# theEricMa/TriplaneTurbo

Measured on AMD Instinct MI355X. Metric: rendered rays/sec (fwd+bwd) at 256x256 rays x 128 samples, higher is better.
Workload: dtype f32 (fp32-grade: exact 3-piece fp16 operand split, 6 x v_mfma_f32_32x32x16_f16 per k-step, fp32 accumulation)

## Files before the change

### triplaneturbo_amd/csrc/tt_backward.hip

```cpp
#include "tt_backward_common.h"

struct BwdGeoParams {
    const float* packed;
    MlpPtrs w;
    const float* rays_o;
    const float* rays_d;
    const float* t_starts;
    const float* t_ends;
    tt_render_cfg cfg;
    TileGeom geom;
    long long n_items;
    int* queue;
    const float* ws;
    int n_copies;
    float* grad_packed;
    MlpGradPtrs grads;
    unsigned long long* phase_cycles;
};

#define GEO_SCRATCH_FLOATS (2 * 64 * XS)
#define GOFF_W1T LDS_GEO_FLOATS
#define GOFF_W2T (GOFF_W1T + IMG16_FLOATS(32, 64))
#define LDS_GEO16_FLOATS (GOFF_W2T + IMG16_FLOATS(64, 64))
#define GLO_W1 LDS_GEO16_FLOATS
#define GLO_W2 (GLO_W1 + LO16_FLOATS(64, 32))
#define GLO_W1T (GLO_W2 + LO16_FLOATS(64, 64))
#define GLO_W2T (GLO_W1T + LO16_FLOATS(32, 64))
#define LDS_GEO3_FLOATS (GLO_W2T + LO16_FLOATS(64, 64))
template <int PREC>
struct GeoWFloats {
    static constexpr int value = PREC == PREC_S3 ? LDS_GEO3_FLOATS : LDS_GEO16_FLOATS;
};

template <int PREC, bool WG16, bool STATS = false>
__global__ __launch_bounds__(256, 1) void k_decode_bwd_geo(BwdGeoParams p) {
    constexpr bool EXACT = PREC == PREC_F32;
    constexpr int NT = PrecNT<PREC>::value, WF = GeoWFloats<PREC>::value;
    __shared__ __attribute__((aligned(16))) float L[WF + 4 * (GEO_SCRATCH_FLOATS + SCATTER_TAG_INTS)];
    {
        MlpPtrs w = p.w;
        stage_weights<PREC, 64, 32>(L + OFF_W1, L + GLO_W1, w.w1);
        stage_weights<PREC, 64, 64>(L + OFF_W2, L + GLO_W2, w.w2);
        lds_load_matrix(L + OFF_W3, w.w3, 1, 64, 64);
        stage_weights_t<PREC, 64, 32>(L + GOFF_W1T, L + GLO_W1T, w.w1);
        stage_weights_t<PREC, 64, 64>(L + GOFF_W2T, L + GLO_W2T, w.w2);
    }
    const tt_render_cfg& cfg = p.cfg;
    float sA1 = 1.f, sU = 1.f, sA2 = 1.f, sV = 1.f;
    if (WG16) {
        const unsigned* bnd = reinterpret_cast<const unsigned*>(p.queue) + TT_SLOT_BOUNDS;
        const float Pm = __builtin_bit_cast(float, bnd[TT_BOUND_PLANES]), Sb = __builtin_bit_cast(float, bnd[TT_BOUND_UP0]),
                    Gb = __builtin_bit_cast(float, bnd[TT_BOUND_UP1]);
        unsigned* word = reinterpret_cast<unsigned*>(L + WF);
        const int t = threadIdx.x;
        float w1row = 0.f, a1col = 0.f, w3abs = 0.f;
        if (t < 64) {
            for (int c = 0; c < 32; ++c) w1row += __builtin_fabsf(p.w.w1[t * 32 + c]);
            for (int r = 0; r < 64; ++r) a1col += __builtin_fabsf(p.w.w2[r * 64 + t]) * __builtin_fabsf(p.w.w3[r]);
            w3abs = __builtin_fabsf(p.w.w3[t]);
        }
        const float W1max = block_max(w1row, word), A1max = block_max(a1col, word), A2max = block_max(w3abs, word);
        const float jsum = (0.5f * cfg.plane_w + 0.5f * cfg.plane_h) / cfg.radius;
        const float Fmax = 3.f * Pm, H1max = W1max * Fmax;
        const float Umax = Fmax * (Sb + 2.f * jsum * Gb), QBmax = Fmax * 2.f * jsum * Gb;
        const float Vmax = Sb * H1max + W1max * QBmax;
        sA1 = wg16_scale(A1max);
        sU = wg16_scale(Umax);
        sA2 = wg16_scale(A2max);
        sV = wg16_scale(Vmax);
    }
    const TileGeom& tg = p.geom;
    const int lane = threadIdx.x & 63, i = lane & 31, hi = lane >> 5, wave_in_blk = threadIdx.x >> 6;
    float* Xs = L + WF + wave_in_blk * (GEO_SCRATCH_FLOATS + SCATTER_TAG_INTS);
    float* Ys = Xs + 64 * XS;
    int* tags = reinterpret_cast<int*>(Ys + 64 * XS);
    scatter_init_tags(tags, lane);
    __syncthreads();
    const int S = cfg.n_samples;
    ItemQueue iq = item_queue(p.queue, tg.n_blocks, tg.n_chunks, tg.unit);
    const int H = cfg.plane_h, W = cfg.plane_w;
    const size_t HW = (size_t)H * W;
    const size_t plane_stride = 6 * HW * TT_C;
    const float ju = 0.5f * W / cfg.radius, jv = 0.5f * H / cfg.radius;
    float* const grad_out =
        p.grad_packed + (size_t)(blockIdx.x % (unsigned)p.n_copies) * cfg.n_prompts * plane_stride;
    const unsigned grad_bytes =
        TT_DBG(cfg.flags, TT_DBG_NO_ATOMICS) ? 0u : (unsigned)(cfg.n_prompts * plane_stride * sizeof(float));

    const TileStats st = STATS ? tile_stats(cfg.stats) : TileStats{nullptr};
    f32x16 accW1[2][1] = {{ZERO16}, {ZERO16}};
    f32x16 accW2[2][2] = {{ZERO16, ZERO16}, {ZERO16, ZERO16}};
    float accw3 = 0.f;
#ifdef TT_TUNING
    unsigned long long ph_acc[20] = {0, 0, 0, 0, 0, 0, 0, 0, 0, 0, 0, 0, 0, 0, 0, 0, 0, 0, 0, 0};
    unsigned long long ph_t = __builtin_amdgcn_s_memtime();
#endif

#pragma nounroll
    for (;;) {
        long long b;
        int ck;
        if (!item_pop(iq, tg.order, tg.n_chunks, b, ck)) break;
        if (b >= tg.n_blocks) continue;
        bool ray_ok;
        const long long ray = tile_ray(tg, b, i, ray_ok);
        const float ray_okf = tt_opaque(ray_ok ? 1.f : 0.f);
        const int ks = i % tg.sb;
        const int view = (int)(ray / cfg.rays_per_view);
        const size_t pofs = (size_t)(view / cfg.views_per_prompt) * plane_stride;
        const float ox = p.rays_o[ray * 3 + 0], oy = p.rays_o[ray * 3 + 1], oz = p.rays_o[ray * 3 + 2];
        const float dx = p.rays_d ? p.rays_d[ray * 3 + 0] : 0.f, dy = p.rays_d ? p.rays_d[ray * 3 + 1] : 0.f,
                    dz = p.rays_d ? p.rays_d[ray * 3 + 2] : 0.f;
        const int s_end = (ck + 1) * tg.chunk < S ? (ck + 1) * tg.chunk : S;
        struct StepIn {
            f32x4 up;
            float ts, te;
        };
        auto load_step = [&](int sb0) {
            StepIn r;
            const int si = sb0 + ks;
            const long long sidx = ray * S + (si < S ? si : S - 1);
            r.up = *reinterpret_cast<const f32x4*>(p.ws + sidx * 4);
            r.ts = p.rays_d ? p.t_starts[sidx] : 0.f;
            r.te = p.rays_d ? p.t_ends[sidx] : 0.f;
            return r;
        };
        StepIn in = load_step(ck * tg.chunk), in_next;
#pragma nounroll
        for (int sb0 = ck * tg.chunk; sb0 < s_end; sb0 += tg.sb, in = in_next) {
            in_next = load_step(sb0 + tg.sb);
            const int si = sb0 + ks;
            const bool rvalid = ray_ok && si < s_end;
            const float vf = ray_okf * (si < s_end ? 1.f : 0.f);
            const float sbar = in.up[0] * vf, gbx = in.up[1] * vf, gby = in.up[2] * vf, gbz = in.up[3] * vf;
            tile_stat(st, TT_STAT_VISITED);
            TT_PHASE(0);
            if (!__any(!((__builtin_fabsf(sbar) + __builtin_fabsf(gbx)) + (__builtin_fabsf(gby) + __builtin_fabsf(gbz)) <=
                         cfg.skip_eps_geo)))
                continue;
            float tm, px, py, pz;
            sample_position(ox, oy, oz, dx, dy, dz, in.ts, in.te, tm, px, py, pz);
            const float X = scale_coord(px, cfg.radius), Y = scale_coord(py, cfg.radius),
                        Z = scale_coord(pz, cfg.radius);
            float f[16], u[16];
            bool anyp[3];
            const bool any = __any(gather_geo_bwd_c(p.packed, (unsigned)(pofs / TT_C), H, W, X, Y, Z, rvalid, sbar, gbx,
                                                    gby, gbz, ju, jv, lane, Xs, f, u, anyp,
                                                    tile_stat_ptr(st, TT_STAT_INBOUNDS)));
            TT_PHASE(1);
            if (!any) continue;
            tile_stat(st, TT_STAT_EXECUTED);
            float h1[32], h2[32], a2[32], a1[32], q[16], u1, u2;
            mvx<PREC, 64, 32, true>(L + OFF_W1, L + GLO_W1, f, h1, i, hi, 1.f, &u1);
#pragma unroll
            for (int r = 0; r < 32; ++r) h1[r] = fmaxf(h1[r], 0.f);
            mvx<PREC, 64, 64, true>(L + OFF_W2, L + GLO_W2, h1, h2, i, hi, u1, &u2);
#pragma unroll
            for (int r = 0; r < 32; ++r) h2[r] = fmaxf(h2[r], 0.f);
#pragma unroll
            for (int g = 0; g < 8; ++g) {
                f32x4 w3 = *reinterpret_cast<const f32x4*>(L + OFF_W3 + 8 * g + 4 * hi);
#pragma unroll
                for (int e2 = 0; e2 < 4; ++e2) a2[4 * g + e2] = h2[4 * g + e2] > 0.f ? w3[e2] : 0.f;
            }
            Split16<64, PAIR_SEQ, NT> a2s, a1s;
            float ua1 = 1.f;
            if (WG16) {
                split16_vec<64, PAIR_SEQ, NT>(a2, sA2, a2s);
                mv16_pre<64, 64, true, NT>(L + GOFF_W2T, a2s, 1.f / sA2, a1, i, hi, &ua1, L + GLO_W2T);
            } else {
                mvtx_copy<PREC, 64, 64, 64>(L + GOFF_W2T, L + GLO_W2T, L + OFF_W2, a2, a1, i, hi);
            }
#pragma unroll
            for (int r = 0; r < 32; ++r) a1[r] = h1[r] > 0.f ? a1[r] : 0.f;
            if (WG16) {
                split16_vec<64, PAIR_SEQ, NT>(a1, sA1 * ua1, a1s);
                mv16_pre<32, 64, false, NT>(L + GOFF_W1T, a1s, 1.f / sA1, q, i, hi, nullptr, L + GLO_W1T);
            } else {
                mvtx_copy<PREC, 32, 64, 32>(L + GOFF_W1T, L + GLO_W1T, L + OFF_W1, a1, q, i, hi);
            }
            TT_PHASE(3);
            {
                float qb[16];
#pragma unroll
                for (int r = 0; r < 16; ++r) qb[r] = fmaf(-sbar, f[r], u[r]);
                const bool region = WG16 ? true : cfg.flags >= 0;
                const bool do_wgrad = region && !TT_DBG(cfg.flags, TT_DBG_NO_WGRAD);
                if (do_wgrad) {
                    if (WG16) {
                        stage_rows16_pre<64>(Xs, a1s, i, hi);
                        stage_rows16<32>(Ys, u, i, hi, sU);
                        wgrad16<64, 32>(accW1, Xs, Ys, i, hi);
                    } else {
                        stage_rows<64>(Xs, a1, i, hi);
                        stage_rows<32>(Ys, u, i, hi);
                        wgrad<64, 32>(accW1, Xs, Ys, i, hi);
                    }
                }
                TT_PHASE(7);
                float t1[32];
                mvx<PREC, 64, 32>(L + OFF_W1, L + GLO_W1, qb, t1, i, hi);
#pragma unroll
                for (int r = 0; r < 32; ++r) t1[r] = h1[r] > 0.f ? t1[r] : 0.f;
                float v[32];
#pragma unroll
                for (int r = 0; r < 32; ++r) v[r] = fmaf(sbar * u1, h1[r], t1[r]);
                TT_PHASE(4);
                if (do_wgrad) {
                    if (WG16) {
                        stage_rows16_pre<64>(Xs, a2s, i, hi);
                        stage_rows16<64>(Ys, v, i, hi, sV);
                        wgrad16<64, 64>(accW2, Xs, Ys, i, hi);
                    } else {
                        stage_rows<64>(Xs, a2, i, hi);
                        stage_rows<64>(Ys, v, i, hi);
                        wgrad<64, 64>(accW2, Xs, Ys, i, hi);
                    }
                }
                TT_PHASE(8);
                float t2[32];
                mvx<PREC, 64, 64>(L + OFF_W2, L + GLO_W2, t1, t2, i, hi);
#pragma unroll
                for (int r = 0; r < 32; ++r) t2[r] = fmaf(sbar * u2, h2[r], h2[r] > 0.f ? t2[r] : 0.f);
                stage_rows<64>(Xs, t2, i, hi);
                accw3 += rowsum32(Xs, lane);
                TT_PHASE(5);
                if (region && !TT_DBG(cfg.flags, TT_DBG_NO_SCATTER)) {
                    scatter_clear<EXACT>(Xs, lane);
                    float* Qs = Xs + SCATTER_M_FLOATS;
                    TT_PHASE(9);
                    const int tex0 = (int)(pofs / TT_C);
                    scatter_planes<EXACT>(grad_out, grad_bytes, Qs, Xs, tags, Qs + 32 * 33, i, hi,
                                          [&](int pl, PlaneRefs& refs) {
                        Corners c;
                        float coef[4];
                        geo_corner_coefs(pl, H, W, X, Y, Z, rvalid, sbar, gbx, gby, gbz, ju, jv, c, coef);
                        int aoff[4];
#pragma unroll
                        for (int q4 = 0; q4 < 4; ++q4) aoff[q4] = tex0 + (int)(pl * HW) + c.off[q4];
                        refs = plane_refs<!EXACT>(coef, aoff, c.hs, hi);
#pragma unroll
                        for (int r = 0; r < 16; ++r) Qs[i * 33 + LIDX(r, hi)] = q[r] * refs.qs;
                    }
#ifdef TT_TUNING
                    , ph_acc + 14
#endif
                    );
                    TT_PHASE(10);
                }
            }
        }
    }
#ifdef TT_TUNING
    TT_PHASE(11);
    if (p.phase_cycles && lane == 0)
        for (int k = 0; k < 20; ++k) atomicAdd(p.phase_cycles + 20 + k, ph_acc[k]);
#endif
    __syncthreads();
    int parity = 0;
    flush_wgrad_reduced<64, 32>(L, parity, accW1, p.grads.w1, wave_in_blk, lane, 1.f / sA1, 1.f / sU);
    flush_wgrad_reduced<64, 64>(L, parity, accW2, p.grads.w2, wave_in_blk, lane, 1.f / sA2, 1.f / sV);
    atomicAdd(p.grads.w3 + lane, accw3);
    tile_stats_flush(st);
}

#ifdef TT_TUNING
unsigned long long* g_phase_cycles = nullptr;
extern "C" int tt_tuning_phase_cycles(unsigned long long* out40) {
    if (!g_phase_cycles) {
        if (hipMalloc((void**)&g_phase_cycles, 40 * sizeof(unsigned long long)) != hipSuccess) return -4;
        if (hipMemset(g_phase_cycles, 0, 40 * sizeof(unsigned long long)) != hipSuccess) return -4;
    }
    if (hipDeviceSynchronize() != hipSuccess) return -4;
    if (out40 && hipMemcpy(out40, g_phase_cycles, 40 * sizeof(unsigned long long), hipMemcpyDeviceToHost) != hipSuccess)
        return -4;
    return hipMemset(g_phase_cycles, 0, 40 * sizeof(unsigned long long)) == hipSuccess ? 0 : -4;
}
#endif
static void launch_bwd_geo(const BwdGeoParams& p0, long long blocks, hipStream_t s) {
    BwdGeoParams p = p0;
#ifdef TT_TUNING
    p.phase_cycles = g_phase_cycles;
#else
    p.phase_cycles = nullptr;
#endif
    if (use_wg16(p.cfg)) {
        unsigned* bnd = reinterpret_cast<unsigned*>(p.queue) + TT_SLOT_BOUNDS;
        launch_planes_bound(p.packed, p.cfg, 0, bnd + TT_BOUND_PLANES, s);
        const long long n = p.cfg.n_rays * p.cfg.n_samples;
        hipLaunchKernelGGL(k_absmax4, dim3(absmax_blocks(n), 1), dim3(256), 0, s, reinterpret_cast<const f32x4*>(p.ws), n, n,
                           bnd + TT_BOUND_UP0, bnd + TT_BOUND_UP1);
    }
    tt_dispatch_prec(tt_prec_of_r(p.cfg.flags), [&](auto P) {
        constexpr int PREC = decltype(P)::value;
        constexpr bool WG16 = PREC != PREC_F32;
        if (p.cfg.stats)
            hipLaunchKernelGGL((k_decode_bwd_geo<PREC, WG16, true>), dim3((unsigned)blocks), dim3(256), 0, s, p);
        else
            hipLaunchKernelGGL((k_decode_bwd_geo<PREC, WG16>), dim3((unsigned)blocks), dim3(256), 0, s, p);
    });
}

extern "C" int tt_render_bwd_geo(const float* packed, const tt_mlp_weights* w, const float* rays_o,
                                 const float* rays_d, const float* t_starts, const float* t_ends,
                                 const tt_render_cfg* cfg, const float* opacity, const float* depth,
                                 const float* trans, const float* sdf, const float* sdf_grad, const float* features,
                                 const float* g_opacity, const float* g_depth, const float* g_rgb_fg,
                                 const float* g_z_variance, const float* g_normal_acc, const float* g_weights,
                                 const float* g_sdf, const float* g_sdf_grad, float* g_inv_std_rays, float* workspace,
                                 float* grad_packed, const tt_mlp_grads* grads, void* stream) {
    int st = tt_validate_cfg(cfg);
    if (st != TT_OK) return st;
    if (!packed || !w || !rays_o || !rays_d || !t_starts || !t_ends || !opacity || !depth || !trans || !sdf ||
        !sdf_grad || !features || !workspace || !grad_packed || !grads)
        return TT_ERR_BAD_ARG;
    if (!w->w1 || !w->w2 || !w->w3 || !grads->w1 || !grads->w2 || !grads->w3) return TT_ERR_BAD_ARG;
    if (grad_buffer_too_large(cfg)) return TT_ERR_UNSUPPORTED;
    int cus = tt_num_cus();
    if (cus <= 0) return TT_ERR_DEVICE;
    hipStream_t s = (hipStream_t)stream;
    st = tt_launch_march_bwd(rays_d, t_starts, t_ends, cfg, sdf, sdf_grad, features, trans, opacity, depth, g_opacity,
                             g_depth, g_rgb_fg, g_z_variance, g_normal_acc, g_weights, g_sdf, g_sdf_grad, g_inv_std_rays,
                             workspace, s);
    if (st != TT_OK) return st;
    BwdGeoParams p;
    tt_fill_rays(p, packed, w, rays_o, rays_d, t_starts, t_ends, *cfg);
    p.cfg.flags |= debug_flags();
    p.ws = workspace;
    p.grad_packed = grad_packed;
    p.n_copies = cfg->grad_copies > 0 ? cfg->grad_copies : 1;
    p.grads = to_gptrs(grads);
    st = tt_plan_queue(cfg, 4LL * cus, s, &p.geom, &p.n_items, &p.queue);
    if (st != TT_OK) return st;
    launch_bwd_geo(p, tt_persistent_blocks(p.n_items, cus, 4), s);
    return tt_check_launch();
}

__global__ void k_interleave_ws(const float* __restrict__ g_sdf, const float* __restrict__ g_sdf_grad,
                                float* __restrict__ ws, long long n) {
    const long long i = (long long)blockIdx.x * blockDim.x + threadIdx.x;
    if (i >= n) return;
    f32x4 o = {g_sdf ? g_sdf[i] : 0.f, g_sdf_grad ? g_sdf_grad[i * 3 + 0] : 0.f,
               g_sdf_grad ? g_sdf_grad[i * 3 + 1] : 0.f, g_sdf_grad ? g_sdf_grad[i * 3 + 2] : 0.f};
    *reinterpret_cast<f32x4*>(ws + i * 4) = o;
}

extern "C" int tt_points_bwd_geo(const float* packed, const tt_mlp_weights* w, const float* points, int32_t n_batch,
                                 int64_t n_points, int32_t n_prompts, int32_t views_per_prompt, int32_t plane_h,
                                 int32_t plane_w, float radius, float sdf_bias_radius, int32_t flags,
                                 const float* g_sdf, const float* g_sdf_grad, float* workspace, float* grad_packed,
                                 const tt_mlp_grads* grads, void* stream) {
    tt_render_cfg cfg;
    int st = points_cfg(&cfg, n_batch, n_points, n_prompts, views_per_prompt, plane_h, plane_w, radius,
                        sdf_bias_radius, 1, flags);
    if (st != TT_OK) return st;
    if (grad_buffer_too_large(&cfg)) return TT_ERR_UNSUPPORTED;
    if (!packed || !w || !points || !workspace || !grad_packed || !grads || (!g_sdf && !g_sdf_grad))
        return TT_ERR_BAD_ARG;
    if (!w->w1 || !w->w2 || !w->w3 || !grads->w1 || !grads->w2 || !grads->w3) return TT_ERR_BAD_ARG;
    int cus = tt_num_cus();
    if (cus <= 0) return TT_ERR_DEVICE;
    hipStream_t s = (hipStream_t)stream;
    const long long n = cfg.n_rays;
    hipLaunchKernelGGL(k_interleave_ws, dim3((unsigned)((n + 255) / 256)), dim3(256), 0, s, g_sdf, g_sdf_grad,
                       workspace, n);
    st = tt_check_launch();
    if (st != TT_OK) return st;
    BwdGeoParams p;
    tt_fill_rays(p, packed, w, points, nullptr, nullptr, nullptr, cfg);
    p.ws = workspace;
    p.grad_packed = grad_packed;
    p.n_copies = 1;
    p.grads = to_gptrs(grads);
    st = tt_plan_queue(&cfg, 4LL * cus, s, &p.geom, &p.n_items, &p.queue);
    if (st != TT_OK) return st;
    launch_bwd_geo(p, tt_persistent_blocks(p.n_items, cus, 4), s);
    return tt_check_launch();
}
```

### triplaneturbo_amd/csrc/tt_backward_common.h

```cpp
#pragma once
#include "tt_device.h"
#include "tt_mfma16.h"
#include "tt_alpha.h"
#include "tt_launch.h"
#include <type_traits>

typedef int i32x4 __attribute__((ext_vector_type(4)));

#ifdef TT_TUNING
#define TT_PHASE(k)                                              \
    do {                                                         \
        __builtin_amdgcn_sched_barrier(0);                       \
        const unsigned long long t_now = __builtin_amdgcn_s_memtime(); \
        ph_acc[k] += t_now - ph_t;                               \
        ph_t = t_now;                                            \
        __builtin_amdgcn_sched_barrier(0);                       \
    } while (0)
#else
#define TT_PHASE(k) \
    do {            \
    } while (0)
#endif
#define XS 36

template <int N>
__device__ __forceinline__ void stage_rows(float* S, const float (&v)[N / 2], int j, int hi) {
#pragma unroll
    for (int r = 0; r < N / 2; ++r) S[LIDX(r, hi) * XS + j] = v[r];
}
template <int N, int OFF, int TOT>
__device__ __forceinline__ void stage_rows_sub(float* S, const float (&v)[TOT], int j, int hi) {
#pragma unroll
    for (int r = 0; r < N / 2; ++r) S[LIDX(r, hi) * XS + j] = v[OFF + r];
}

template <int NX, int NY>
__device__ __forceinline__ void wgrad(f32x16 (&acc)[NX / 32][NY / 32], const float* Xs, const float* Ys, int i,
                                      int hi) {
#pragma unroll
    for (int t4 = 0; t4 < 4; ++t4) {
        f32x4 xa[NX / 32], yb[NY / 32];
#pragma unroll
        for (int m = 0; m < NX / 32; ++m)
            xa[m] = *reinterpret_cast<const f32x4*>(Xs + (32 * m + i) * XS + 16 * hi + 4 * t4);
#pragma unroll
        for (int n = 0; n < NY / 32; ++n)
            yb[n] = *reinterpret_cast<const f32x4*>(Ys + (32 * n + i) * XS + 16 * hi + 4 * t4);
#pragma unroll
        for (int k = 0; k < 4; ++k)
#pragma unroll
            for (int m = 0; m < NX / 32; ++m)
#pragma unroll
                for (int n = 0; n < NY / 32; ++n)
                    acc[m][n] = __builtin_amdgcn_mfma_f32_32x32x2f32(xa[m][k], yb[n][k], acc[m][n], 0, 0, 0);
    }
}

template <int NY>
__device__ __forceinline__ void wgrad_row(f32x16 (&acc)[NY / 32], const float* Xs, const float* Ys, int i, int hi) {
#pragma unroll
    for (int t4 = 0; t4 < 4; ++t4) {
        f32x4 yb[NY / 32];
        const f32x4 xa = *reinterpret_cast<const f32x4*>(Xs + i * XS + 16 * hi + 4 * t4);
#pragma unroll
        for (int n = 0; n < NY / 32; ++n)
            yb[n] = *reinterpret_cast<const f32x4*>(Ys + (32 * n + i) * XS + 16 * hi + 4 * t4);
#pragma unroll
        for (int k = 0; k < 4; ++k)
#pragma unroll
            for (int n = 0; n < NY / 32; ++n)
                acc[n] = __builtin_amdgcn_mfma_f32_32x32x2f32(xa[k], yb[n][k], acc[n], 0, 0, 0);
    }
}

__device__ __forceinline__ float rowsum32(const float* Xs, int lane) {
    float s = 0.f;
#pragma unroll
    for (int g = 0; g < 8; ++g) {
        f32x4 a = *reinterpret_cast<const f32x4*>(Xs + lane * XS + 4 * g);
        s += (a[0] + a[1]) + (a[2] + a[3]);
    }
    return s;
}

typedef unsigned u32x4 __attribute__((ext_vector_type(4)));

__device__ __forceinline__ float wg16_scale(float bound) {
    int E = (int)(__builtin_bit_cast(unsigned, bound * 1.0001f) >> 23) & 0xff;
    E = E < 16 ? 16 : (E > 240 ? 240 : E);
    return __builtin_bit_cast(float, (unsigned)(268 - E) << 23);
}
__device__ __forceinline__ unsigned wg16_pack(float x) {
    unsigned out;
    float r;
    asm("v_cvt_pk_f16_f32 %0, %2, 0\n\t"
        "v_fma_mix_f32 %1, %2, 1.0, -%0 op_sel_hi:[0,0,1]\n\t"
        "v_cvt_pk_f16_f32 %0, %2, %1"
        : "=&v"(out), "=&v"(r)
        : "v"(x));
    return out;
}
template <int N>
__device__ __forceinline__ void stage_rows16(float* S, const float (&v)[N / 2], int j, int hi, float sc) {
    unsigned* U = reinterpret_cast<unsigned*>(S);
#pragma unroll
    for (int r = 0; r < N / 2; ++r) U[LIDX(r, hi) * XS + j] = wg16_pack(v[r] * sc);
}
template <int N, int OFF, int TOT>
__device__ __forceinline__ void stage_rows16_sub(float* S, const float (&v)[TOT], int j, int hi, float sc) {
    unsigned* U = reinterpret_cast<unsigned*>(S);
#pragma unroll
    for (int r = 0; r < N / 2; ++r) U[LIDX(r, hi) * XS + j] = wg16_pack(v[OFF + r] * sc);
}
template <int N, int PAIR, int NT>
__device__ __forceinline__ void stage_rows16_pre(float* S, const Split16<N, PAIR, NT>& v, int j, int hi) {
    unsigned* U = reinterpret_cast<unsigned*>(S);
#pragma unroll
    for (int t = 0; t < N / 4; ++t) {
        U[LIDX(pair_reg<PAIR>(t, 0), hi) * XS + j] = __builtin_amdgcn_perm(v.l[t], v.h[t], 0x05040100u);
        U[LIDX(pair_reg<PAIR>(t, 1), hi) * XS + j] = __builtin_amdgcn_perm(v.l[t], v.h[t], 0x07060302u);
    }
}
__device__ __forceinline__ h8_t wg16_frag(const float* S, int row, int t, int hi) {
    return __builtin_bit_cast(h8_t, *reinterpret_cast<const u32x4*>(S + row * XS + 8 * t + 4 * hi));
}
__device__ __forceinline__ h8_t wg16_swap(h8_t v) {
    u32x4 u = __builtin_bit_cast(u32x4, v);
#pragma unroll
    for (int d = 0; d < 4; ++d) u[d] = __builtin_amdgcn_alignbit(u[d], u[d], 16);
    return __builtin_bit_cast(h8_t, u);
}
template <int NX, int NY>
__device__ __forceinline__ void wgrad16(f32x16 (&acc)[NX / 32][NY / 32], const float* Xs, const float* Ys, int i,
                                        int hi) {
#pragma unroll
    for (int t = 0; t < 4; ++t) {
        h8_t xa[NX / 32], yb[NY / 32], ys[NY / 32];
#pragma unroll
        for (int m = 0; m < NX / 32; ++m) xa[m] = wg16_frag(Xs, 32 * m + i, t, hi);
#pragma unroll
        for (int n = 0; n < NY / 32; ++n) {
            yb[n] = wg16_frag(Ys, 32 * n + i, t, hi);
            ys[n] = wg16_swap(yb[n]);
        }
#pragma unroll
        for (int m = 0; m < NX / 32; ++m)
#pragma unroll
            for (int n = 0; n < NY / 32; ++n)
                acc[m][n] = __builtin_amdgcn_mfma_f32_32x32x16_f16(xa[m], yb[n], acc[m][n], 0, 0, 0);
#pragma unroll
        for (int m = 0; m < NX / 32; ++m)
#pragma unroll
            for (int n = 0; n < NY / 32; ++n)
                acc[m][n] = __builtin_amdgcn_mfma_f32_32x32x16_f16(xa[m], ys[n], acc[m][n], 0, 0, 0);
    }
}
template <int NY>
__device__ __forceinline__ void wgrad16_row(f32x16 (&acc)[NY / 32], const float* Xs, const float* Ys, int i, int hi) {
#pragma unroll
    for (int t = 0; t < 4; ++t) {
        const h8_t xa = wg16_frag(Xs, i, t, hi);
        h8_t yb[NY / 32], ys[NY / 32];
#pragma unroll
        for (int n = 0; n < NY / 32; ++n) {
            yb[n] = wg16_frag(Ys, 32 * n + i, t, hi);
            ys[n] = wg16_swap(yb[n]);
        }
#pragma unroll
        for (int n = 0; n < NY / 32; ++n) acc[n] = __builtin_amdgcn_mfma_f32_32x32x16_f16(xa, yb[n], acc[n], 0, 0, 0);
#pragma unroll
        for (int n = 0; n < NY / 32; ++n) acc[n] = __builtin_amdgcn_mfma_f32_32x32x16_f16(xa, ys[n], acc[n], 0, 0, 0);
    }
}

__device__ __forceinline__ float block_max(float v, unsigned* word) {
    __syncthreads();
    if (threadIdx.x == 0) *word = 0u;
    __syncthreads();
#pragma unroll
    for (int o = 32; o > 0; o >>= 1) v = fmaxf(v, __shfl_xor(v, o));
    if ((threadIdx.x & 63) == 0) atomicMax(word, __builtin_bit_cast(unsigned, v));
    __syncthreads();
    const float r = __builtin_bit_cast(float, *word);
    __syncthreads();
    return r;
}

template <int NX, int NY>
__device__ __forceinline__ void flush_wgrad(const f32x16 (&acc)[NX / 32][NY / 32], float* __restrict__ dst, int i,
                                            int hi, float ux = 1.f, float uy = 1.f) {
#pragma unroll
    for (int m = 0; m < NX / 32; ++m)
#pragma unroll
        for (int n = 0; n < NY / 32; ++n)
#pragma unroll
            for (int r = 0; r < 16; ++r)
                atomicAdd(dst + (32 * m + LIDX(r, hi)) * NY + 32 * n + i, (acc[m][n][r] * ux) * uy);
}

template <class Addr>
__device__ __forceinline__ void flush_tile_reduced(float* R, int parity, const f32x16& acc, int wave, int lane,
                                                   float ux, float uy, Addr addr) {
    float* B = R + parity * 4096;
#pragma unroll
    for (int r = 0; r < 16; ++r) B[(wave * 16 + r) * 64 + lane] = (acc[r] * ux) * uy;
    __syncthreads();
#pragma unroll
    for (int q = 0; q < 4; ++q) {
        const int r = 4 * wave + q;
        const float v = (B[r * 64 + lane] + B[(16 + r) * 64 + lane]) + (B[(32 + r) * 64 + lane] + B[(48 + r) * 64 + lane]);
        atomicAdd(addr(r), v);
    }
}
template <int NX, int NY>
__device__ __forceinline__ void flush_wgrad_reduced(float* R, int& parity, const f32x16 (&acc)[NX / 32][NY / 32],
                                                    float* __restrict__ dst, int wave, int lane, float ux, float uy) {
    const int i = lane & 31, hi = lane >> 5;
#pragma unroll
    for (int m = 0; m < NX / 32; ++m)
#pragma unroll
        for (int n = 0; n < NY / 32; ++n) {
            flush_tile_reduced(R, parity, acc[m][n], wave, lane, ux, uy,
                               [&](int r) { return dst + (32 * m + LIDX(r, hi)) * NY + 32 * n + i; });
            parity ^= 1;
        }
}

#define ZERO16 \
    { 0.f, 0.f, 0.f, 0.f, 0.f, 0.f, 0.f, 0.f, 0.f, 0.f, 0.f, 0.f, 0.f, 0.f, 0.f, 0.f }

#define MS XS

#define M16_RS 40
#define M16_PLANE (65 * M16_RS)
#define SCATTER_M_FLOATS 2624
template <bool EXACT>
__device__ __forceinline__ void scatter_clear(float* M, int lane) {
    const f32x4 z = {0.f, 0.f, 0.f, 0.f};
    if (EXACT) {
#pragma unroll
        for (int g = 0; g < MS / 4; ++g) *reinterpret_cast<f32x4*>(M + lane * MS + 4 * g) = z;
    } else {
#pragma unroll
        for (int g = 0; g < SCATTER_M_FLOATS / 256; ++g) *reinterpret_cast<f32x4*>(M + (g * 64 + lane) * 4) = z;
        if (lane < (SCATTER_M_FLOATS % 256) / 4)
            *reinterpret_cast<f32x4*>(M + ((SCATTER_M_FLOATS / 256) * 64 + lane) * 4) = z;
    }
}

#define SCATTER_TAG_INTS 160

struct PlaneRefs {
    float c0, c1;
    int o0, o1;
    int h0, h1;
    float qs;
};
template <bool NORM>
__device__ __forceinline__ PlaneRefs plane_refs(const float (&coef)[4], const int (&aoff)[4], const int (&hs)[4],
                                                int hi) {
    PlaneRefs r;
    float cn = 1.f;
    r.qs = 1.f;
    if (NORM) {
        const float m = fmaxf(fmaxf(__builtin_fabsf(coef[0]), __builtin_fabsf(coef[1])),
                              fmaxf(__builtin_fabsf(coef[2]), __builtin_fabsf(coef[3])));
        int E = (int)(__builtin_bit_cast(unsigned, m) >> 23);
        E = E < 16 ? 16 : (E > 240 ? 240 : E);
        cn = __builtin_bit_cast(float, (unsigned)(268 - E) << 23);
        r.qs = __builtin_bit_cast(float, (unsigned)(E - 14) << 23);
    }
    r.c0 = (hi ? coef[2] : coef[0]) * cn;
    r.c1 = (hi ? coef[3] : coef[1]) * cn;
    r.o0 = hi ? aoff[2] : aoff[0];
    r.o1 = hi ? aoff[3] : aoff[1];
    r.h0 = hi ? hs[2] : hs[0];
    r.h1 = hi ? hs[3] : hs[1];
    return r;
}
__device__ __forceinline__ void scatter_init_tags(int* tags, int lane) {
    if (lane < 32) tags[lane] = -2;
}

template <bool EXACT>
__device__ __forceinline__ void m_store(float* M, int row, int i, float c) {
    if (EXACT) {
        M[row * MS + i] = c;
    } else {
        half_t h, l;
        split16(c, h, l);
        half_t* Mh = reinterpret_cast<half_t*>(M);
        Mh[row * M16_RS + i] = h;
        Mh[M16_PLANE + row * M16_RS + i] = l;
    }
}
template <bool EXACT>
__device__ __forceinline__ void m_zero(float* M, int row, int i) {
    if (EXACT) {
        M[row * MS + i] = 0.f;
    } else {
        half_t* Mh = reinterpret_cast<half_t*>(M);
        Mh[row * M16_RS + i] = (half_t)0.f;
        Mh[M16_PLANE + row * M16_RS + i] = (half_t)0.f;
    }
}

__device__ __forceinline__ void scatter_lost(const PlaneRefs& r, bool l0, bool l1, const float* Qs, float* Ls,
                                             __amdgpu_buffer_rsrc_t grsrc, int i, int hi) {
    const float lc0 = l0 ? r.c0 : 0.f, lc1 = l1 ? r.c1 : 0.f;
    const unsigned long long bal = __ballot(__builtin_fabsf(lc0) + __builtin_fabsf(lc1) != 0.f);
    if (bal == 0) return;
    float* Lc = Ls;
    int* Lo = reinterpret_cast<int*>(Ls + 32 * 4);
    Lc[4 * i + 2 * hi] = lc0;
    Lc[4 * i + 2 * hi + 1] = lc1;
    Lo[4 * i + 2 * hi] = r.o0;
    Lo[4 * i + 2 * hi + 1] = r.o1;
    unsigned todo = (unsigned)(bal & 0xffffffffull) | (unsigned)(bal >> 32);
    while (todo) {
        const int s0 = __builtin_ctz(todo);
        todo &= todo - 1;
        int s1 = -1;
        if (todo) {
            s1 = __builtin_ctz(todo);
            todo &= todo - 1;
        }
        const int sidx2 = hi ? s1 : s0;
        if (sidx2 >= 0) {
            const f32x4 c4 = *reinterpret_cast<const f32x4*>(Lc + 4 * sidx2);
            const i32x4 o4 = *reinterpret_cast<const i32x4*>(Lo + 4 * sidx2);
            const float v = Qs[sidx2 * 33 + i];
#pragma unroll
            for (int q = 0; q < 4; ++q) {
                const unsigned tex = c4[q] != 0.f ? (unsigned)o4[q] : ~0u;
                __builtin_amdgcn_raw_ptr_buffer_atomic_fadd_f32(v * c4[q], grsrc, (int)((tex << 7) | (4u * (unsigned)i)),
                                                                0, 0);
            }
        }
    }
}

#define SC2_HT 256
#define SC2_CT 136
#define SC2_INTS (SC2_HT + 2 * SC2_CT + 64)

struct Sc2State {
    int rx0, rx1;
    bool l0, l1;
    int n;
};

__device__ __forceinline__ Sc2State sc2_claim_rank(const PlaneRefs& r, int* htab, int* ct, int* cdump, int* dummy,
                                                   int lane, unsigned long long* st = nullptr) {
    Sc2State s;
    const bool a0 = r.c0 != 0.f, a1 = r.c1 != 0.f;
    int* const e0 = a0 ? htab + r.h0 : dummy;
    int* const e1 = a1 ? htab + r.h1 : dummy;
    const int old0 = atomicCAS(e0, -1, r.o0);
    const int old1 = atomicCAS(e1, -1, r.o1);
    const bool w0 = tt_eq_either(old0, -1, r.o0), w1 = tt_eq_either(old1, -1, r.o1);
    s.l0 = !w0;
    s.l1 = !w1;
    const bool m0 = old0 == -1, m1 = old1 == -1;
    const unsigned long long b0 = __ballot(m0), b1 = __ballot(m1);
    const int n0 = __popcll(b0);
    const int r0 = (int)__builtin_amdgcn_mbcnt_hi((unsigned)(b0 >> 32), __builtin_amdgcn_mbcnt_lo((unsigned)b0, 0u));
    const int r1 = n0 + (int)__builtin_amdgcn_mbcnt_hi((unsigned)(b1 >> 32), __builtin_amdgcn_mbcnt_lo((unsigned)b1, 0u));
    s.n = n0 + __popcll(b1);
    int* const x0 = m0 ? e0 : dummy;
    int* const x1 = m1 ? e1 : dummy;
    *x0 = -2 - r0;
    *x1 = -2 - r1;
    *(m0 ? ct + r0 : cdump + lane) = r.o0;
    *(m1 ? ct + r1 : cdump + lane) = r.o1;
    *(lane < 8 ? ct + s.n + lane : cdump + lane) = -1;
    const int q0 = -2 - *e0, q1 = -2 - *e1;
    *x0 = m0 ? -1 : -2;
    *x1 = m1 ? -1 : -2;
    s.rx0 = w0 ? q0 : 255;
    s.rx1 = w1 ? q1 : 255;
#ifdef TT_TUNING
    if (st) {
        st[0] += __popcll(__ballot(a0)) + __popcll(__ballot(a1));
        st[1] += __popcll(__ballot((s.l0 ? r.c0 : 0.f) != 0.f)) + __popcll(__ballot((s.l1 ? r.c1 : 0.f) != 0.f));
        st[2] += 1;
    }
#endif
    return s;
}
__device__ __forceinline__ int sc2_row_a(int rx) { return rx < 64 ? rx : 64; }
__device__ __forceinline__ int sc2_row_b(int rx) {
    const unsigned d = (unsigned)(rx - 64);
    return (int)(d < 64u ? d : 64u);
}

struct ScA16 {
    h8_t ah[2][2], al[2][2];
};
struct ScB16 {
    float bs[2][8];
    h8_t bh[2], bl[2];
    float bun;
};
struct ScA32 {
    f32x4 a4[2][4];
};
struct ScB32 {
    float bq[16];
};
__device__ __forceinline__ void sc2_load_a(const float* M, int i, int hi, int n, ScA16& A) {
    const half_t* Mh = reinterpret_cast<const half_t*>(M);
#pragma unroll
    for (int m = 0; m < 2; ++m) {
        if (m == 1 && n <= 32) break;
#pragma unroll
        for (int ks = 0; ks < 2; ++ks) {
            const half_t* a = Mh + (32 * m + i) * M16_RS + 16 * ks + 8 * hi;
            A.ah[m][ks] = *reinterpret_cast<const h8_t*>(a);
            A.al[m][ks] = *reinterpret_cast<const h8_t*>(a + M16_PLANE);
        }
    }
}
__device__ __forceinline__ void sc2_load_a(const float* M, int i, int hi, int n, ScA32& A) {
#pragma unroll
    for (int m = 0; m < 2; ++m) {
        if (m == 1 && n <= 32) break;
#pragma unroll
        for (int t4 = 0; t4 < 4; ++t4)
            A.a4[m][t4] = *reinterpret_cast<const f32x4*>(M + (32 * m + i) * MS + 16 * hi + 4 * t4);
    }
}
__device__ __forceinline__ void sc2_load_b(const float* Qs, int i, int hi, ScB16& B) {
#pragma unroll
    for (int ks = 0; ks < 2; ++ks)
#pragma unroll
        for (int j = 0; j < 8; ++j) B.bs[ks][j] = Qs[(16 * ks + 8 * hi + j) * 33 + i];
}
__device__ __forceinline__ void sc2_load_b(const float* Qs, int i, int hi, ScB32& B) {
#pragma unroll
    for (int t = 0; t < 16; ++t) B.bq[t] = Qs[(t + 16 * hi) * 33 + i];
}
__device__ __forceinline__ void sc2_split_b(ScB32&) {}
__device__ __forceinline__ void sc2_split_b(ScB16& B) {
    const float (&bs)[2][8] = B.bs;
    float mx = 0.f;
#pragma unroll
    for (int ks = 0; ks < 2; ++ks)
#pragma unroll
        for (int j = 0; j < 8; ++j) mx = fmaxf(mx, __builtin_fabsf(bs[ks][j]));
    mx = fmaxf(mx, __shfl_xor(mx, 32));
    int E = (int)(__builtin_bit_cast(unsigned, mx) >> 23);
    E = E < 16 ? 16 : (E > 240 ? 240 : E);
    const float bsc = __builtin_bit_cast(float, (unsigned)(268 - E) << 23);
    B.bun = __builtin_bit_cast(float, (unsigned)(E - 14) << 23);
#pragma unroll
    for (int ks = 0; ks < 2; ++ks)
#pragma unroll
        for (int j = 0; j < 4; ++j) {
            const float x0 = bs[ks][2 * j] * bsc, x1 = bs[ks][2 * j + 1] * bsc;
            h2_t ph, pq;
            split_pair(x0, x1, ph, pq);
            B.bh[ks][2 * j] = ph.x;
            B.bh[ks][2 * j + 1] = ph.y;
            B.bl[ks][2 * j] = pq.x;
            B.bl[ks][2 * j + 1] = pq.y;
        }
}
__device__ __forceinline__ void sc2_gemm(const ScA16& A, const ScB16& B, int n, f32x16& acc0, f32x16& acc1) {
    acc0 = f32x16 ZERO16;
#pragma unroll
    for (int ks = 0; ks < 2; ++ks) {
        acc0 = __builtin_amdgcn_mfma_f32_32x32x16_f16(A.ah[0][ks], B.bh[ks], acc0, 0, 0, 0);
        acc0 = __builtin_amdgcn_mfma_f32_32x32x16_f16(A.ah[0][ks], B.bl[ks], acc0, 0, 0, 0);
        acc0 = __builtin_amdgcn_mfma_f32_32x32x16_f16(A.al[0][ks], B.bh[ks], acc0, 0, 0, 0);
    }
#pragma unroll
    for (int r = 0; r < 16; ++r) acc0[r] *= B.bun;
    if (n > 32) {
        acc1 = f32x16 ZERO16;
#pragma unroll
        for (int ks = 0; ks < 2; ++ks) {
            acc1 = __builtin_amdgcn_mfma_f32_32x32x16_f16(A.ah[1][ks], B.bh[ks], acc1, 0, 0, 0);
            acc1 = __builtin_amdgcn_mfma_f32_32x32x16_f16(A.ah[1][ks], B.bl[ks], acc1, 0, 0, 0);
            acc1 = __builtin_amdgcn_mfma_f32_32x32x16_f16(A.al[1][ks], B.bh[ks], acc1, 0, 0, 0);
        }
#pragma unroll
        for (int r = 0; r < 16; ++r) acc1[r] *= B.bun;
    }
}
__device__ __forceinline__ void sc2_gemm(const ScA32& A, const ScB32& B, int n, f32x16& acc0, f32x16& acc1) {
    acc0 = f32x16 ZERO16;
#pragma unroll
    for (int t = 0; t < 16; ++t) acc0 = __builtin_amdgcn_mfma_f32_32x32x2f32(A.a4[0][t >> 2][t & 3], B.bq[t], acc0, 0, 0, 0);
    if (n > 32) {
        acc1 = f32x16 ZERO16;
#pragma unroll
        for (int t = 0; t < 16; ++t) acc1 = __builtin_amdgcn_mfma_f32_32x32x2f32(A.a4[1][t >> 2][t & 3], B.bq[t], acc1, 0, 0, 0);
    }
}
__device__ __forceinline__ void sc2_flush(const f32x16& acc0, const f32x16& acc1, const int* ct, int n,
                                          __amdgpu_buffer_rsrc_t grsrc, unsigned lane_b, int hi) {
#pragma unroll
    for (int g = 0; g < 4; ++g) {
        if (n > 8 * g) {
            const i32x4 k0 = *reinterpret_cast<const i32x4*>(ct + 8 * g + 4 * hi);
#pragma unroll
            for (int e2 = 0; e2 < 4; ++e2)
                __builtin_amdgcn_raw_ptr_buffer_atomic_fadd_f32(acc0[4 * g + e2], grsrc,
                                                                (int)(((unsigned)k0[e2] << 7) | lane_b), 0, 0);
        }
    }
#pragma unroll
    for (int g = 0; g < 4; ++g) {
        if (n > 32 + 8 * g) {
            const i32x4 k1 = *reinterpret_cast<const i32x4*>(ct + 32 + 8 * g + 4 * hi);
#pragma unroll
            for (int e2 = 0; e2 < 4; ++e2)
                __builtin_amdgcn_raw_ptr_buffer_atomic_fadd_f32(acc1[4 * g + e2], grsrc,
                                                                (int)(((unsigned)k1[e2] << 7) | lane_b), 0, 0);
        }
    }
}

template <bool EXACT, class Prep>
__device__ __forceinline__ void scatter_planes(float* __restrict__ grad, unsigned grad_bytes, const float* Qs, float* M,
                                               int* tags, float* Ls, int i, int hi, Prep&& prep,
                                               unsigned long long* st = nullptr) {
    const __amdgpu_buffer_rsrc_t grsrc = __builtin_amdgcn_make_buffer_rsrc(grad, 0, (int)grad_bytes, 0x00020000);
    const unsigned lane_b = 4u * (unsigned)i;
    const int lane = i + 32 * hi;
    int* const dummy = tags + i;
    int* const htab = reinterpret_cast<int*>(Ls + 256);
    int* const ctag = htab + SC2_HT;
    int* const cdump = ctag + 2 * SC2_CT;
    typedef typename std::conditional<EXACT, ScA32, ScA16>::type AOp;
    typedef typename std::conditional<EXACT, ScB32, ScB16>::type BOp;
#ifdef TT_TUNING
    unsigned long long sp_t = __builtin_amdgcn_s_memtime();
#define TT_SUBPHASE(k)                                                    \
    do {                                                                  \
        if (st) {                                                         \
            __builtin_amdgcn_sched_barrier(0);                            \
            const unsigned long long t_now = __builtin_amdgcn_s_memtime(); \
            st[k] += t_now - sp_t;                                        \
            sp_t = t_now;                                                 \
            __builtin_amdgcn_sched_barrier(0);                            \
        }                                                                 \
    } while (0)
#else
#define TT_SUBPHASE(k) \
    do {               \
    } while (0)
#endif
    {
        const i32x4 e4 = {-1, -1, -1, -1};
        *reinterpret_cast<i32x4*>(htab + 4 * lane) = e4;
    }
    PlaneRefs rc, rn;
    Sc2State sc, sn;
    prep(0, rc);
    sc = sc2_claim_rank(rc, htab, ctag, cdump, dummy, lane, st);
    scatter_lost(rc, sc.l0, sc.l1, Qs, Ls, grsrc, i, hi);
    m_store<EXACT>(M, sc2_row_a(sc.rx0), i, rc.c0);
    m_store<EXACT>(M, sc2_row_a(sc.rx1), i, rc.c1);
#pragma unroll
    for (int pl = 0; pl < 3; ++pl) {
        const int* const ct = ctag + SC2_CT * (pl & 1);
        int* const ct_next = ctag + SC2_CT * ((pl + 1) & 1);
        const bool pass_b = sc.n > 64;
        f32x16 acc0, acc1;
        AOp A;
        BOp B;
        sc2_load_a(M, i, hi, sc.n, A);
        m_zero<EXACT>(M, sc2_row_a(sc.rx0), i);
        m_zero<EXACT>(M, sc2_row_a(sc.rx1), i);
        if (pass_b) {
            m_store<EXACT>(M, sc2_row_b(sc.rx0), i, rc.c0);
            m_store<EXACT>(M, sc2_row_b(sc.rx1), i, rc.c1);
        }
        sc2_load_b(Qs, i, hi, B);
        if (pl < 2) prep(pl + 1, rn);
        sc2_split_b(B);
        sc2_gemm(A, B, sc.n, acc0, acc1);
        TT_SUBPHASE(3);
        if (pass_b) {
            sc2_flush(acc0, acc1, ct, 64, grsrc, lane_b, hi);
            sc2_load_a(M, i, hi, sc.n - 64, A);
            m_zero<EXACT>(M, sc2_row_b(sc.rx0), i);
            m_zero<EXACT>(M, sc2_row_b(sc.rx1), i);
        }
        if (pl < 2) sn = sc2_claim_rank(rn, htab, ct_next, cdump, dummy, lane, st);
        TT_SUBPHASE(4);
        if (pass_b) {
            sc2_gemm(A, B, sc.n - 64, acc0, acc1);
            sc2_flush(acc0, acc1, ct + 64, sc.n - 64, grsrc, lane_b, hi);
        } else {
            sc2_flush(acc0, acc1, ct, sc.n, grsrc, lane_b, hi);
        }
        if (pl < 2) {
            scatter_lost(rn, sn.l0, sn.l1, Qs, Ls, grsrc, i, hi);
            m_store<EXACT>(M, sc2_row_a(sn.rx0), i, rn.c0);
            m_store<EXACT>(M, sc2_row_a(sn.rx1), i, rn.c1);
            rc = rn;
            sc = sn;
        }
        TT_SUBPHASE(5);
    }
}

struct BwdTexParams {
    const float* packed;
    MlpPtrs w;
    const float* rays_o;
    const float* rays_d;
    const float* t_starts;
    const float* t_ends;
    tt_render_cfg cfg;
    const float* weights;
    const float* features;
    const float* g_rgb;
    const float* g_features;
    TileGeom geom;
    long long n_items;
    int* queue;
    int n_copies;
    float* grad_packed;
    MlpGradPtrs grads;
    unsigned long long* phase_cycles;
};

#define TEX_W_FLOATS (LDS_W_FLOATS - OFF_V1)
#define TV1 0
#define TV2 (OFF_V2 - OFF_V1)
#define TV3 (OFF_V3 - OFF_V1)
#define TV1T TEX_W_FLOATS
#define TV2T (TV1T + IMG16_FLOATS(96, 64))
#define TEX_W16_FLOATS (TV2T + IMG16_FLOATS(64, 64))
#define TLO_V1 TEX_W_FLOATS
#define TLO_V2 (TLO_V1 + LO16_FLOATS(64, 96))
#define TEX_W3P_FLOATS (TLO_V2 + LO16_FLOATS(64, 64))
template <int PREC>
struct TexWFloats {
    static constexpr int value = PREC == PREC_S3 ? TEX_W3P_FLOATS : TEX_W16_FLOATS;
};

static inline bool grad_buffer_too_large(const tt_render_cfg* cfg) {
    return (long long)cfg->n_prompts * 6 * cfg->plane_h * cfg->plane_w * TT_C * 4 >= (1LL << 32) - 256;
}

#ifdef TT_TUNING
extern unsigned long long* g_phase_cycles;
#endif
static __global__ __launch_bounds__(256) void k_absmax4(const f32x4* __restrict__ x, long long seg4, long long seg_stride4,
                                                 unsigned* __restrict__ out0, unsigned* __restrict__ out1) {
    const f32x4* seg = x + (long long)blockIdx.y * seg_stride4;
    const long long stride = (long long)gridDim.x * blockDim.x;
    float m0 = 0.f, m1 = 0.f;
    long long e = (long long)blockIdx.x * blockDim.x + threadIdx.x;
    for (; e + 3 * stride < seg4; e += 4 * stride) {
        const f32x4 a = seg[e], b = seg[e + stride], c = seg[e + 2 * stride], d = seg[e + 3 * stride];
        m0 = fmaxf(fmaxf(m0, __builtin_fabsf(a[0])), fmaxf(__builtin_fabsf(b[0]), fmaxf(__builtin_fabsf(c[0]), __builtin_fabsf(d[0]))));
#pragma unroll
        for (int k = 1; k < 4; ++k)
            m1 = fmaxf(fmaxf(m1, __builtin_fabsf(a[k])), fmaxf(__builtin_fabsf(b[k]), fmaxf(__builtin_fabsf(c[k]), __builtin_fabsf(d[k]))));
    }
    for (; e < seg4; e += stride) {
        const f32x4 v = seg[e];
        m0 = fmaxf(m0, __builtin_fabsf(v[0]));
        m1 = fmaxf(m1, fmaxf(__builtin_fabsf(v[1]), fmaxf(__builtin_fabsf(v[2]), __builtin_fabsf(v[3]))));
    }
    if (!out1) m0 = fmaxf(m0, m1);
    __shared__ unsigned w[2];
    if (threadIdx.x < 2) w[threadIdx.x] = 0u;
    __syncthreads();
    for (int o = 32; o > 0; o >>= 1) {
        m0 = fmaxf(m0, __shfl_xor(m0, o));
        m1 = fmaxf(m1, __shfl_xor(m1, o));
    }
    if ((threadIdx.x & 63) == 0) {
        atomicMax(&w[0], __builtin_bit_cast(unsigned, m0));
        atomicMax(&w[1], __builtin_bit_cast(unsigned, m1));
    }
    __syncthreads();
    if (threadIdx.x == 0) {
        if (w[0] > __hip_atomic_load(out0, __ATOMIC_RELAXED, __HIP_MEMORY_SCOPE_AGENT)) atomicMax(out0, w[0]);
        if (out1 && w[1] > __hip_atomic_load(out1, __ATOMIC_RELAXED, __HIP_MEMORY_SCOPE_AGENT)) atomicMax(out1, w[1]);
    }
}
static __global__ __launch_bounds__(256) void k_absmax1(const float* __restrict__ x, long long n, unsigned* __restrict__ out) {
    float m = 0.f;
    for (long long e = (long long)blockIdx.x * blockDim.x + threadIdx.x; e < n; e += (long long)gridDim.x * blockDim.x)
        m = fmaxf(m, __builtin_fabsf(x[e]));
    for (int o = 32; o > 0; o >>= 1) m = fmaxf(m, __shfl_xor(m, o));
    __shared__ unsigned w;
    if (threadIdx.x == 0) w = 0u;
    __syncthreads();
    if ((threadIdx.x & 63) == 0) atomicMax(&w, __builtin_bit_cast(unsigned, m));
    __syncthreads();
    if (threadIdx.x == 0 && w > __hip_atomic_load(out, __ATOMIC_RELAXED, __HIP_MEMORY_SCOPE_AGENT)) atomicMax(out, w);
}
static inline unsigned absmax_blocks(long long n) {
    long long b = (n + 256 * 8 - 1) / (256 * 8);
    return (unsigned)(b < 1 ? 1 : (b > 1024 ? 1024 : b));
}
static inline void launch_planes_bound(const float* packed, const tt_render_cfg& cfg, int first_plane, unsigned* out,
                                hipStream_t s) {
    const long long hw4 = (long long)cfg.plane_h * cfg.plane_w * TT_C / 4;
    hipLaunchKernelGGL(k_absmax4, dim3(absmax_blocks(3 * hw4), (unsigned)cfg.n_prompts), dim3(256), 0, s,
                       reinterpret_cast<const f32x4*>(packed) + first_plane * hw4, 3 * hw4, 6 * hw4, out,
                       (unsigned*)nullptr);
}

static inline bool use_wg16(const tt_render_cfg& cfg) { return !(cfg.flags & TT_R_EXACT_F32); }

static inline int points_cfg(tt_render_cfg* c, int32_t n_batch, int64_t n_points, int32_t n_prompts,
                      int32_t views_per_prompt, int32_t plane_h, int32_t plane_w, float radius, float sdf_bias_radius,
                      int32_t grad_copies, int32_t q_flags) {
    if (!tt_points_counts_ok(n_batch, n_points, n_prompts, views_per_prompt, q_flags) || n_points > 0x7fffffffLL)
        return TT_ERR_BAD_ARG;
    c->n_prompts = n_prompts;
    c->views_per_prompt = views_per_prompt;
    c->plane_h = plane_h;
    c->plane_w = plane_w;
    c->rays_per_view = (int32_t)n_points;
    c->n_samples = 1;
    c->n_rays = (int64_t)n_batch * n_points;
    c->radius = radius;
    c->sdf_bias_radius = sdf_bias_radius;
    c->inv_std = 1.f;
    c->inv_std_dev = nullptr;
    c->stats = nullptr;
    c->cos_anneal_ratio = 1.f;
    c->rgb_grad_shrink = 1.f;
    c->flags = (q_flags & TT_Q_EXACT_F32) ? TT_R_EXACT_F32 : ((q_flags & TT_Q_SPLIT2) ? TT_R_SPLIT2 : 0);
    c->image_w = 0;
    c->tile_sb = 1;
    c->tile_chunk = 0;
    c->grad_copies = grad_copies;
    c->skip_eps_tex = 0.f;
    c->skip_eps_geo = 0.f;
    return tt_validate_cfg(c);
}
```

### triplaneturbo_amd/csrc/tt_backward_tex.hip

```cpp
#include "tt_backward_common.h"

#define TEX_SCRATCH_FLOATS (128 * XS)

template <int PREC, bool WG16, bool STATS = false>
__global__ __launch_bounds__(256, 1) void k_decode_bwd_tex(BwdTexParams p) {
    constexpr bool EXACT = PREC == PREC_F32;
    constexpr bool COPIES = PREC != PREC_S3;
    constexpr int NT = PrecNT<PREC>::value, WF = TexWFloats<PREC>::value;
    __shared__ __attribute__((aligned(16))) float Lt[WF + 4 * (TEX_SCRATCH_FLOATS + SCATTER_TAG_INTS)];
    {
        MlpPtrs w = p.w;
        stage_weights<PREC, 64, 96>(Lt + TV1, Lt + TLO_V1, w.v1);
        stage_weights<PREC, 64, 64>(Lt + TV2, Lt + TLO_V2, w.v2);
        lds_load_matrix(Lt + TV3, w.v3, 3, 64, 64);
        if constexpr (COPIES) {
            stage_weights_t<PREC, 64, 96>(Lt + TV1T, nullptr, w.v1);
            stage_weights_t<PREC, 64, 64>(Lt + TV2T, nullptr, w.v2);
        }
    }
    const tt_render_cfg& cfg = p.cfg;
    float sKB1 = 1.f, sE = 1.f, sK2B = 1.f, sK1 = 1.f;
    if (WG16) {
        const unsigned* bnd = reinterpret_cast<const unsigned*>(p.queue) + TT_SLOT_BOUNDS;
        const float Pm = __builtin_bit_cast(float, bnd[TT_BOUND_PLANES]), Gr = __builtin_bit_cast(float, bnd[TT_BOUND_UP0]),
                    Gf = __builtin_bit_cast(float, bnd[TT_BOUND_UP1]);
        unsigned* word = reinterpret_cast<unsigned*>(Lt + WF);
        const int t = threadIdx.x;
        const float CBmax = __builtin_fabsf(cfg.rgb_grad_shrink) * (1.002f * 0.25f) * Gr + Gf;
        float v1row = 0.f, k2b = 0.f, kb1 = 0.f;
        if (t < 64) {
            for (int c = 0; c < 96; ++c) v1row += __builtin_fabsf(p.w.v1[t * 96 + c]);
            for (int o = 0; o < 3; ++o) k2b += __builtin_fabsf(p.w.v3[o * 64 + t]);
            for (int r = 0; r < 64; ++r) {
                float c3 = 0.f;
                for (int o = 0; o < 3; ++o) c3 += __builtin_fabsf(p.w.v3[o * 64 + r]);
                kb1 += __builtin_fabsf(p.w.v2[r * 64 + t]) * c3;
            }
        }
        const float V1max = block_max(v1row, word), K2Bw = block_max(k2b, word), KB1w = block_max(kb1, word);
        sE = wg16_scale(Pm);
        sK1 = wg16_scale(V1max * Pm);
        sK2B = wg16_scale(K2Bw * CBmax);
        sKB1 = wg16_scale(KB1w * CBmax);
    }
    const TileGeom& tg = p.geom;
    const int lane = threadIdx.x & 63, i = lane & 31, hi = lane >> 5, wave_in_blk = threadIdx.x >> 6;
    float* Xs = Lt + WF + wave_in_blk * (TEX_SCRATCH_FLOATS + SCATTER_TAG_INTS);
    float* Ys = Xs + 32 * XS;
    int* tags = reinterpret_cast<int*>(Xs + 128 * XS);
    float* Cb = Xs + 32;
#define CB_AT(idx) Cb[((idx) >> 2) * XS + ((idx)&3)]
    scatter_init_tags(tags, lane);
    __syncthreads();
    const int S = cfg.n_samples;
    const int H = cfg.plane_h, W = cfg.plane_w;
    const size_t HW = (size_t)H * W;
    const size_t plane_stride = 6 * HW * TT_C;
    ItemQueue iq = item_queue(p.queue, tg.n_blocks, tg.n_chunks, tg.unit);
    const float shrink = cfg.rgb_grad_shrink;
    float* const grad_out =
        p.grad_packed + (size_t)(blockIdx.x % (unsigned)p.n_copies) * cfg.n_prompts * plane_stride;
    const unsigned grad_bytes =
        TT_DBG(cfg.flags, TT_DBG_NO_ATOMICS) ? 0u : (unsigned)(cfg.n_prompts * plane_stride * sizeof(float));

    const TileStats st = STATS ? tile_stats(cfg.stats) : TileStats{nullptr};
    f32x16 accV1a[2][2] = {{ZERO16, ZERO16}, {ZERO16, ZERO16}};
    f32x16 accV1b[2][1] = {{ZERO16}, {ZERO16}};
    f32x16 accV2[2][2] = {{ZERO16, ZERO16}, {ZERO16, ZERO16}};
    float accV3[2][3] = {{0.f, 0.f, 0.f}, {0.f, 0.f, 0.f}};
#ifdef TT_TUNING
    unsigned long long ph_acc[20] = {0, 0, 0, 0, 0, 0, 0, 0, 0, 0, 0, 0, 0, 0, 0, 0, 0, 0, 0, 0};
    unsigned long long scat_st[3] = {0, 0, 0};
    unsigned long long ph_t = __builtin_amdgcn_s_memtime();
#endif

#pragma nounroll
    for (;;) {
      long long b;
      int ck;
      TT_PHASE(17);
      if (!item_pop(iq, tg.order, tg.n_chunks, b, ck)) break;
      TT_PHASE(18);
        if (b >= tg.n_blocks) continue;
      bool ray_ok;
      const long long ray = tile_ray(tg, b, i, ray_ok);
      const float ray_okf = tt_opaque(ray_ok ? 1.f : 0.f);
      const int ks = i % tg.sb;
      const int view = (int)(ray / cfg.rays_per_view);
      const size_t pofs = (size_t)(view / cfg.views_per_prompt) * plane_stride;
      const int s_end = (ck + 1) * tg.chunk < S ? (ck + 1) * tg.chunk : S;
      TT_PHASE(19);
      struct StepIn {
          float wgt, f[3], gf[3], ts, te;
      };
      auto load_step = [&](int sb0) {
          StepIn r;
          const int si = sb0 + ks;
          const long long sidx = ray * S + (si < S ? si : S - 1);
          r.wgt = p.weights ? p.weights[sidx] : 0.f;
#pragma unroll
          for (int o = 0; o < 3; ++o) {
              r.f[o] = p.weights ? p.features[sidx * 3 + o] : 0.f;
              r.gf[o] = p.g_features ? p.g_features[sidx * 3 + o] : 0.f;
          }
          r.ts = p.rays_d ? p.t_starts[sidx] : 0.f;
          r.te = p.rays_d ? p.t_ends[sidx] : 0.f;
          return r;
      };
      StepIn in = load_step(ck * tg.chunk), in_next;
#pragma nounroll
      for (int sb0 = ck * tg.chunk; sb0 < s_end; sb0 += tg.sb, in = in_next) {
        in_next = load_step(sb0 + tg.sb);
        const int si = sb0 + ks;
        const bool valid = ray_ok && si < s_end;
        const float vf = ray_okf * (si < s_end ? 1.f : 0.f);
        long long rr = ray;
        asm volatile("" : "+v"(rr));
        const float ox = p.rays_o[rr * 3 + 0], oy = p.rays_o[rr * 3 + 1], oz = p.rays_o[rr * 3 + 2];
        const float dx = p.rays_d ? p.rays_d[rr * 3 + 0] : 0.f, dy = p.rays_d ? p.rays_d[rr * 3 + 1] : 0.f,
                    dz = p.rays_d ? p.rays_d[rr * 3 + 2] : 0.f;
        float grgb[3];
#pragma unroll
        for (int o = 0; o < 3; ++o) grgb[o] = p.g_rgb ? p.g_rgb[rr * 3 + o] : 0.f;
        float cb[3];
#pragma unroll
        for (int o = 0; o < 3; ++o) {
            const float s = sigmoid_(in.f[o]);
            const float c = shrink * in.wgt * grgb[o] * 1.002f * s * (1.f - s) + in.gf[o];
            cb[o] = c * vf;
        }
        tile_stat(st, TT_STAT_VISITED);
        TT_PHASE(0);
        if (!__any(!((__builtin_fabsf(cb[0]) + __builtin_fabsf(cb[1])) + __builtin_fabsf(cb[2]) <= cfg.skip_eps_tex)))
            continue;
#ifdef TT_TUNING
        {
            const unsigned long long live = __ballot(cb[0] != 0.f || cb[1] != 0.f || cb[2] != 0.f) & 0xffffffffull;
            const unsigned long long big = __ballot(fabsf(cb[0]) + fabsf(cb[1]) + fabsf(cb[2]) > 1e-12f) & 0xffffffffull;
            ph_acc[12] += 1;
            ph_acc[13] += __popcll(live);
            ph_acc[14] += __popcll(big);
        }
#endif
        float tm, px, py, pz;
        sample_position(ox, oy, oz, dx, dy, dz, in.ts, in.te, tm, px, py, pz);
        const float X = scale_coord(px, cfg.radius), Y = scale_coord(py, cfg.radius), Z = scale_coord(pz, cfg.radius);
        float e[48];
        const bool any =
            __any(gather_tex_c(p.packed, (unsigned)(pofs / TT_C), H, W, X, Y, Z, valid, lane, Xs, e,
                               tile_stat_ptr(st, TT_STAT_INBOUNDS)));
        TT_PHASE(1);
        if (!any) continue;
        tile_stat(st, TT_STAT_EXECUTED);
        const bool region = cfg.flags >= 0;
        const bool region_w = WG16 ? true : region;
        const bool do_wgrad = region_w && !TT_DBG(cfg.flags, TT_DBG_NO_WGRAD);
        float k1[32], k2[32];
        if (WG16) {
            Split16<96, PAIR_SEQ, NT> es;
            split16_vec<96, PAIR_SEQ, NT>(e, sE, es);
            if (do_wgrad) stage_rows16_pre<96>(Ys, es, i, hi);
            TT_PHASE(2);
            mv16_pre<64, 96, false, NT>(Lt + TV1, es, 1.f / sE, k1, i, hi, nullptr, Lt + TLO_V1);
        } else {
            if (do_wgrad) stage_rows<96>(Ys, e, i, hi);
            TT_PHASE(2);
            mvx<PREC, 64, 96>(Lt + TV1, Lt + TLO_V1, e, k1, i, hi);
        }
#pragma unroll
        for (int r = 0; r < 32; ++r) k1[r] = fmaxf(k1[r], 0.f);
        TT_PHASE(3);
        Split16<64, PAIR_SEQ, NT> k1s;
        if (WG16) {
            split16_vec<64, PAIR_SEQ, NT>(k1, sK1, k1s);
            mv16_pre<64, 64, false, NT>(Lt + TV2, k1s, 1.f / sK1, k2, i, hi, nullptr, Lt + TLO_V2);
        } else {
            mvx<PREC, 64, 64>(Lt + TV2, Lt + TLO_V2, k1, k2, i, hi);
        }
#pragma unroll
        for (int r = 0; r < 32; ++r) k2[r] = fmaxf(k2[r], 0.f);
        TT_PHASE(4);
        if (hi == 0) {
            CB_AT(0 * 32 + i) = cb[0];
            CB_AT(1 * 32 + i) = cb[1];
            CB_AT(2 * 32 + i) = cb[2];
        }
#pragma unroll
        for (int h2 = 0; h2 < 2; ++h2) {
            if (h2 == 0)
                stage_rows_sub<32, 0, 32>(Xs, k2, i, hi);
            else
                stage_rows_sub<32, 16, 32>(Xs, k2, i, hi);
#pragma unroll
            for (int g = 0; g < 4; ++g) {
                const f32x4 kk = *reinterpret_cast<const f32x4*>(Xs + i * XS + 16 * hi + 4 * g);
#pragma unroll
                for (int o = 0; o < 3; ++o) {
                    const f32x4 cc = *reinterpret_cast<const f32x4*>(&CB_AT(o * 32 + 16 * hi + 4 * g));
                    accV3[h2][o] += (kk[0] * cc[0] + kk[1] * cc[1]) + (kk[2] * cc[2] + kk[3] * cc[3]);
                }
            }
        }
        TT_PHASE(5);
#pragma unroll
        for (int g = 0; g < 8; ++g) {
            f32x4 v0 = *reinterpret_cast<const f32x4*>(Lt + TV3 + 0 * 64 + 8 * g + 4 * hi);
            f32x4 v1 = *reinterpret_cast<const f32x4*>(Lt + TV3 + 1 * 64 + 8 * g + 4 * hi);
            f32x4 v2 = *reinterpret_cast<const f32x4*>(Lt + TV3 + 2 * 64 + 8 * g + 4 * hi);
#pragma unroll
            for (int e2 = 0; e2 < 4; ++e2) {
                const float t = fmaf(v0[e2], cb[0], fmaf(v1[e2], cb[1], v2[e2] * cb[2]));
                k2[4 * g + e2] = k2[4 * g + e2] > 0.f ? t : 0.f;
            }
        }
        float kb1[32];
        if constexpr (COPIES)
            mvtx_copy<PREC, 64, 64, 64>(Lt + TV2T, nullptr, Lt + TV2, k2, kb1, i, hi);
        else
            mvtx<PREC, 64, 64, 64>(Lt + TV2, Lt + TLO_V2, 0, k2, kb1, i, hi);
#pragma unroll
        for (int r = 0; r < 32; ++r) kb1[r] = k1[r] > 0.f ? kb1[r] : 0.f;
        TT_PHASE(6);
        if (do_wgrad) {
            __builtin_amdgcn_sched_barrier(0);
#pragma unroll
            for (int h2 = 0; h2 < 2; ++h2) {
                if (WG16) {
                    if (h2 == 0)
                        stage_rows16_sub<32, 0, 32>(Xs, kb1, i, hi, sKB1);
                    else
                        stage_rows16_sub<32, 16, 32>(Xs, kb1, i, hi, sKB1);
                    wgrad16_row<64>(accV1a[h2], Xs, Ys, i, hi);
                    wgrad16_row<32>(accV1b[h2], Xs, Ys + 64 * XS, i, hi);
                } else {
                    if (h2 == 0)
                        stage_rows_sub<32, 0, 32>(Xs, kb1, i, hi);
                    else
                        stage_rows_sub<32, 16, 32>(Xs, kb1, i, hi);
                    wgrad_row<64>(accV1a[h2], Xs, Ys, i, hi);
                    wgrad_row<32>(accV1b[h2], Xs, Ys + 64 * XS, i, hi);
                }
            }
            TT_PHASE(7);
            if (WG16) {
                stage_rows16<64>(Xs, k2, i, hi, sK2B);
                stage_rows16_pre<64>(Xs + 64 * XS, k1s, i, hi);
                wgrad16<64, 64>(accV2, Xs, Xs + 64 * XS, i, hi);
            } else {
                stage_rows<64>(Xs, k2, i, hi);
                stage_rows<64>(Xs + 64 * XS, k1, i, hi);
                wgrad<64, 64>(accV2, Xs, Xs + 64 * XS, i, hi);
            }
            TT_PHASE(8);
        }
        if (region && !TT_DBG(cfg.flags, TT_DBG_NO_SCATTER)) {
            float* M = Xs;
            float* Es = Xs + (EXACT ? 65 * XS : SCATTER_M_FLOATS);
            scatter_clear<EXACT>(M, lane);
            float eb[48];
            if constexpr (COPIES)
                mvtx_copy<PREC, 96, 64, 96>(Lt + TV1T, nullptr, Lt + TV1, kb1, eb, i, hi);
            else
                mvtx<PREC, 96, 64, 96>(Lt + TV1, Lt + TLO_V1, 0, kb1, eb, i, hi);
            TT_PHASE(9);
            const int tex0 = (int)(pofs / TT_C);
            scatter_planes<EXACT>(grad_out, grad_bytes, Es, M, tags, Es + 32 * 33, i, hi, [&](int pl, PlaneRefs& refs) {
                Corners c;
                corners_setup(PLANE_U(pl, X, Y, Z), PLANE_V(pl, X, Y, Z), H, W, valid, c);
                int aoff[4];
#pragma unroll
                for (int q4 = 0; q4 < 4; ++q4)
                    aoff[q4] = tex0 + (int)((3 + pl) * HW) + c.off[q4];
                refs = plane_refs<!EXACT>(c.w, aoff, c.hs, hi);
#pragma unroll
                for (int r = 0; r < 16; ++r) Es[i * 33 + LIDX(r, hi)] = eb[16 * pl + r] * refs.qs;
            }
#ifdef TT_TUNING
            , scat_st
#endif
            );
            TT_PHASE(10);
        }
      }
    }
#ifdef TT_TUNING
    TT_PHASE(11);
    ph_acc[15] = scat_st[0];
    ph_acc[16] = scat_st[1];
    if (p.phase_cycles && lane == 0)
        for (int k = 0; k < 20; ++k) atomicAdd(p.phase_cycles + k, ph_acc[k]);
#endif
    __syncthreads();
    int parity = 0;
    {
        const float u1 = 1.f / sKB1, u2 = 1.f / sE;
#pragma unroll
        for (int m = 0; m < 2; ++m) {
            float* const base = p.grads.v1 + (32 * m) * 96 + i;
            flush_tile_reduced(Lt, parity, accV1a[m][0], wave_in_blk, lane, u1, u2,
                               [&](int r) { return base + LIDX(r, hi) * 96; });
            parity ^= 1;
            flush_tile_reduced(Lt, parity, accV1a[m][1], wave_in_blk, lane, u1, u2,
                               [&](int r) { return base + LIDX(r, hi) * 96 + 32; });
            parity ^= 1;
            flush_tile_reduced(Lt, parity, accV1b[m][0], wave_in_blk, lane, u1, u2,
                               [&](int r) { return base + LIDX(r, hi) * 96 + 64; });
            parity ^= 1;
        }
    }
    flush_wgrad_reduced<64, 64>(Lt, parity, accV2, p.grads.v2, wave_in_blk, lane, 1.f / sK2B, 1.f / sK1);
#pragma unroll
    for (int h2 = 0; h2 < 2; ++h2)
#pragma unroll
        for (int o = 0; o < 3; ++o) atomicAdd(p.grads.v3 + o * 64 + 32 * h2 + i, accV3[h2][o]);
    tile_stats_flush(st);
}

static void launch_bwd_tex(const BwdTexParams& p0, long long blocks, hipStream_t s) {
    BwdTexParams p = p0;
#ifdef TT_TUNING
    p.phase_cycles = g_phase_cycles;
#else
    p.phase_cycles = nullptr;
#endif
    if (use_wg16(p.cfg)) {
        unsigned* bnd = reinterpret_cast<unsigned*>(p.queue) + TT_SLOT_BOUNDS;
        launch_planes_bound(p.packed, p.cfg, 3, bnd + TT_BOUND_PLANES, s);
        if (p.g_rgb)
            hipLaunchKernelGGL(k_absmax1, dim3(absmax_blocks(p.cfg.n_rays * 3)), dim3(256), 0, s, p.g_rgb,
                               (long long)p.cfg.n_rays * 3, bnd + TT_BOUND_UP0);
        if (p.g_features) {
            const long long n = p.cfg.n_rays * p.cfg.n_samples * 3;
            hipLaunchKernelGGL(k_absmax1, dim3(absmax_blocks(n)), dim3(256), 0, s, p.g_features, n, bnd + TT_BOUND_UP1);
        }
    }
    tt_dispatch_prec(tt_prec_of_r(p.cfg.flags), [&](auto P) {
        constexpr int PREC = decltype(P)::value;
        constexpr bool WG16 = PREC != PREC_F32;
        if (p.cfg.stats)
            hipLaunchKernelGGL((k_decode_bwd_tex<PREC, WG16, true>), dim3((unsigned)blocks), dim3(256), 0, s, p);
        else
            hipLaunchKernelGGL((k_decode_bwd_tex<PREC, WG16>), dim3((unsigned)blocks), dim3(256), 0, s, p);
    });
}

extern "C" int tt_render_bwd_tex(const float* packed, const tt_mlp_weights* w, const float* rays_o,
                                 const float* rays_d, const float* t_starts, const float* t_ends,
                                 const tt_render_cfg* cfg, const float* weights, const float* features,
                                 const float* g_rgb_fg, const float* g_features, float* grad_packed,
                                 const tt_mlp_grads* grads, void* stream) {
    int st = tt_validate_cfg(cfg);
    if (st != TT_OK) return st;
    if (!packed || !w || !rays_o || !rays_d || !t_starts || !t_ends || !weights || !features || !grad_packed ||
        !grads)
        return TT_ERR_BAD_ARG;
    if (!w->v1 || !w->v2 || !w->v3 || !grads->v1 || !grads->v2 || !grads->v3) return TT_ERR_BAD_ARG;
    if (grad_buffer_too_large(cfg)) return TT_ERR_UNSUPPORTED;
    int cus = tt_num_cus();
    if (cus <= 0) return TT_ERR_DEVICE;
    hipStream_t s = (hipStream_t)stream;
    BwdTexParams p;
    tt_fill_rays(p, packed, w, rays_o, rays_d, t_starts, t_ends, *cfg);
    p.cfg.flags |= debug_flags();
    p.weights = weights;
    p.features = features;
    p.g_rgb = g_rgb_fg;
    p.g_features = g_features;
    p.grad_packed = grad_packed;
    p.n_copies = cfg->grad_copies > 0 ? cfg->grad_copies : 1;
    p.grads = to_gptrs(grads);
    st = tt_plan_queue(cfg, 4LL * cus, s, &p.geom, &p.n_items, &p.queue, 12);
    if (st != TT_OK) return st;
    launch_bwd_tex(p, tt_persistent_blocks(p.n_items, cus, 4), s);
    return tt_check_launch();
}

extern "C" int tt_points_bwd_tex(const float* packed, const tt_mlp_weights* w, const float* points, int32_t n_batch,
                                 int64_t n_points, int32_t n_prompts, int32_t views_per_prompt, int32_t plane_h,
                                 int32_t plane_w, float radius, int32_t plane_base, int32_t flags,
                                 const float* g_features, float* grad_packed, const tt_mlp_grads* grads,
                                 void* stream) {
    tt_render_cfg cfg;
    int st = points_cfg(&cfg, n_batch, n_points, n_prompts, views_per_prompt, plane_h, plane_w, radius, 0.5f, 1,
                        flags);
    if (st != TT_OK) return st;
    if (grad_buffer_too_large(&cfg)) return TT_ERR_UNSUPPORTED;
    if (!packed || !w || !points || !g_features || !grad_packed || !grads) return TT_ERR_BAD_ARG;
    if (!w->v1 || !w->v2 || !w->v3 || !grads->v1 || !grads->v2 || !grads->v3) return TT_ERR_BAD_ARG;
    if (plane_base != 0 && plane_base != 3) return TT_ERR_BAD_ARG;
    int cus = tt_num_cus();
    if (cus <= 0) return TT_ERR_DEVICE;
    const ptrdiff_t shift = (ptrdiff_t)(plane_base - 3) * plane_h * plane_w * TT_C;
    hipStream_t s = (hipStream_t)stream;
    BwdTexParams p;
    tt_fill_rays(p, packed + shift, w, points, nullptr, nullptr, nullptr, cfg);
    p.weights = nullptr;
    p.features = nullptr;
    p.g_rgb = nullptr;
    p.g_features = g_features;
    p.grad_packed = grad_packed + shift;
    p.n_copies = 1;
    p.grads = to_gptrs(grads);
    st = tt_plan_queue(&cfg, 4LL * cus, s, &p.geom, &p.n_items, &p.queue);
    if (st != TT_OK) return st;
    launch_bwd_tex(p, tt_persistent_blocks(p.n_items, cus, 4), s);
    return tt_check_launch();
}
```

### triplaneturbo_amd/csrc/tt_device.h

```cpp
#pragma once
#include <hip/hip_runtime.h>
#include <stdint.h>

typedef float f32x16 __attribute__((ext_vector_type(16)));
typedef float f32x4 __attribute__((ext_vector_type(4)));

#ifdef TT_TUNING
#define TT_DBG(flags, bit) (((flags) & (bit)) != 0)
#else
#define TT_DBG(flags, bit) false
#endif
#define TT_DBG_NO_SCATTER 0x100
#define TT_DBG_NO_WGRAD 0x200
#define TT_DBG_NO_GATHER 0x400
#define TT_DBG_NO_MLP 0x800
#define TT_DBG_NO_STORE 0x1000
#define TT_DBG_NO_ATOMICS 0x2000

#define TT_C 32
#define TT_HID 64
#define TT_TILE 32

#define LIDX(r, hi) (((r) & 3) + 8 * ((r) >> 2) + 4 * (hi))

#include "tt_mask.h"

#define W1S 36
#define W2S 68
#define V1S 100
#define V2S 68
#define OFF_W1 0
#define OFF_W2 (OFF_W1 + 64 * W1S)
#define OFF_W3 (OFF_W2 + 64 * W2S)
#define OFF_V1 (OFF_W3 + 64)
#define OFF_V2 (OFF_V1 + 64 * V1S)
#define OFF_V3 (OFF_V2 + 64 * V2S)
#define LDS_W_FLOATS (OFF_V3 + 3 * 64)
#define LDS_GEO_FLOATS (OFF_W3 + 64)

struct MlpPtrs {
    const float* w1;
    const float* w2;
    const float* w3;
    const float* v1;
    const float* v2;
    const float* v3;
};

__device__ __forceinline__ void lds_load_matrix(float* dst, const float* __restrict__ src, int rows, int cols,
                                                int stride) {
    for (int e = threadIdx.x; e < rows * cols; e += blockDim.x) {
        int r = e / cols, c = e - r * cols;
        dst[r * stride + c] = src[e];
    }
}

__device__ __forceinline__ void lds_load_geo_weights(float* L, const MlpPtrs& w) {
    lds_load_matrix(L + OFF_W1, w.w1, 64, 32, W1S);
    lds_load_matrix(L + OFF_W2, w.w2, 64, 64, W2S);
    lds_load_matrix(L + OFF_W3, w.w3, 1, 64, 64);
}
__device__ __forceinline__ void lds_load_tex_weights(float* L, const MlpPtrs& w) {
    lds_load_matrix(L + OFF_V1, w.v1, 64, 96, V1S);
    lds_load_matrix(L + OFF_V2, w.v2, 64, 64, V2S);
    lds_load_matrix(L + OFF_V3, w.v3, 3, 64, 64);
}

template <int NOUT, int NIN>
__device__ __forceinline__ void mv_fwd(const float* Wl, const float (&x)[NIN / 2], float (&y)[NOUT / 2], int i,
                                       int hi) {
    constexpr int MT = NOUT / 32;
    f32x16 acc[MT];
    f32x4 a_cur[MT], a_nxt[MT];
    const float* row = Wl + i * (NIN + 4) + 4 * hi;
#pragma unroll
    for (int m = 0; m < MT; ++m) {
        acc[m] = f32x16{0.f, 0.f, 0.f, 0.f, 0.f, 0.f, 0.f, 0.f, 0.f, 0.f, 0.f, 0.f, 0.f, 0.f, 0.f, 0.f};
        a_cur[m] = *reinterpret_cast<const f32x4*>(row + 32 * m * (NIN + 4));
    }
#pragma unroll
    for (int g = 0; g < NIN / 8; ++g) {
        if (g + 1 < NIN / 8) {
#pragma unroll
            for (int m = 0; m < MT; ++m)
                a_nxt[m] = *reinterpret_cast<const f32x4*>(row + 32 * m * (NIN + 4) + 8 * (g + 1));
        }
#pragma unroll
        for (int k = 0; k < 4; ++k)
#pragma unroll
            for (int m = 0; m < MT; ++m)
                acc[m] = __builtin_amdgcn_mfma_f32_32x32x2f32(a_cur[m][k], x[4 * g + k], acc[m], 0, 0, 0);
#pragma unroll
        for (int m = 0; m < MT; ++m) a_cur[m] = a_nxt[m];
    }
#pragma unroll
    for (int m = 0; m < MT; ++m)
#pragma unroll
        for (int k = 0; k < 16; ++k) y[16 * m + k] = acc[m][k];
}

template <int NOUT, int NIN, int STRIDE = NOUT + 4>
__device__ __forceinline__ void mv_bwd(const float* Wl, const float (&x)[NIN / 2], float (&y)[NOUT / 2], int i,
                                       int hi) {
    constexpr int MT = NOUT / 32;
    const float* base = Wl + 4 * hi * STRIDE + i;
    if (MT == 1) {
        f32x16 acc0 = {0.f, 0.f, 0.f, 0.f, 0.f, 0.f, 0.f, 0.f, 0.f, 0.f, 0.f, 0.f, 0.f, 0.f, 0.f, 0.f};
        f32x16 acc1 = acc0;
#pragma unroll
        for (int r = 0; r < NIN / 4; ++r) {
            const float a0 = base[LIDX(r, 0) * STRIDE], a1 = base[LIDX(r + NIN / 4, 0) * STRIDE];
            acc0 = __builtin_amdgcn_mfma_f32_32x32x2f32(a0, x[r], acc0, 0, 0, 0);
            acc1 = __builtin_amdgcn_mfma_f32_32x32x2f32(a1, x[r + NIN / 4], acc1, 0, 0, 0);
        }
#pragma unroll
        for (int k = 0; k < 16; ++k) y[k] = acc0[k] + acc1[k];
    } else {
        f32x16 acc[MT];
#pragma unroll
        for (int m = 0; m < MT; ++m)
            acc[m] = f32x16{0.f, 0.f, 0.f, 0.f, 0.f, 0.f, 0.f, 0.f, 0.f, 0.f, 0.f, 0.f, 0.f, 0.f, 0.f, 0.f};
#pragma unroll
        for (int r = 0; r < NIN / 2; ++r) {
#pragma unroll
            for (int m = 0; m < MT; ++m) {
                const float a = base[LIDX(r, 0) * STRIDE + 32 * m];
                acc[m] = __builtin_amdgcn_mfma_f32_32x32x2f32(a, x[r], acc[m], 0, 0, 0);
            }
        }
#pragma unroll
        for (int m = 0; m < MT; ++m)
#pragma unroll
            for (int k = 0; k < 16; ++k) y[16 * m + k] = acc[m][k];
    }
}

template <int N>
__device__ __forceinline__ float dot_lds(const float* wl, const float (&x)[N / 2], int hi) {
    float s = 0.f;
#pragma unroll
    for (int g = 0; g < N / 8; ++g) {
        f32x4 a = *reinterpret_cast<const f32x4*>(wl + 8 * g + 4 * hi);
        s = fmaf(a[0], x[4 * g + 0], s);
        s = fmaf(a[1], x[4 * g + 1], s);
        s = fmaf(a[2], x[4 * g + 2], s);
        s = fmaf(a[3], x[4 * g + 3], s);
    }
    return s + __shfl_xor(s, 32);
}

struct Corners {
    int off[4];
    float w[4];
    float du[4];
    float dv[4];
    int hs[4];
    bool any;
    int inmask;
};

#pragma clang fp contract(off)
__device__ __forceinline__ void corners_setup(float gx, float gy, int H, int W, bool valid, Corners& c) {
    gx = __builtin_fabsf(gx) < 1e30f ? gx : 4.f;
    gy = __builtin_fabsf(gy) < 1e30f ? gy : 4.f;
    float ix = ((gx + 1.f) * (float)W - 1.f) / 2.f;
    float iy = ((gy + 1.f) * (float)H - 1.f) / 2.f;
    float fx = floorf(ix), fy = floorf(iy);
    float wx1 = ix - fx, wx0 = (fx + 1.f) - ix;
    float wy1 = iy - fy, wy0 = (fy + 1.f) - iy;
    int x0 = (int)fminf(fmaxf(fx, -2.f), (float)W + 1.f);
    int y0 = (int)fminf(fmaxf(fy, -2.f), (float)H + 1.f);
    x0 = valid ? x0 : -2;
    const float bx0 = (unsigned)x0 < (unsigned)W ? 1.f : 0.f, bx1 = (unsigned)(x0 + 1) < (unsigned)W ? 1.f : 0.f;
    const float by0 = (unsigned)y0 < (unsigned)H ? 1.f : 0.f, by1 = (unsigned)(y0 + 1) < (unsigned)H ? 1.f : 0.f;
    const float mx0 = wx0 * bx0, mx1 = wx1 * bx1, my0 = wy0 * by0, my1 = wy1 * by1;
    c.w[0] = mx0 * my0;
    c.w[1] = mx1 * my0;
    c.w[2] = mx0 * my1;
    c.w[3] = mx1 * my1;
    c.du[0] = -(my0 * bx0);
    c.du[1] = my0 * bx1;
    c.du[2] = -(my1 * bx0);
    c.du[3] = my1 * bx1;
    c.dv[0] = -(mx0 * by0);
    c.dv[1] = -(mx1 * by0);
    c.dv[2] = mx0 * by1;
    c.dv[3] = mx1 * by1;
    const int xc0 = min(max(x0, 0), W - 1), xc1 = min(max(x0 + 1, 0), W - 1);
    const int yc0 = min(max(y0, 0), H - 1) * W, yc1 = min(max(y0 + 1, 0), H - 1) * W;
    c.off[0] = yc0 + xc0;
    c.off[1] = yc0 + xc1;
    c.off[2] = yc1 + xc0;
    c.off[3] = yc1 + xc1;
    const float i0 = bx0 * by0, i1 = bx1 * by0, i2 = bx0 * by1, i3 = bx1 * by1;
    c.hs[0] = ((y0 & 15) << 4) | (x0 & 15);
    c.hs[1] = ((y0 & 15) << 4) | ((x0 + 1) & 15);
    c.hs[2] = (((y0 + 1) & 15) << 4) | (x0 & 15);
    c.hs[3] = (((y0 + 1) & 15) << 4) | ((x0 + 1) & 15);
    c.any = (bx0 + bx1) * (by0 + by1) != 0.f;
    c.inmask = (int)i0 | ((int)i1 << 1) | ((int)i2 << 2) | ((int)i3 << 3);
}

__device__ __forceinline__ float scale_coord(float x, float radius) {
    float t = (x - (-radius)) / (radius - (-radius));
    return t * 2.f + (-1.f);
}

__device__ __forceinline__ void sample_position(float ox, float oy, float oz, float dx, float dy, float dz, float ts,
                                                float te, float& tm, float& px, float& py, float& pz) {
    tm = (ts + te) / 2.f;
    px = ox + dx * tm;
    py = oy + dy * tm;
    pz = oz + dz * tm;
}

__device__ __forceinline__ float sphere_bias(float px, float py, float pz, float bias_radius, float& nrm) {
    nrm = sqrtf((px * px + py * py) + pz * pz);
    return nrm - bias_radius;
}
#pragma clang fp contract(fast)

#define PLANE_U(p, X, Y, Z) ((p) == 2 ? (Z) : (X))
#define PLANE_V(p, X, Y, Z) ((p) == 1 ? (Z) : (Y))

template <bool NEED_J>
__device__ __forceinline__ bool gather_geo(const float* __restrict__ planes, int H, int W, float X, float Y, float Z,
                                           bool valid, float jscale_u, float jscale_v, int hi, float (&f)[16],
                                           float (&jx)[16], float (&jy)[16], float (&jz)[16], int dbg = 0) {
#pragma unroll
    for (int r = 0; r < 16; ++r) {
        f[r] = 0.f;
        jx[r] = 0.f;
        jy[r] = 0.f;
        jz[r] = 0.f;
    }
    bool any = false;
    const size_t HW = (size_t)H * W;
#pragma unroll
    for (int p = 0; p < 3; ++p) {
        Corners c;
        corners_setup(PLANE_U(p, X, Y, Z), PLANE_V(p, X, Y, Z), H, W, valid, c);
        if (!__any(c.any)) continue;
        any = any || c.any;
#pragma unroll
        for (int k = 0; k < 4; ++k) {
            const f32x4* t = reinterpret_cast<const f32x4*>(planes + (p * HW + (size_t)c.off[k]) * TT_C) + hi;
            f32x4 v[4];
            if (TT_DBG(dbg, TT_DBG_NO_GATHER)) {
                const f32x4 z = {c.w[k], c.du[k], c.dv[k], X};
                v[0] = v[1] = v[2] = v[3] = z;
            } else {
                v[0] = t[0];
                v[1] = t[2];
                v[2] = t[4];
                v[3] = t[6];
            }
            const float wk = c.w[k], a = c.du[k] * jscale_u, b = c.dv[k] * jscale_v;
#pragma unroll
            for (int q = 0; q < 4; ++q)
#pragma unroll
                for (int e = 0; e < 4; ++e) {
                    const float tv = v[q][e];
                    f[4 * q + e] = fmaf(wk, tv, f[4 * q + e]);
                    if (NEED_J) {
                        if (p == 0) {
                            jx[4 * q + e] = fmaf(a, tv, jx[4 * q + e]);
                            jy[4 * q + e] = fmaf(b, tv, jy[4 * q + e]);
                        } else if (p == 1) {
                            jx[4 * q + e] = fmaf(a, tv, jx[4 * q + e]);
                            jz[4 * q + e] = fmaf(b, tv, jz[4 * q + e]);
                        } else {
                            jz[4 * q + e] = fmaf(a, tv, jz[4 * q + e]);
                            jy[4 * q + e] = fmaf(b, tv, jy[4 * q + e]);
                        }
                    }
                }
        }
    }
    return any;
}

__device__ __forceinline__ bool gather_tex(const float* __restrict__ planes, int H, int W, float X, float Y, float Z,
                                           bool valid, int hi, float (&e)[48], int dbg = 0) {
#pragma unroll
    for (int r = 0; r < 48; ++r) e[r] = 0.f;
    bool any = false;
    const size_t HW = (size_t)H * W;
#pragma unroll
    for (int p = 0; p < 3; ++p) {
        Corners c;
        corners_setup(PLANE_U(p, X, Y, Z), PLANE_V(p, X, Y, Z), H, W, valid, c);
        if (!__any(c.any)) continue;
        any = any || c.any;
#pragma unroll
        for (int k = 0; k < 4; ++k) {
            const f32x4* t = reinterpret_cast<const f32x4*>(planes + ((3 + p) * HW + (size_t)c.off[k]) * TT_C) + hi;
            f32x4 v[4];
            if (TT_DBG(dbg, TT_DBG_NO_GATHER)) {
                const f32x4 z = {c.w[k], Y, Z, X};
                v[0] = v[1] = v[2] = v[3] = z;
            } else {
                v[0] = t[0];
                v[1] = t[2];
                v[2] = t[4];
                v[3] = t[6];
            }
            const float wk = c.w[k];
#pragma unroll
            for (int q = 0; q < 4; ++q)
#pragma unroll
                for (int ee = 0; ee < 4; ++ee) e[16 * p + 4 * q + ee] = fmaf(wk, v[q][ee], e[16 * p + 4 * q + ee]);
        }
    }
    return any;
}

struct TileStats {
    unsigned long long* p;
    unsigned* w;
};
enum { TT_STAT_VISITED = 0, TT_STAT_EXECUTED = 1, TT_STAT_INBOUNDS = 2 };
__device__ __forceinline__ TileStats tile_stats(uint64_t* stats64) {
    TileStats st = {nullptr, nullptr};
    __shared__ unsigned tt_stat_slots[16 * 4];
    st.p = reinterpret_cast<unsigned long long*>(stats64);
    if (st.p) {
        st.w = tt_stat_slots + 4 * __builtin_amdgcn_readfirstlane((int)(threadIdx.x >> 6));
        if ((threadIdx.x & 63) < 4) st.w[threadIdx.x & 63] = 0u;
    }
    return st;
}
__device__ __forceinline__ void tile_stat(const TileStats& st, int which, unsigned v = 1) {
    if (st.p) {
        if ((threadIdx.x & 63) == 0) st.w[which] += v;
    }
}
__device__ __forceinline__ unsigned* tile_stat_ptr(const TileStats& st, int which) { return st.p ? st.w + which : nullptr; }
__device__ __forceinline__ void tile_stats_flush(const TileStats& st) {
    if (st.p) {
        const int l = threadIdx.x & 63;
        if (l < 3) atomicAdd(st.p + l, (unsigned long long)st.w[l]);
    }
}

typedef int ti32x4 __attribute__((ext_vector_type(4)));
#define GC_TABLE_FLOATS(NW) (3 * 32 * 4 * (1 + (NW)))
#define GC_TILE_FLOATS (32 * 36)

#define GC_PLANE_TABLE_FLOATS (32 * 16)
#define GC_SCRATCH_FLOATS (GC_PLANE_TABLE_FLOATS + GC_TILE_FLOATS)

__device__ __forceinline__ const f32x4* gc_addr(const float* __restrict__ planes, int texel, unsigned cbyte) {
    return reinterpret_cast<const f32x4*>(reinterpret_cast<const char*>(planes) + (((unsigned)texel << 7) | cbyte));
}

__device__ __forceinline__ void gc_load16(const float* __restrict__ pl, const int* Toff, int js, f32x4 (&t)[4][4]) {
#pragma unroll
    for (int n = 0; n < 4; ++n) {
        const ti32x4 o4 = *reinterpret_cast<const ti32x4*>(Toff + (8 * n + js) * 4);
#pragma unroll
        for (int k = 0; k < 4; ++k) t[n][k] = *reinterpret_cast<const f32x4*>(pl + (size_t)(unsigned)o4[k] * TT_C);
    }
}

__device__ __forceinline__ void gc_transpose(float* R, const f32x4 (&acc)[4], int i, int hi, int js, int c,
                                             float* out16) {
#pragma unroll
    for (int n = 0; n < 4; ++n) *reinterpret_cast<f32x4*>(R + (8 * n + js) * 36 + 4 * c) = acc[n];
#pragma unroll
    for (int q = 0; q < 4; ++q) {
        const f32x4 v = *reinterpret_cast<const f32x4*>(R + i * 36 + 4 * (hi + 2 * q));
#pragma unroll
        for (int ee = 0; ee < 4; ++ee) out16[4 * q + ee] = v[ee];
    }
}

template <bool NEED_J>
__device__ __forceinline__ bool gather_geo_c(const float* __restrict__ planes, unsigned tex0, int H, int W, float X,
                                             float Y, float Z, bool valid, float jscale_u, float jscale_v, int lane,
                                             float* T, float (&f)[16], float (&jx)[16], float (&jy)[16],
                                             float (&jz)[16], unsigned* inb = nullptr) {
    const int i = lane & 31, hi = lane >> 5, js = lane >> 3, c = lane & 7;
    int* Toff = reinterpret_cast<int*>(T);
    float* Tw = T + 32 * 4;
    float* Ta = T + 2 * 32 * 4;
    float* Tb = T + 3 * 32 * 4;
    float* R = T + GC_PLANE_TABLE_FLOATS;
    const size_t HW = (size_t)H * W;
    const f32x4 z4 = {0.f, 0.f, 0.f, 0.f};
    f32x4 af[4] = {z4, z4, z4, z4}, ax[4] = {z4, z4, z4, z4}, ay[4] = {z4, z4, z4, z4}, az[4] = {z4, z4, z4, z4};
    bool any = false;
#pragma unroll
    for (int p = 0; p < 3; ++p) {
        Corners cn;
        corners_setup(PLANE_U(p, X, Y, Z), PLANE_V(p, X, Y, Z), H, W, valid, cn);
        any = any || cn.any;
        const unsigned long long inmask = __ballot(cn.any);
        if (inb) {
            if ((threadIdx.x & 63) == 0) *inb += (unsigned)__popcll(inmask & 0xffffffffull);
        }
        if (inmask == 0) continue;
        if (hi == 0) {
            const unsigned b = tex0 + (unsigned)(p * HW);
            const ti32x4 o = {(int)(b + cn.off[0]), (int)(b + cn.off[1]), (int)(b + cn.off[2]), (int)(b + cn.off[3])};
            *reinterpret_cast<ti32x4*>(Toff + i * 4) = o;
            const f32x4 w = {cn.w[0], cn.w[1], cn.w[2], cn.w[3]};
            *reinterpret_cast<f32x4*>(Tw + i * 4) = w;
        } else if (NEED_J) {
            const f32x4 a = {cn.du[0] * jscale_u, cn.du[1] * jscale_u, cn.du[2] * jscale_u, cn.du[3] * jscale_u};
            const f32x4 b = {cn.dv[0] * jscale_v, cn.dv[1] * jscale_v, cn.dv[2] * jscale_v, cn.dv[3] * jscale_v};
            *reinterpret_cast<f32x4*>(Ta + i * 4) = a;
            *reinterpret_cast<f32x4*>(Tb + i * 4) = b;
        }
        f32x4 t[4][4];
        gc_load16(planes + 4 * c, Toff, js, t);
#pragma unroll
        for (int n = 0; n < 4; ++n) {
            const f32x4 w4 = *reinterpret_cast<const f32x4*>(Tw + (8 * n + js) * 4);
            f32x4 a4 = z4, b4 = z4;
            if (NEED_J) {
                a4 = *reinterpret_cast<const f32x4*>(Ta + (8 * n + js) * 4);
                b4 = *reinterpret_cast<const f32x4*>(Tb + (8 * n + js) * 4);
            }
#pragma unroll
            for (int k = 0; k < 4; ++k)
#pragma unroll
                for (int ee = 0; ee < 4; ++ee) {
                    const float tv = t[n][k][ee];
                    af[n][ee] = fmaf(w4[k], tv, af[n][ee]);
                    if (NEED_J) {
                        if (p == 0) {
                            ax[n][ee] = fmaf(a4[k], tv, ax[n][ee]);
                            ay[n][ee] = fmaf(b4[k], tv, ay[n][ee]);
                        } else if (p == 1) {
                            ax[n][ee] = fmaf(a4[k], tv, ax[n][ee]);
                            az[n][ee] = fmaf(b4[k], tv, az[n][ee]);
                        } else {
                            az[n][ee] = fmaf(a4[k], tv, az[n][ee]);
                            ay[n][ee] = fmaf(b4[k], tv, ay[n][ee]);
                        }
                    }
                }
        }
    }
    gc_transpose(R, af, i, hi, js, c, f);
    if (NEED_J) {
        gc_transpose(R, ax, i, hi, js, c, jx);
        gc_transpose(R, ay, i, hi, js, c, jy);
        gc_transpose(R, az, i, hi, js, c, jz);
    }
    return any;
}

__device__ __forceinline__ bool gather_tex_cp(const float* __restrict__ planes, unsigned tex0, int H, int W, float X,
                                              float Y, float Z, bool valid, int lane, float* T, float (&e)[48]) {
    const int i = lane & 31, hi = lane >> 5, js = lane >> 3, c = lane & 7;
    int* Toff = reinterpret_cast<int*>(T);
    float* Tw = T + 32 * 4;
    float* R = T + GC_PLANE_TABLE_FLOATS;
    const size_t HW = (size_t)H * W;
    bool any = false;
#pragma unroll
    for (int p = 0; p < 3; ++p) {
        Corners cn;
        corners_setup(PLANE_U(p, X, Y, Z), PLANE_V(p, X, Y, Z), H, W, valid, cn);
        any = any || cn.any;
        if (!__any(cn.any)) {
#pragma unroll
            for (int r = 0; r < 16; ++r) e[16 * p + r] = 0.f;
            continue;
        }
        if (hi == 0) {
            const unsigned b = tex0 + (unsigned)((3 + p) * HW);
            const ti32x4 o = {(int)(b + cn.off[0]), (int)(b + cn.off[1]), (int)(b + cn.off[2]), (int)(b + cn.off[3])};
            *reinterpret_cast<ti32x4*>(Toff + i * 4) = o;
        } else {
            const f32x4 w = {cn.w[0], cn.w[1], cn.w[2], cn.w[3]};
            *reinterpret_cast<f32x4*>(Tw + i * 4) = w;
        }
        f32x4 t[4][4], acc[4];
        gc_load16(planes + 4 * c, Toff, js, t);
#pragma unroll
        for (int n = 0; n < 4; ++n) {
            const f32x4 w4 = *reinterpret_cast<const f32x4*>(Tw + (8 * n + js) * 4);
            f32x4 a = {0.f, 0.f, 0.f, 0.f};
#pragma unroll
            for (int k = 0; k < 4; ++k)
#pragma unroll
                for (int ee = 0; ee < 4; ++ee) a[ee] = fmaf(w4[k], t[n][k][ee], a[ee]);
            acc[n] = a;
        }
        gc_transpose(R, acc, i, hi, js, c, &e[16 * p]);
    }
    return any;
}

__device__ __forceinline__ bool gather_tex_c(const float* __restrict__ planes, unsigned tex0, int H, int W, float X,
                                             float Y, float Z, bool valid, int lane, float* T, float (&e)[48],
                                             unsigned* inb = nullptr) {
    const int i = lane & 31, hi = lane >> 5, js = lane >> 3, c = lane & 7;
    int* Toff = reinterpret_cast<int*>(T);
    float* Tw = T + 3 * 32 * 4;
    float* R = T + GC_TABLE_FLOATS(1);
    const size_t HW = (size_t)H * W;
    bool any = false, anyp[3];
#pragma unroll
    for (int p = 0; p < 3; ++p) {
        Corners cn;
        corners_setup(PLANE_U(p, X, Y, Z), PLANE_V(p, X, Y, Z), H, W, valid, cn);
        const unsigned long long inmask = __ballot(cn.any);
        if (inb) {
            if ((threadIdx.x & 63) == 0) *inb += (unsigned)__popcll(inmask & 0xffffffffull);
        }
        anyp[p] = inmask != 0;
        any = any || cn.any;
        if (hi == 0) {
            const unsigned b = tex0 + (unsigned)((3 + p) * HW);
            const ti32x4 o = {(int)(b + cn.off[0]), (int)(b + cn.off[1]), (int)(b + cn.off[2]), (int)(b + cn.off[3])};
            *reinterpret_cast<ti32x4*>(Toff + (p * 32 + i) * 4) = o;
        } else {
            const f32x4 w = {cn.w[0], cn.w[1], cn.w[2], cn.w[3]};
            *reinterpret_cast<f32x4*>(Tw + (p * 32 + i) * 4) = w;
        }
    }
#pragma unroll
    for (int p = 0; p < 3; ++p) {
        if (!anyp[p]) {
#pragma unroll
            for (int r = 0; r < 16; ++r) e[16 * p + r] = 0.f;
            continue;
        }
        f32x4 acc[4];
#pragma unroll
        for (int n = 0; n < 4; ++n) {
            const int sidx = (p * 32 + 8 * n + js) * 4;
            const ti32x4 o4 = *reinterpret_cast<const ti32x4*>(Toff + sidx);
            const f32x4 w4 = *reinterpret_cast<const f32x4*>(Tw + sidx);
            f32x4 a = {0.f, 0.f, 0.f, 0.f};
#pragma unroll
            for (int k = 0; k < 4; ++k) {
                const f32x4 t = *gc_addr(planes, o4[k], 16u * (unsigned)c);
#pragma unroll
                for (int ee = 0; ee < 4; ++ee) a[ee] = fmaf(w4[k], t[ee], a[ee]);
            }
            acc[n] = a;
        }
#pragma unroll
        for (int n = 0; n < 4; ++n) *reinterpret_cast<f32x4*>(R + (8 * n + js) * 36 + 4 * c) = acc[n];
#pragma unroll
        for (int q = 0; q < 4; ++q) {
            const f32x4 v = *reinterpret_cast<const f32x4*>(R + i * 36 + 4 * (hi + 2 * q));
#pragma unroll
            for (int ee = 0; ee < 4; ++ee) e[16 * p + 4 * q + ee] = v[ee];
        }
    }
    return any;
}

__device__ __forceinline__ void geo_corner_coefs(int p, int H, int W, float X, float Y, float Z, bool valid, float sbar,
                                                 float gux, float guy, float guz, float jscale_u, float jscale_v,
                                                 Corners& cn, float (&coef)[4]) {
    corners_setup(PLANE_U(p, X, Y, Z), PLANE_V(p, X, Y, Z), H, W, valid, cn);
    const float gu = (p == 2 ? guz : gux) * jscale_u, gv = (p == 1 ? guz : guy) * jscale_v;
#pragma unroll
    for (int k = 0; k < 4; ++k) coef[k] = fmaf(cn.w[k], sbar, fmaf(cn.du[k], gu, cn.dv[k] * gv));
}

__device__ __forceinline__ bool gather_geo_bwd_c(const float* __restrict__ planes, unsigned tex0, int H, int W, float X,
                                                 float Y, float Z, bool valid, float sbar, float gux, float guy,
                                                 float guz, float jscale_u, float jscale_v, int lane, float* T,
                                                 float (&f)[16], float (&u)[16], bool (&anyp)[3],
                                                 unsigned* inb = nullptr) {
    const int i = lane & 31, hi = lane >> 5, js = lane >> 3, c = lane & 7;
    int* Toff = reinterpret_cast<int*>(T);
    float* Tw = T + 3 * 32 * 4;
    float* Tc = T + 2 * 3 * 32 * 4;
    float* R = T + GC_TABLE_FLOATS(2);
    const size_t HW = (size_t)H * W;
    bool any = false;
#pragma unroll
    for (int p = 0; p < 3; ++p) {
        Corners cn;
        float coef[4];
        geo_corner_coefs(p, H, W, X, Y, Z, valid, sbar, gux, guy, guz, jscale_u, jscale_v, cn, coef);
        const unsigned long long inmask = __ballot(cn.any);
        if (inb) {
            if ((threadIdx.x & 63) == 0) *inb += (unsigned)__popcll(inmask & 0xffffffffull);
        }
        anyp[p] = inmask != 0;
        any = any || cn.any;
        if (hi == 0) {
            const unsigned b = tex0 + (unsigned)(p * HW);
            const ti32x4 o = {(int)(b + cn.off[0]), (int)(b + cn.off[1]), (int)(b + cn.off[2]), (int)(b + cn.off[3])};
            *reinterpret_cast<ti32x4*>(Toff + (p * 32 + i) * 4) = o;
            const f32x4 w = {cn.w[0], cn.w[1], cn.w[2], cn.w[3]};
            *reinterpret_cast<f32x4*>(Tw + (p * 32 + i) * 4) = w;
        } else {
            const f32x4 w = {coef[0], coef[1], coef[2], coef[3]};
            *reinterpret_cast<f32x4*>(Tc + (p * 32 + i) * 4) = w;
        }
    }
    f32x4 af[4], au[4];
#pragma unroll
    for (int n = 0; n < 4; ++n) {
        const f32x4 z = {0.f, 0.f, 0.f, 0.f};
        af[n] = z;
        au[n] = z;
    }
#pragma unroll
    for (int p = 0; p < 3; ++p) {
        if (!anyp[p]) continue;
        f32x4 t[4][4];
#pragma unroll
        for (int n = 0; n < 4; ++n) {
            const ti32x4 o4 = *reinterpret_cast<const ti32x4*>(Toff + (p * 32 + 8 * n + js) * 4);
#pragma unroll
            for (int k = 0; k < 4; ++k)
                t[n][k] = *gc_addr(planes, o4[k], 16u * (unsigned)c);
        }
#pragma unroll
        for (int n = 0; n < 4; ++n) {
            const int sidx = (p * 32 + 8 * n + js) * 4;
            const f32x4 w4 = *reinterpret_cast<const f32x4*>(Tw + sidx);
            const f32x4 c4 = *reinterpret_cast<const f32x4*>(Tc + sidx);
#pragma unroll
            for (int k = 0; k < 4; ++k)
#pragma unroll
                for (int ee = 0; ee < 4; ++ee) {
                    af[n][ee] = fmaf(w4[k], t[n][k][ee], af[n][ee]);
                    au[n][ee] = fmaf(c4[k], t[n][k][ee], au[n][ee]);
                }
        }
    }
#pragma unroll
    for (int n = 0; n < 4; ++n) *reinterpret_cast<f32x4*>(R + (8 * n + js) * 36 + 4 * c) = af[n];
#pragma unroll
    for (int q = 0; q < 4; ++q) {
        const f32x4 v = *reinterpret_cast<const f32x4*>(R + i * 36 + 4 * (hi + 2 * q));
#pragma unroll
        for (int ee = 0; ee < 4; ++ee) f[4 * q + ee] = v[ee];
    }
#pragma unroll
    for (int n = 0; n < 4; ++n) *reinterpret_cast<f32x4*>(R + (8 * n + js) * 36 + 4 * c) = au[n];
#pragma unroll
    for (int q = 0; q < 4; ++q) {
        const f32x4 v = *reinterpret_cast<const f32x4*>(R + i * 36 + 4 * (hi + 2 * q));
#pragma unroll
        for (int ee = 0; ee < 4; ++ee) u[4 * q + ee] = v[ee];
    }
    return any;
}

struct ItemQueue {
    int* ctr;
    long long unit;
    long long nb;
    long long n_local;
    int home;
    int hop;
};
__device__ __forceinline__ ItemQueue item_queue(int* ctr, long long n_blocks, int n_chunks, long long unit) {
    ItemQueue q;
    q.ctr = ctr;
    q.unit = unit;
    const long long n_units = (n_blocks + unit - 1) / unit;
    q.nb = ((n_units + 7) / 8) * unit;
    q.n_local = q.nb * n_chunks;
    q.home = blockIdx.x & 7;
    q.hop = 0;
    return q;
}
__device__ __forceinline__ bool item_pop(ItemQueue& q, int order, int n_chunks, long long& b, int& ck) {
    while (q.hop < 8) {
        const int xcd = (q.home + q.hop) & 7;
        int li = 0;
        if ((threadIdx.x & 63) == 0) li = atomicAdd(q.ctr + xcd, 1);
        li = __builtin_amdgcn_readfirstlane(li);
        if (li < q.n_local) {
            long long bl;
            if (order == 0) {
                ck = (int)(li / q.nb);
                bl = li - (long long)ck * q.nb;
            } else {
                bl = li / n_chunks;
                ck = (int)(li - bl * n_chunks);
            }
            const long long round = bl / q.unit;
            b = (round * 8 + xcd) * q.unit + (bl - round * q.unit);
            return true;
        }
        ++q.hop;
    }
    return false;
}

struct TileGeom {
    long long n_rays;
    int rays_per_view;
    int image_w, image_h;
    int sb, bw, bh;
    int bpr, bpv;
    int n_samples, chunk, n_chunks;
    long long n_blocks;
    long long unit;
    int order;
};

__device__ __forceinline__ long long tile_ray(const TileGeom& g, long long b, int j, bool& rvalid) {
    long long ray;
    float okf = 1.f;
    const int jr = j / g.sb;
    if (g.image_w > 0) {
        const long long view = b / g.bpv;
        const int rem = (int)(b - view * g.bpv);
        const int by = rem / g.bpr, bx = rem - by * g.bpr;
        const int x = bx * g.bw + (jr % g.bw), y = by * g.bh + (jr / g.bw);
        okf = tt_opaque(x < g.image_w ? 1.f : 0.f) * (y < g.image_h ? 1.f : 0.f);
        ray = view * g.rays_per_view + (long long)min(y, g.image_h - 1) * g.image_w + min(x, g.image_w - 1);
    } else {
        ray = b * (32 / g.sb) + jr;
    }
    okf = tt_opaque(okf) * (ray < g.n_rays ? 1.f : 0.f);
    rvalid = okf != 0.f;
    return ray < g.n_rays - 1 ? ray : g.n_rays - 1;
}

__device__ __forceinline__ float sigmoidf_(float x) { return 1.f / (1.f + expf(-x)); }
```

### triplaneturbo_amd/csrc/tt_forward.hip

```cpp
#ifndef TT_MV16_FENCE
#define TT_MV16_FENCE 1
#endif
#include "tt_device.h"
#include "tt_mfma16.h"
#include "tt_alpha.h"
#include "tt_launch.h"

__device__ __forceinline__ void rot_dst(int k3, int y, int x, int H, int W, int& h, int& w) {
    if (k3 == 0) {
        h = x;
        w = y;
    } else if (k3 == 1) {
        h = H - 1 - y;
        w = W - 1 - x;
    } else {
        h = x;
        w = H - 1 - y;
    }
}

template <bool UNPACK>
__global__ __launch_bounds__(256) void k_planes_pack(const float* __restrict__ src, float* __restrict__ dst, int H,
                                                     int W, int n_copies, size_t copy_stride) {
    extern __shared__ float tile[];
    const int y = blockIdx.x, plane = blockIdx.y;
    const int k3 = plane % 3;
    const size_t HW = (size_t)H * W;
    const float* nchw_c = (UNPACK ? dst : src) + (size_t)plane * TT_C * HW;
    float* nchw = const_cast<float*>(nchw_c);
    const float* nhwc_c = (UNPACK ? src : dst) + (size_t)plane * HW * TT_C;
    float* nhwc = const_cast<float*>(nhwc_c);
    const int ws = W + 1;
    if (!UNPACK) {
        for (int e = threadIdx.x; e < TT_C * W; e += blockDim.x) {
            int c = e / W, x = e - c * W;
            tile[c * ws + x] = nchw[(size_t)c * HW + (size_t)y * W + x];
        }
        __syncthreads();
        for (int e = threadIdx.x; e < TT_C * W; e += blockDim.x) {
            int x = e >> 5, c = e & 31, h, w;
            rot_dst(k3, y, x, H, W, h, w);
            nhwc[((size_t)h * W + w) * TT_C + c] = tile[c * ws + x];
        }
    } else {
        for (int e = threadIdx.x; e < TT_C * W; e += blockDim.x) {
            int x = e >> 5, c = e & 31, h, w;
            rot_dst(k3, y, x, H, W, h, w);
            const size_t o = ((size_t)h * W + w) * TT_C + c;
            float acc = nhwc[o];
            for (int k = 1; k < n_copies; ++k) acc += nhwc[o + (size_t)k * copy_stride];
            tile[c * ws + x] = acc;
        }
        __syncthreads();
        for (int e = threadIdx.x; e < TT_C * W; e += blockDim.x) {
            int c = e / W, x = e - c * W;
            nchw[(size_t)c * HW + (size_t)y * W + x] = tile[c * ws + x];
        }
    }
}

__host__ __device__ inline int pack4_row_stride(int W) { return W + (36 - W % 32) % 32; }
template <bool UNPACK>
__global__ __launch_bounds__(256) void k_planes_pack4(const float* __restrict__ src, float* __restrict__ dst, int H,
                                                      int W, int n_copies, size_t copy_stride) {
    extern __shared__ __attribute__((aligned(16))) float tile[];
    const int y = blockIdx.x, plane = blockIdx.y;
    const int k3 = plane % 3;
    const size_t HW = (size_t)H * W;
    const float* nchw_c = (UNPACK ? dst : src) + (size_t)plane * TT_C * HW + (size_t)y * W;
    float* nchw = const_cast<float*>(nchw_c);
    const float* nhwc_c = (UNPACK ? src : dst) + (size_t)plane * HW * TT_C;
    float* nhwc = const_cast<float*>(nhwc_c);
    const int RS = pack4_row_stride(W), W4 = W >> 2;
    const int c_lane = threadIdx.x & 31, x4_0 = threadIdx.x >> 5;
    if (!UNPACK) {
        for (int e4 = threadIdx.x; e4 < TT_C * W4; e4 += 256) {
            const int c = e4 / W4, x4 = e4 - c * W4;
            *reinterpret_cast<f32x4*>(tile + c * RS + 4 * x4) =
                *reinterpret_cast<const f32x4*>(nchw_c + (size_t)c * HW + 4 * x4);
        }
        __syncthreads();
        for (int x4 = x4_0; x4 < W4; x4 += 8) {
            const f32x4 v = *reinterpret_cast<const f32x4*>(tile + c_lane * RS + 4 * x4);
#pragma unroll
            for (int j = 0; j < 4; ++j) {
                int h, w;
                rot_dst(k3, y, 4 * x4 + j, H, W, h, w);
                nhwc[((size_t)h * W + w) * TT_C + c_lane] = v[j];
            }
        }
    } else {
        for (int x4 = x4_0; x4 < W4; x4 += 8) {
            f32x4 v;
#pragma unroll
            for (int j = 0; j < 4; ++j) {
                int h, w;
                rot_dst(k3, y, 4 * x4 + j, H, W, h, w);
                const size_t o = ((size_t)h * W + w) * TT_C + c_lane;
                float acc = nhwc_c[o];
                for (int k = 1; k < n_copies; ++k) acc += nhwc_c[o + (size_t)k * copy_stride];
                v[j] = acc;
            }
            *reinterpret_cast<f32x4*>(tile + c_lane * RS + 4 * x4) = v;
        }
        __syncthreads();
        for (int e4 = threadIdx.x; e4 < TT_C * W4; e4 += 256) {
            const int c = e4 / W4, x4 = e4 - c * W4;
            *reinterpret_cast<f32x4*>(nchw + (size_t)c * HW + 4 * x4) =
                *reinterpret_cast<const f32x4*>(tile + c * RS + 4 * x4);
        }
    }
}

struct DecodeCfg {
    const float* planes;
    unsigned tex0;
    float* T;
    int H, W;
    float radius;
    float ju, jv;
    int dbg;
    TileStats st = {nullptr};
};


template <int PREC>
__device__ __forceinline__ void decode_tex_fwd(const float* L, const DecodeCfg& dc, float X, float Y, float Z,
                                               bool valid, int i, int hi, float (&c)[3]) {
    c[0] = c[1] = c[2] = 0.f;
    float e[48];
    bool any = gather_tex_cp(dc.planes, dc.tex0, dc.H, dc.W, X, Y, Z, valid, 32 * hi + i, dc.T, e);
    if (TT_DBG(dc.dbg, TT_DBG_NO_MLP)) {
        float t = 0.f;
#pragma unroll
        for (int r = 0; r < 48; ++r) t += e[r];
        c[0] = c[1] = c[2] = t;
    } else if (__any(any)) {
        float k1[32], k2[32], u1, u2;
        mvx<PREC, 64, 96, true>(L + OFF_V1, L + LO_V1, e, k1, i, hi, 1.f, &u1);
#pragma unroll
        for (int r = 0; r < 32; ++r) k1[r] = fmaxf(k1[r], 0.f);
        mvx<PREC, 64, 64, true>(L + OFF_V2, L + LO_V2, k1, k2, i, hi, u1, &u2);
#pragma unroll
        for (int r = 0; r < 32; ++r) k2[r] = fmaxf(k2[r], 0.f);
#pragma unroll
        for (int o = 0; o < 3; ++o) c[o] = dot_lds<64>(L + OFF_V3 + 64 * o, k2, hi) * u2;
    }
}

template <bool NEED_N, int PREC>
__device__ __forceinline__ void decode_geo_fwd(const float* L, const DecodeCfg& dc, float X, float Y, float Z,
                                               bool valid, int i, int hi, float& s0, float (&gq)[3]) {
    s0 = 0.f;
    gq[0] = gq[1] = gq[2] = 0.f;
    float f[16], jx[16], jy[16], jz[16];
    bool any = gather_geo_c<NEED_N>(dc.planes, dc.tex0, dc.H, dc.W, X, Y, Z, valid, dc.ju, dc.jv, 32 * hi + i, dc.T, f, jx,
                                 jy, jz, tile_stat_ptr(dc.st, TT_STAT_INBOUNDS));
    if (TT_DBG(dc.dbg, TT_DBG_NO_MLP)) {
        float t = 0.f, tx = 0.f, ty = 0.f, tz = 0.f;
#pragma unroll
        for (int r = 0; r < 16; ++r) {
            t += f[r];
            tx += jx[r];
            ty += jy[r];
            tz += jz[r];
        }
        s0 = t;
        gq[0] = tx;
        gq[1] = ty;
        gq[2] = tz;
    } else if (__any(any)) {
        tile_stat(dc.st, TT_STAT_EXECUTED);
        float h1[32], h2[32], u1, u2;
        mvx<PREC, 64, 32, true>(L + OFF_W1, L + LO_W1, f, h1, i, hi, 1.f, &u1);
#pragma unroll
        for (int r = 0; r < 32; ++r) h1[r] = fmaxf(h1[r], 0.f);
        mvx<PREC, 64, 64, true>(L + OFF_W2, L + LO_W2, h1, h2, i, hi, u1, &u2);
#pragma unroll
        for (int r = 0; r < 32; ++r) h2[r] = fmaxf(h2[r], 0.f);
        s0 = dot_lds<64>(L + OFF_W3, h2, hi) * u2;
        if (NEED_N) {
            float a2[32], a1[32], q[16];
#pragma unroll
            for (int g = 0; g < 8; ++g) {
                f32x4 w3 = *reinterpret_cast<const f32x4*>(L + OFF_W3 + 8 * g + 4 * hi);
#pragma unroll
                for (int e2 = 0; e2 < 4; ++e2) a2[4 * g + e2] = h2[4 * g + e2] > 0.f ? w3[e2] : 0.f;
            }
            float ua1;
            mvtx<PREC, 64, 64, 64, true>(L + OFF_W2, L + LO_W2, 0, a2, a1, i, hi, 1.f, &ua1);
#pragma unroll
            for (int r = 0; r < 32; ++r) a1[r] = h1[r] > 0.f ? a1[r] : 0.f;
            mvtx<PREC, 32, 64, 32>(L + OFF_W1, L + LO_W1, 0, a1, q, i, hi, ua1);
            float sx = 0.f, sy = 0.f, sz = 0.f;
#pragma unroll
            for (int r = 0; r < 16; ++r) {
                sx = fmaf(q[r], jx[r], sx);
                sy = fmaf(q[r], jy[r], sy);
                sz = fmaf(q[r], jz[r], sz);
            }
            gq[0] = sx + __shfl_xor(sx, 32);
            gq[1] = sy + __shfl_xor(sy, 32);
            gq[2] = sz + __shfl_xor(sz, 32);
        }
    }
}

template <bool NEED_N, bool NEED_TEX, int PREC>
__device__ __forceinline__ void decode_fwd(const float* L, const DecodeCfg& dc, float px, float py, float pz,
                                           bool valid, int i, int hi, float& s0, float (&gq)[3], float (&c)[3]) {
    const float X = scale_coord(px, dc.radius), Y = scale_coord(py, dc.radius), Z = scale_coord(pz, dc.radius);
    c[0] = c[1] = c[2] = 0.f;
    if (NEED_TEX) decode_tex_fwd<PREC>(L, dc, X, Y, Z, valid, i, hi, c);
    decode_geo_fwd<NEED_N, PREC>(L, dc, X, Y, Z, valid, i, hi, s0, gq);
}

struct QueryParams {
    const float* packed;
    MlpPtrs w;
    const float* points;
    int n_batch;
    long long n_points;
    int views_per_prompt;
    int H, W;
    float radius, bias_radius;
    float* out_sdf;
    float* out_grad;
    float* out_feat;
};

template <bool NEED_N, bool NEED_TEX, int PREC>
__device__ __forceinline__ void stage_decode_images(float* L, const MlpPtrs& w) {
    stage_weights<PREC, 64, 32>(L + OFF_W1, L + LO_W1, w.w1);
    stage_weights<PREC, 64, 64>(L + OFF_W2, L + LO_W2, w.w2);
    lds_load_matrix(L + OFF_W3, w.w3, 1, 64, 64);
    if (NEED_TEX) {
        stage_weights<PREC, 64, 96>(L + OFF_V1, L + LO_V1, w.v1);
        stage_weights<PREC, 64, 64>(L + OFF_V2, L + LO_V2, w.v2);
        lds_load_matrix(L + OFF_V3, w.v3, 3, 64, 64);
    }
}

#define TT_DR_GEO_SAMPLES 64
#define TT_DR_GEO_MIN_ITEMS 0
#define DECODE_THREADS 512

template <bool NEED_N, bool NEED_TEX, int PREC>
__global__ __launch_bounds__(DECODE_THREADS) void k_query_points(QueryParams p) {
    __shared__ __attribute__((aligned(16))) float L[FwdWFloats<PREC>::value + (DECODE_THREADS / 64) * GC_SCRATCH_FLOATS];
    float* T = L + FwdWFloats<PREC>::value + (threadIdx.x >> 6) * GC_SCRATCH_FLOATS;
    stage_decode_images<NEED_N, NEED_TEX, PREC>(L, p.w);
    __syncthreads();
    const int lane = threadIdx.x & 63, i = lane & 31, hi = lane >> 5;
    const long long tiles_per_batch = (p.n_points + TT_TILE - 1) / TT_TILE;
    const long long n_tiles = tiles_per_batch * p.n_batch;
    const long long wave0 = (long long)blockIdx.x * (blockDim.x >> 6) + (threadIdx.x >> 6);
    const long long n_waves = (long long)gridDim.x * (blockDim.x >> 6);
    const size_t plane_stride = (size_t)6 * p.H * p.W * TT_C;
#pragma nounroll
    for (long long tile = wave0; tile < n_tiles; tile += n_waves) {
        const int b = (int)(tile / tiles_per_batch);
        const long long n = (tile - (long long)b * tiles_per_batch) * TT_TILE + i;
        const bool valid = n < p.n_points;
        const long long idx = (long long)b * p.n_points + (valid ? n : 0);
        DecodeCfg dc;
        dc.planes = p.packed;
        dc.tex0 = (unsigned)((size_t)(b / p.views_per_prompt) * (plane_stride / TT_C));
        dc.T = T;
        dc.H = p.H;
        dc.W = p.W;
        dc.radius = p.radius;
        dc.ju = 0.5f * p.W / p.radius;
        dc.jv = 0.5f * p.H / p.radius;
        dc.dbg = 0;
        const float px = p.points[idx * 3 + 0], py = p.points[idx * 3 + 1], pz = p.points[idx * 3 + 2];
        float s0, gq[3], c[3];
        decode_fwd<NEED_N, NEED_TEX, PREC>(L, dc, px, py, pz, valid, i, hi, s0, gq, c);
        float nrm;
        const float sdf = s0 + sphere_bias(px, py, pz, p.bias_radius, nrm);
        if (valid && hi == 0) {
            if (p.out_sdf) p.out_sdf[idx] = sdf;
            if (NEED_N && p.out_grad) {
                p.out_grad[idx * 3 + 0] = gq[0] + px / nrm;
                p.out_grad[idx * 3 + 1] = gq[1] + py / nrm;
                p.out_grad[idx * 3 + 2] = gq[2] + pz / nrm;
            }
            if (NEED_TEX && p.out_feat) {
                p.out_feat[idx * 3 + 0] = c[0];
                p.out_feat[idx * 3 + 1] = c[1];
                p.out_feat[idx * 3 + 2] = c[2];
            }
        }
    }
}

#define OFF_D1 LDS_GEO_FLOATS
#define OFF_D2 (OFF_D1 + 64 * W1S)
#define OFF_D3 (OFF_D2 + 64 * W2S)
#define LDS_FIELD_FLOATS (OFF_D3 + 3 * 64)
#define LO_FW1 LDS_FIELD_FLOATS
#define LO_FW2 (LO_FW1 + LO16_FLOATS(64, 32))
#define LO_D1 (LO_FW2 + LO16_FLOATS(64, 64))
#define LO_D2 (LO_D1 + LO16_FLOATS(64, 32))
#define LDS_FIELD3_FLOATS (LO_D2 + LO16_FLOATS(64, 64))
template <int PREC>
struct FieldWFloats {
    static constexpr int value = PREC == PREC_S3 ? LDS_FIELD3_FLOATS : LDS_FIELD_FLOATS;
};

struct QueryFieldParams {
    const float* packed;
    MlpPtrs w;
    const float* points;
    int n_batch;
    long long n_points;
    int views_per_prompt;
    int H, W;
    float radius, bias_radius;
    float* out_sdf;
    float* out_def;
};

template <int PREC>
struct QueryFieldWaves {
    static constexpr int value = PREC == PREC_S3 ? 8 : 4;
};
template <int PREC>
__global__ __launch_bounds__(64 * QueryFieldWaves<PREC>::value, PREC == PREC_S3 ? 1 : 2) void k_query_field(QueryFieldParams p) {
    __shared__ __attribute__((aligned(16))) float L[FieldWFloats<PREC>::value + QueryFieldWaves<PREC>::value * GC_SCRATCH_FLOATS];
    float* T = L + FieldWFloats<PREC>::value + (threadIdx.x >> 6) * GC_SCRATCH_FLOATS;
    {
        MlpPtrs w = p.w;
        stage_weights<PREC, 64, 32>(L + OFF_W1, L + LO_FW1, w.w1);
        stage_weights<PREC, 64, 64>(L + OFF_W2, L + LO_FW2, w.w2);
        lds_load_matrix(L + OFF_W3, w.w3, 1, 64, 64);
        stage_weights<PREC, 64, 32>(L + OFF_D1, L + LO_D1, w.v1);
        stage_weights<PREC, 64, 64>(L + OFF_D2, L + LO_D2, w.v2);
        lds_load_matrix(L + OFF_D3, w.v3, 3, 64, 64);
    }
    __syncthreads();
    const int lane = threadIdx.x & 63, i = lane & 31, hi = lane >> 5;
    const long long tiles_per_batch = (p.n_points + TT_TILE - 1) / TT_TILE;
    const long long n_tiles = tiles_per_batch * p.n_batch;
    const long long wave0 = (long long)blockIdx.x * (blockDim.x >> 6) + (threadIdx.x >> 6);
    const long long n_waves = (long long)gridDim.x * (blockDim.x >> 6);
    const size_t plane_stride = (size_t)6 * p.H * p.W * TT_C;
#pragma nounroll
    for (long long tile = wave0; tile < n_tiles; tile += n_waves) {
        const int b = (int)(tile / tiles_per_batch);
        const long long n = (tile - (long long)b * tiles_per_batch) * TT_TILE + i;
        const bool valid = n < p.n_points;
        const long long idx = (long long)b * p.n_points + (valid ? n : 0);
        const unsigned tex0 = (unsigned)((size_t)(b / p.views_per_prompt) * (plane_stride / TT_C));
        const float px = p.points[idx * 3 + 0], py = p.points[idx * 3 + 1], pz = p.points[idx * 3 + 2];
        const float X = scale_coord(px, p.radius), Y = scale_coord(py, p.radius), Z = scale_coord(pz, p.radius);
        float f[16], jx[16], jy[16], jz[16];
        const bool any =
            __any(gather_geo_c<false>(p.packed, tex0, p.H, p.W, X, Y, Z, valid, 0.f, 0.f, lane, T, f, jx, jy, jz));
        float s0 = 0.f, d[3] = {0.f, 0.f, 0.f};
        if (any) {
            float h1[32], h2[32];
            mvx<PREC, 64, 32>(L + OFF_W1, L + LO_FW1, f, h1, i, hi);
#pragma unroll
            for (int r = 0; r < 32; ++r) h1[r] = fmaxf(h1[r], 0.f);
            mvx<PREC, 64, 64>(L + OFF_W2, L + LO_FW2, h1, h2, i, hi);
#pragma unroll
            for (int r = 0; r < 32; ++r) h2[r] = fmaxf(h2[r], 0.f);
            s0 = dot_lds<64>(L + OFF_W3, h2, hi);
            mvx<PREC, 64, 32>(L + OFF_D1, L + LO_D1, f, h1, i, hi);
#pragma unroll
            for (int r = 0; r < 32; ++r) h1[r] = fmaxf(h1[r], 0.f);
            mvx<PREC, 64, 64>(L + OFF_D2, L + LO_D2, h1, h2, i, hi);
#pragma unroll
            for (int r = 0; r < 32; ++r) h2[r] = fmaxf(h2[r], 0.f);
#pragma unroll
            for (int o = 0; o < 3; ++o) d[o] = dot_lds<64>(L + OFF_D3 + 64 * o, h2, hi);
        }
        float nrm;
        const float sdf = s0 + sphere_bias(px, py, pz, p.bias_radius, nrm);
        if (valid && hi == 0) {
            p.out_sdf[idx] = sdf;
            p.out_def[idx * 3 + 0] = d[0];
            p.out_def[idx * 3 + 1] = d[1];
            p.out_def[idx * 3 + 2] = d[2];
        }
    }
}

struct DecodeRaysParams {
    const float* packed;
    MlpPtrs w;
    const float* rays_o;
    const float* rays_d;
    const float* t_starts;
    const float* t_ends;
    tt_render_cfg cfg;
    TileGeom geom;
    long long n_items;
    int* queue;
    float* sdf;
    float* sdf_grad;
    float* features;
};

template <bool NEED_N, bool NEED_TEX, int PREC>
__global__ __launch_bounds__(DECODE_THREADS) void k_decode_rays(DecodeRaysParams p) {
    __shared__ __attribute__((aligned(16))) float L[FwdWFloats<PREC>::value + (DECODE_THREADS / 64) * GC_SCRATCH_FLOATS];
    float* T = L + FwdWFloats<PREC>::value + (threadIdx.x >> 6) * GC_SCRATCH_FLOATS;
    stage_decode_images<NEED_N, NEED_TEX, PREC>(L, p.w);
    __syncthreads();
    const tt_render_cfg& cfg = p.cfg;
    const TileGeom& tg = p.geom;
    const int lane = threadIdx.x & 63, i = lane & 31, hi = lane >> 5;
    const int S = cfg.n_samples;
    ItemQueue iq = item_queue(p.queue, tg.n_blocks, tg.n_chunks, tg.unit);
    const size_t plane_stride = (size_t)6 * cfg.plane_h * cfg.plane_w * TT_C;
    const TileStats st = tile_stats(cfg.stats);

#pragma nounroll
    for (;;) {
        long long b;
        int ck;
        if (!item_pop(iq, tg.order, tg.n_chunks, b, ck)) break;
        if (b >= tg.n_blocks) continue;
        bool ray_ok;
        const long long ray = tile_ray(tg, b, i, ray_ok);
        const float ray_okf = tt_opaque(ray_ok ? 1.f : 0.f);
        const int ks = i % tg.sb;
        const int view = (int)(ray / cfg.rays_per_view);
        DecodeCfg dc;
        dc.st = st;
        dc.planes = p.packed;
        dc.tex0 = (unsigned)((size_t)(view / cfg.views_per_prompt) * (plane_stride / TT_C));
        dc.T = T;
        dc.H = cfg.plane_h;
        dc.W = cfg.plane_w;
        dc.radius = cfg.radius;
        dc.ju = 0.5f * cfg.plane_w / cfg.radius;
        dc.jv = 0.5f * cfg.plane_h / cfg.radius;
        dc.dbg = cfg.flags;
        const float ox = p.rays_o[ray * 3 + 0], oy = p.rays_o[ray * 3 + 1], oz = p.rays_o[ray * 3 + 2];
        const float dx = p.rays_d[ray * 3 + 0], dy = p.rays_d[ray * 3 + 1], dz = p.rays_d[ray * 3 + 2];
        const int s_end = (ck + 1) * tg.chunk < S ? (ck + 1) * tg.chunk : S;
        auto load_t = [&](int sb0_, float& ts_, float& te_) {
            const int si_ = sb0_ + ks;
            const long long sidx_ = ray * S + (si_ < S ? si_ : S - 1);
            ts_ = p.t_starts[sidx_];
            te_ = p.t_ends[sidx_];
        };
        float ts_n, te_n;
        load_t(ck * tg.chunk, ts_n, te_n);
#pragma nounroll
        for (int sb0 = ck * tg.chunk; sb0 < s_end; sb0 += tg.sb) {
            const int si = sb0 + ks;
            const bool rvalid = ray_okf * (si < s_end ? 1.f : 0.f) != 0.f;
            tile_stat(st, TT_STAT_VISITED);
            const long long sidx = ray * S + (si < S ? si : S - 1);
            const float ts = ts_n, te = te_n;
            load_t(sb0 + tg.sb, ts_n, te_n);
            float tm, px, py, pz;
            sample_position(ox, oy, oz, dx, dy, dz, ts, te, tm, px, py, pz);
            float s0, gq[3], c[3];
            decode_fwd<NEED_N, NEED_TEX, PREC>(L, dc, px, py, pz, rvalid, i, hi, s0, gq, c);
            float nrm;
            const float sdf = s0 + sphere_bias(px, py, pz, cfg.sdf_bias_radius, nrm);
            if (rvalid && hi == 0 && !TT_DBG(cfg.flags, TT_DBG_NO_STORE)) {
                p.sdf[sidx] = sdf;
                if (NEED_N) {
                    p.sdf_grad[sidx * 3 + 0] = gq[0] + px / nrm;
                    p.sdf_grad[sidx * 3 + 1] = gq[1] + py / nrm;
                    p.sdf_grad[sidx * 3 + 2] = gq[2] + pz / nrm;
                }
                if (NEED_TEX) {
                    p.features[sidx * 3 + 0] = c[0];
                    p.features[sidx * 3 + 1] = c[1];
                    p.features[sidx * 3 + 2] = c[2];
                }
            }
        }
    }
    tile_stats_flush(st);
}

struct RenderEvalParams {
    const float* packed;
    MlpPtrs w;
    const float* rays_o;
    const float* rays_d;
    const float* t_starts;
    const float* t_ends;
    tt_render_cfg cfg;
    TileGeom geom;
    int* queue;
    float eps_T, eps_w;
    float* opacity;
    float* depth;
    float* rgb_fg;
    float* z_var;
    float* nacc;
    unsigned long long* stats;
};

template <int PREC>
__global__ __launch_bounds__(DECODE_THREADS) void k_render_eval(RenderEvalParams p) {
    __shared__ __attribute__((aligned(16))) float L[FwdWFloats<PREC>::value + (DECODE_THREADS / 64) * GC_SCRATCH_FLOATS];
    float* T = L + FwdWFloats<PREC>::value + (threadIdx.x >> 6) * GC_SCRATCH_FLOATS;
    stage_decode_images<true, true, PREC>(L, p.w);
    __syncthreads();
    const tt_render_cfg& cfg = p.cfg;
    const TileGeom& tg = p.geom;
    const int lane = threadIdx.x & 63, i = lane & 31, hi = lane >> 5;
    const int S = cfg.n_samples;
    const float kstd = load_inv_std(cfg.inv_std_dev, cfg.inv_std);
    ItemQueue iq = item_queue(p.queue, tg.n_blocks, 1, tg.unit);
    const size_t plane_stride = (size_t)6 * cfg.plane_h * cfg.plane_w * TT_C;
    unsigned long long n_geo = 0, n_tex = 0;
#pragma nounroll
    for (;;) {
        long long b;
        int ck;
        if (!item_pop(iq, 1, 1, b, ck)) break;
        if (b >= tg.n_blocks) continue;
        bool ray_ok;
        const long long ray = tile_ray(tg, b, i, ray_ok);
        const float ray_okf = tt_opaque(ray_ok ? 1.f : 0.f);
        const int view = (int)(ray / cfg.rays_per_view);
        DecodeCfg dc;
        dc.planes = p.packed;
        dc.tex0 = (unsigned)((size_t)(view / cfg.views_per_prompt) * (plane_stride / TT_C));
        dc.T = T;
        dc.H = cfg.plane_h;
        dc.W = cfg.plane_w;
        dc.radius = cfg.radius;
        dc.ju = 0.5f * cfg.plane_w / cfg.radius;
        dc.jv = 0.5f * cfg.plane_h / cfg.radius;
        dc.dbg = 0;
        float T = 1.f, acc0 = 0.f, acc1 = 0.f, acc2 = 0.f, acc3 = 0.f, acc4 = 0.f;
        const float hif = (float)hi, lof = 1.f - hif;
#pragma nounroll
        for (int si = 0; si < S; ++si) {
            float tm, px, py, pz, cosv, ux, uy, uz, sdf, dt;
            {
                long long rr = ray;
                asm volatile("" : "+v"(rr));
                const float* ro = p.rays_o + rr * 3;
                const float* rd = p.rays_d + rr * 3;
                const float ts = p.t_starts[rr * S + si], te = p.t_ends[rr * S + si];
                const float ox = ro[0], oy = ro[1], oz = ro[2];
                const float dx = rd[0], dy = rd[1], dz = rd[2];
                sample_position(ox, oy, oz, dx, dy, dz, ts, te, tm, px, py, pz);
            }
            const float X = scale_coord(px, dc.radius), Y = scale_coord(py, dc.radius), Z = scale_coord(pz, dc.radius);
            const float livef = ray_okf * (__builtin_fabsf(T) < p.eps_T ? 0.f : 1.f);
            const bool live = livef != 0.f;
            {
                float s0, gq[3];
                decode_geo_fwd<true, PREC>(L, dc, X, Y, Z, live, i, hi, s0, gq);
                ++n_geo;
                float nrm;
                long long rr = ray;
                asm volatile("" : "+v"(rr));
                const float* ro = p.rays_o + rr * 3;
                const float* rd = p.rays_d + rr * 3;
                const float ts = p.t_starts[rr * S + si], te = p.t_ends[rr * S + si];
                dt = te - ts;
                const float ox = ro[0], oy = ro[1], oz = ro[2];
                const float dx = rd[0], dy = rd[1], dz = rd[2];
                sample_position(ox, oy, oz, dx, dy, dz, ts, te, tm, px, py, pz);
                sdf = s0 + sphere_bias(px, py, pz, cfg.sdf_bias_radius, nrm);
                const float gx = gq[0] + px / nrm, gy = gq[1] + py / nrm, gz = gq[2] + pz / nrm;
                const float gn = fmaxf(sqrtf(gx * gx + gy * gy + gz * gz), 1e-12f);
                const float ign = rcp_(gn);
                ux = gx * ign, uy = gy * ign, uz = gz * ign;
                cosv = dx * ux + dy * uy + dz * uz;
            }
            float alpha = (cfg.flags & TT_R_VOLSDF) ? volsdf_alpha_terms(sdf, dt, kstd).alpha
                                                    : neus_alpha_terms(sdf, cosv, dt, kstd, cfg.cos_anneal_ratio).alpha;
            if (!live) alpha = 0.f;
            const float wgt = alpha * T;
            T *= 1.f - alpha;
            acc0 = fmaf(wgt, lof, acc0);
            acc1 = fmaf(wgt * lof, tm, acc1);
            acc2 = fmaf(wgt * lof * tm, tm, acc2);
            acc3 = fmaf(wgt, hi ? uz : ux, acc3);
            acc4 = fmaf(wgt * lof, uy, acc4);
            const bool want_tex = __builtin_fabsf(wgt) > p.eps_w;
            if (__any(want_tex)) {
                float c[3];
                if constexpr (PREC == PREC_F32) {
                    long long rr = ray;
                    asm volatile("" : "+v"(rr));
                    const float* ro = p.rays_o + rr * 3;
                    const float* rd = p.rays_d + rr * 3;
                    float tm2, qx, qy, qz;
                    sample_position(ro[0], ro[1], ro[2], rd[0], rd[1], rd[2], p.t_starts[rr * S + si], p.t_ends[rr * S + si], tm2,
                                    qx, qy, qz);
                    decode_tex_fwd<PREC>(L, dc, scale_coord(qx, dc.radius), scale_coord(qy, dc.radius),
                                         scale_coord(qz, dc.radius), want_tex, i, hi, c);
                } else {
                    decode_tex_fwd<PREC>(L, dc, X, Y, Z, want_tex, i, hi, c);
                }
                ++n_tex;
                if (want_tex) {
                    const float wh = wgt * hif;
                    acc0 = fmaf(wh, sigmoid_(c[0]) * 1.002f - 0.001f, acc0);
                    acc1 = fmaf(wh, sigmoid_(c[1]) * 1.002f - 0.001f, acc1);
                    acc2 = fmaf(wh, sigmoid_(c[2]) * 1.002f - 0.001f, acc2);
                }
            }
            if (p.eps_T > 0.f && !__any(ray_okf * (__builtin_fabsf(T) < p.eps_T ? 0.f : 1.f) != 0.f)) break;
        }
        if (ray_ok) {
            if (hi == 0) {
                const float op = acc0, dep = acc1, wt2 = acc2;
                p.opacity[ray] = op;
                p.depth[ray] = dep;
                p.z_var[ray] = wt2 - 2.f * dep * dep + dep * dep * op;
                p.nacc[ray * 3 + 0] = acc3;
                p.nacc[ray * 3 + 1] = acc4;
            } else {
                p.rgb_fg[ray * 3 + 0] = acc0;
                p.rgb_fg[ray * 3 + 1] = acc1;
                p.rgb_fg[ray * 3 + 2] = acc2;
                p.nacc[ray * 3 + 2] = acc3;
            }
        }
    }
    if (p.stats && lane == 0) {
        atomicAdd(p.stats + 0, n_geo);
        atomicAdd(p.stats + 1, n_tex);
    }
}

extern "C" int tt_planes_pack(const float* space_cache, float* packed, int32_t n_prompts, int32_t plane_h,
                              int32_t plane_w, void* stream) {
    if (!space_cache || !packed || n_prompts <= 0 || plane_h <= 0 || plane_w <= 0) return TT_ERR_BAD_ARG;
    if (plane_h != plane_w) return TT_ERR_UNSUPPORTED;
    dim3 grid(plane_h, n_prompts * 6);
    if (plane_w % 4 == 0 && ((uintptr_t)space_cache & 15) == 0) {
        size_t lds = (size_t)TT_C * pack4_row_stride(plane_w) * sizeof(float);
        hipLaunchKernelGGL(k_planes_pack4<false>, grid, dim3(256), lds, (hipStream_t)stream, space_cache, packed,
                           plane_h, plane_w, 1, (size_t)0);
    } else {
        size_t lds = (size_t)TT_C * (plane_w + 1) * sizeof(float);
        hipLaunchKernelGGL(k_planes_pack<false>, grid, dim3(256), lds, (hipStream_t)stream, space_cache, packed,
                           plane_h, plane_w, 1, (size_t)0);
    }
    return tt_check_launch();
}

extern "C" int tt_planes_unpack_grad(const float* grad_packed, float* grad_space_cache, int32_t n_prompts,
                                     int32_t plane_h, int32_t plane_w, int32_t n_copies, void* stream) {
    if (!grad_packed || !grad_space_cache || n_prompts <= 0 || plane_h <= 0 || plane_w <= 0 || n_copies <= 0)
        return TT_ERR_BAD_ARG;
    if (plane_h != plane_w) return TT_ERR_UNSUPPORTED;
    dim3 grid(plane_h, n_prompts * 6);
    const size_t copy_stride = (size_t)n_prompts * 6 * plane_h * plane_w * TT_C;
    if (plane_w % 4 == 0 && ((uintptr_t)grad_space_cache & 15) == 0) {
        size_t lds = (size_t)TT_C * pack4_row_stride(plane_w) * sizeof(float);
        hipLaunchKernelGGL(k_planes_pack4<true>, grid, dim3(256), lds, (hipStream_t)stream, grad_packed,
                           grad_space_cache, plane_h, plane_w, n_copies, copy_stride);
    } else {
        size_t lds = (size_t)TT_C * (plane_w + 1) * sizeof(float);
        hipLaunchKernelGGL(k_planes_pack<true>, grid, dim3(256), lds, (hipStream_t)stream, grad_packed,
                           grad_space_cache, plane_h, plane_w, n_copies, copy_stride);
    }
    return tt_check_launch();
}

extern "C" int tt_query_points(const float* packed, const tt_mlp_weights* w, const float* points, int32_t n_batch,
                               int64_t n_points, int32_t n_prompts, int32_t views_per_prompt, int32_t plane_h,
                               int32_t plane_w, float radius, float sdf_bias_radius, int32_t flags, float* out_sdf,
                               float* out_sdf_grad, float* out_features, void* stream) {
    if (!packed || !w || !points) return TT_ERR_BAD_ARG;
    const int st = tt_validate_points(n_batch, n_points, n_prompts, views_per_prompt, plane_h, plane_w, radius, flags);
    if (st != TT_OK) return st;
    const bool need_n = (flags & TT_Q_NORMAL) != 0, need_t = (flags & TT_Q_TEX) != 0;
    if (!w->w1 || !w->w2 || !w->w3 || (need_t && (!w->v1 || !w->v2 || !w->v3))) return TT_ERR_BAD_ARG;
    QueryParams p;
    tt_fill_points(p, packed, w, points, n_batch, n_points, views_per_prompt, plane_h, plane_w, radius);
    p.bias_radius = sdf_bias_radius;
    p.out_sdf = out_sdf;
    p.out_grad = out_sdf_grad;
    p.out_feat = out_features;
    const int cus = tt_num_cus();
    if (cus <= 0) return TT_ERR_DEVICE;
    const dim3 grid = tt_point_blocks(n_points, n_batch, DECODE_THREADS / 64, cus);
    tt_dispatch(tt_prec_of_q(flags), need_n, need_t, [&](auto P, auto N, auto T) {
        hipLaunchKernelGGL((k_query_points<decltype(N)::value, decltype(T)::value, decltype(P)::value>), grid,
                           dim3(DECODE_THREADS), 0, (hipStream_t)stream, p);
    });
    return tt_check_launch();
}

bool tt_planes_too_large(long long n_prompts, int plane_h, int plane_w) {
    return n_prompts * 6 * plane_h * plane_w * TT_C * 4 >= (1LL << 32);
}

int tt_validate_cfg(const tt_render_cfg* cfg) {
    if (!cfg) return TT_ERR_BAD_ARG;
    if (cfg->n_prompts <= 0 || cfg->views_per_prompt <= 0 || cfg->rays_per_view <= 0 || cfg->n_samples <= 0 ||
        cfg->n_rays <= 0)
        return TT_ERR_BAD_ARG;
    if (cfg->n_rays != (int64_t)cfg->n_prompts * cfg->views_per_prompt * cfg->rays_per_view) return TT_ERR_BAD_ARG;
    if (cfg->plane_h <= 0 || cfg->plane_h != cfg->plane_w) return TT_ERR_UNSUPPORTED;
    if (tt_planes_too_large(cfg->n_prompts, cfg->plane_h, cfg->plane_w)) return TT_ERR_UNSUPPORTED;
    if (!(cfg->radius > 0.f) || (!cfg->inv_std_dev && !(cfg->inv_std > 0.f))) return TT_ERR_BAD_ARG;
    if (cfg->flags < 0) return TT_ERR_BAD_ARG;
    {
        const int pbits = cfg->flags & (TT_R_EXACT_F32 | TT_R_SPLIT2 | TT_R_SPLIT3);
        if (pbits & (pbits - 1)) return TT_ERR_BAD_ARG;
    }
    if (cfg->flags & (TT_R_BWD_PAIR | TT_R_WGRAD_F32)) return TT_ERR_UNSUPPORTED;
    if (!(cfg->skip_eps_tex >= 0.f) || !(cfg->skip_eps_geo >= 0.f)) return TT_ERR_BAD_ARG;
    return TT_OK;
}

long long tt_make_geom(const tt_render_cfg* cfg, long long wave_slots, TileGeom* g, int default_order,
                       int steps_per_item, int min_items_per_slot) {
    g->n_rays = cfg->n_rays;
    g->rays_per_view = cfg->rays_per_view;
    g->n_samples = cfg->n_samples;
    g->image_w = 0;
    g->image_h = 0;
    g->bpr = g->bpv = 0;
    int sb = cfg->tile_sb;
#ifdef TT_TUNING
    if (const char* e = getenv("TT_SB")) sb = atoi(e);
#endif
    if (!(sb == 1 || sb == 2 || sb == 4 || sb == 8 || sb == 16 || sb == 32)) sb = 2;
    while (sb > 1 && sb > cfg->n_samples) sb /= 2;
    g->sb = sb;
    static const int BW[6] = {8, 4, 4, 2, 2, 1}, BH[6] = {4, 4, 2, 2, 1, 1};
    int l2 = 0;
    while ((1 << l2) < sb) ++l2;
    g->bw = BW[l2];
    g->bh = BH[l2];
    const int rb = 32 / sb;
    long long n_blocks;
    if (cfg->image_w > 0 && cfg->rays_per_view % cfg->image_w == 0) {
        g->image_w = cfg->image_w;
        g->image_h = cfg->rays_per_view / cfg->image_w;
        g->bpr = (g->image_w + g->bw - 1) / g->bw;
        g->bpv = g->bpr * ((g->image_h + g->bh - 1) / g->bh);
        n_blocks = (cfg->n_rays / cfg->rays_per_view) * g->bpv;
    } else {
        n_blocks = (cfg->n_rays + rb - 1) / rb;
    }
    const int n_steps = (cfg->n_samples + sb - 1) / sb;
    int n_chunks = (n_steps + steps_per_item - 1) / steps_per_item;
    const int min_chunks = (int)(((long long)min_items_per_slot * wave_slots + n_blocks - 1) / n_blocks);
    if (n_chunks < min_chunks) n_chunks = min_chunks;
    if (n_chunks < 1) n_chunks = 1;
    if (n_chunks > n_steps) n_chunks = n_steps;
    if (cfg->tile_chunk > 0) {
        n_chunks = (cfg->n_samples + cfg->tile_chunk - 1) / cfg->tile_chunk;
        if (n_chunks > n_steps) n_chunks = n_steps;
    }
#ifdef TT_TUNING
    if (const char* e = getenv("TT_CHUNK")) {
        int c = atoi(e);
        if (c > 0) n_chunks = (cfg->n_samples + c - 1) / c;
        if (n_chunks > n_steps) n_chunks = n_steps;
    }
#endif
    const int steps_per_chunk = (n_steps + n_chunks - 1) / n_chunks;
    g->chunk = steps_per_chunk * sb;
    g->n_chunks = (cfg->n_samples + g->chunk - 1) / g->chunk;
    g->n_blocks = n_blocks;
    g->unit = n_blocks / 256;
    if (g->unit > 32) g->unit = 32;
#ifdef TT_TUNING
    if (const char* e = getenv("TT_UNIT")) {
        long long u = atoll(e);
        if (u > 0) g->unit = u;
    }
#endif
    if (g->unit < 1) g->unit = 1;
    g->order = default_order;
#ifdef TT_TUNING
    if (const char* e = getenv("TT_ORDER")) g->order = atoi(e) ? 1 : 0;
#endif
    return n_blocks * g->n_chunks;
}

extern "C" int tt_render_fwd(const float* packed, const tt_mlp_weights* w, const float* rays_o, const float* rays_d,
                             const float* t_starts, const float* t_ends, const tt_render_cfg* cfg, float* opacity,
                             float* depth, float* rgb_fg, float* z_variance, float* normal_acc, float* weights,
                             float* trans, float* sdf, float* sdf_grad, float* features, void* stream) {
    int st = tt_validate_cfg(cfg);
    if (st != TT_OK) return st;
    if (!packed || !w || !rays_o || !rays_d || !t_starts || !t_ends || !opacity || !depth || !rgb_fg || !z_variance ||
        !normal_acc || !weights || !trans || !sdf || !sdf_grad || !features)
        return TT_ERR_BAD_ARG;
    if (!w->w1 || !w->w2 || !w->w3 || !w->v1 || !w->v2 || !w->v3) return TT_ERR_BAD_ARG;
    const int cus = tt_num_cus();
    if (cus <= 0) return TT_ERR_DEVICE;
    DecodeRaysParams p;
    tt_fill_rays(p, packed, w, rays_o, rays_d, t_starts, t_ends, *cfg);
    p.cfg.flags |= debug_flags();
    p.sdf = sdf;
    p.sdf_grad = sdf_grad;
    p.features = features;
    hipStream_t s = (hipStream_t)stream;
    st = tt_plan_queue(cfg, (long long)cus * (DECODE_THREADS / 64), s, &p.geom, &p.n_items, &p.queue, 12);
    if (st != TT_OK) return st;
    const dim3 grid((unsigned)tt_persistent_blocks(p.n_items, cus, DECODE_THREADS / 64));
    tt_dispatch_prec(tt_prec_of_r(cfg->flags), [&](auto P) {
        hipLaunchKernelGGL((k_decode_rays<true, true, decltype(P)::value>), grid, dim3(DECODE_THREADS), 0, s, p);
    });
    st = tt_check_launch();
    if (st != TT_OK) return st;
    return tt_launch_march_fwd(rays_d, t_starts, t_ends, cfg, sdf, sdf_grad, features, opacity, depth, rgb_fg,
                               z_variance, normal_acc, weights, trans, s);
}

extern "C" int tt_decode_rays(const float* packed, const tt_mlp_weights* w, const float* rays_o, const float* rays_d,
                              const float* t_starts, const float* t_ends, const tt_render_cfg* cfg, int32_t flags,
                              float* sdf, float* sdf_grad, float* features, void* stream) {
    int st = tt_validate_cfg(cfg);
    if (st != TT_OK) return st;
    const bool need_n = (flags & TT_Q_NORMAL) != 0, need_t = (flags & TT_Q_TEX) != 0;
    if (!packed || !w || !rays_o || !rays_d || !t_starts || !t_ends || !sdf || (need_n && !sdf_grad) ||
        (need_t && !features) || !tt_qflags_ok(flags))
        return TT_ERR_BAD_ARG;
    if (!w->w1 || !w->w2 || !w->w3 || (need_t && (!w->v1 || !w->v2 || !w->v3))) return TT_ERR_BAD_ARG;
    const int cus = tt_num_cus();
    if (cus <= 0) return TT_ERR_DEVICE;
    DecodeRaysParams p;
    tt_fill_rays(p, packed, w, rays_o, rays_d, t_starts, t_ends, *cfg);
    p.sdf = sdf;
    p.sdf_grad = sdf_grad;
    p.features = features;
    hipStream_t s = (hipStream_t)stream;
    const long long slots = (long long)cus * (DECODE_THREADS / 64);
    int steps_per_item = 12, min_items_per_slot = 8;
    if (!need_n && !need_t) {
        const int sb = cfg->tile_sb > 0 ? cfg->tile_sb : 2;
        const int spi = (TT_DR_GEO_SAMPLES + sb - 1) / sb;
        steps_per_item = spi > 1 ? spi : 1;
        min_items_per_slot = TT_DR_GEO_MIN_ITEMS;
    }
    st = tt_plan_queue(cfg, slots, s, &p.geom, &p.n_items, &p.queue, steps_per_item, min_items_per_slot);
    if (st != TT_OK) return st;
    const dim3 grid((unsigned)tt_persistent_blocks(p.n_items, cus, DECODE_THREADS / 64));
    const int prec = (flags & (TT_Q_EXACT_F32 | TT_Q_SPLIT2 | TT_Q_SPLIT3)) ? tt_prec_of_q(flags) : tt_prec_of_r(cfg->flags);
    tt_dispatch(prec, need_n, need_t, [&](auto P, auto N, auto T) {
        hipLaunchKernelGGL((k_decode_rays<decltype(N)::value, decltype(T)::value, decltype(P)::value>), grid,
                           dim3(DECODE_THREADS), 0, s, p);
    });
    return tt_check_launch();
}

extern "C" int tt_query_field(const float* packed, const tt_mlp_weights* w, const float* points, int32_t n_batch,
                              int64_t n_points, int32_t n_prompts, int32_t views_per_prompt, int32_t plane_h,
                              int32_t plane_w, float radius, float sdf_bias_radius, int32_t flags, float* out_sdf,
                              float* out_deformation, void* stream) {
    if (!packed || !w || !points || !out_sdf || !out_deformation) return TT_ERR_BAD_ARG;
    const int st = tt_validate_points(n_batch, n_points, n_prompts, views_per_prompt, plane_h, plane_w, radius, flags);
    if (st != TT_OK) return st;
    if (!w->w1 || !w->w2 || !w->w3 || !w->v1 || !w->v2 || !w->v3) return TT_ERR_BAD_ARG;
    QueryFieldParams p;
    tt_fill_points(p, packed, w, points, n_batch, n_points, views_per_prompt, plane_h, plane_w, radius);
    p.bias_radius = sdf_bias_radius;
    p.out_sdf = out_sdf;
    p.out_def = out_deformation;
    const int cus = tt_num_cus();
    if (cus <= 0) return TT_ERR_DEVICE;
    tt_dispatch_prec(tt_prec_of_q(flags), [&](auto P) {
        constexpr int PREC = decltype(P)::value, waves = QueryFieldWaves<PREC>::value;
        hipLaunchKernelGGL(k_query_field<PREC>, tt_point_blocks(n_points, n_batch, waves, (8LL / waves) * cus),
                           dim3(64 * waves), 0, (hipStream_t)stream, p);
    });
    return tt_check_launch();
}

extern "C" int tt_render_eval(const float* packed, const tt_mlp_weights* w, const float* rays_o, const float* rays_d,
                              const float* t_starts, const float* t_ends, const tt_render_cfg* cfg,
                              float transmittance_eps, float weight_eps, float* opacity, float* depth, float* rgb_fg,
                              float* z_variance, float* normal_acc, uint64_t* stats, void* stream) {
    int st = tt_validate_cfg(cfg);
    if (st != TT_OK) return st;
    if (!packed || !w || !rays_o || !rays_d || !t_starts || !t_ends || !opacity || !depth || !rgb_fg || !z_variance ||
        !normal_acc)
        return TT_ERR_BAD_ARG;
    if (!w->w1 || !w->w2 || !w->w3 || !w->v1 || !w->v2 || !w->v3) return TT_ERR_BAD_ARG;
    if (!(transmittance_eps >= 0.f) || !(weight_eps >= 0.f)) return TT_ERR_BAD_ARG;
    const int cus = tt_num_cus();
    if (cus <= 0) return TT_ERR_DEVICE;
    RenderEvalParams p;
    tt_fill_rays(p, packed, w, rays_o, rays_d, t_starts, t_ends, *cfg);
    p.cfg.tile_sb = 1;
    p.cfg.tile_chunk = cfg->n_samples;
    p.eps_T = transmittance_eps;
    p.eps_w = weight_eps;
    p.opacity = opacity;
    p.depth = depth;
    p.rgb_fg = rgb_fg;
    p.z_var = z_variance;
    p.nacc = normal_acc;
    p.stats = (unsigned long long*)stats;
    hipStream_t s = (hipStream_t)stream;
    long long n_items;
    st = tt_plan_queue(&p.cfg, (long long)cus * (DECODE_THREADS / 64), s, &p.geom, &n_items, &p.queue);
    if (st != TT_OK) return st;
    if (p.geom.n_chunks != 1) return TT_ERR_UNSUPPORTED;
    const dim3 grid((unsigned)tt_persistent_blocks(n_items, cus, DECODE_THREADS / 64));
    tt_dispatch_prec(tt_prec_of_r(cfg->flags), [&](auto P) {
        hipLaunchKernelGGL(k_render_eval<decltype(P)::value>, grid, dim3(DECODE_THREADS), 0, s, p);
    });
    return tt_check_launch();
}
```

### triplaneturbo_amd/csrc/tt_mfma16.h

```cpp
#pragma once
#include "tt_device.h"
#include "tt_host.h"

typedef _Float16 h8_t __attribute__((ext_vector_type(8)));
typedef _Float16 h2_t __attribute__((ext_vector_type(2)));
typedef _Float16 half_t;
typedef float f2_t __attribute__((ext_vector_type(2)));

#define IMG16_FLOATS(ROWS, K) ((ROWS) * ((K) + 4))
#define LO16_FLOATS(ROWS, K) ((ROWS) * ((K) / 2 + 4))


__device__ __forceinline__ h2_t cvt_pk16(float a, float b) {
    unsigned r;
    asm("v_cvt_pk_f16_f32 %0, %1, %2" : "=v"(r) : "v"(a), "v"(b));
    return __builtin_bit_cast(h2_t, r);
}

__device__ __forceinline__ void split_pair(float a, float b, unsigned& hi, unsigned& lo) {
    asm("v_cvt_pk_f16_f32 %0, %2, %3\n\t"
        "v_fma_mix_f32 %2, %2, 1.0, -%0 op_sel_hi:[0,0,1]\n\t"
        "v_fma_mix_f32 %3, %3, 1.0, -%0 op_sel:[0,0,1] op_sel_hi:[0,0,1]\n\t"
        "v_cvt_pk_f16_f32 %1, %2, %3"
        : "=&v"(hi), "=v"(lo), "+v"(a), "+v"(b));
}
__device__ __forceinline__ void split_pair(float a, float b, h2_t& hi, h2_t& lo) {
    unsigned h, l;
    split_pair(a, b, h, l);
    hi = __builtin_bit_cast(h2_t, h);
    lo = __builtin_bit_cast(h2_t, l);
}

__device__ __forceinline__ void split_pair3(float a, float b, unsigned& hi, unsigned& mid, unsigned& lo) {
    asm("v_cvt_pk_f16_f32 %0, %3, %4\n\t"
        "v_fma_mix_f32 %3, %3, 1.0, -%0 op_sel_hi:[0,0,1]\n\t"
        "v_fma_mix_f32 %4, %4, 1.0, -%0 op_sel:[0,0,1] op_sel_hi:[0,0,1]\n\t"
        "v_cvt_pk_f16_f32 %1, %3, %4\n\t"
        "v_fma_mix_f32 %3, %3, 1.0, -%1 op_sel_hi:[0,0,1]\n\t"
        "v_fma_mix_f32 %4, %4, 1.0, -%1 op_sel:[0,0,1] op_sel_hi:[0,0,1]\n\t"
        "v_cvt_pk_f16_f32 %2, %3, %4"
        : "=&v"(hi), "=&v"(mid), "=&v"(lo), "+v"(a), "+v"(b));
}
__device__ __forceinline__ void split_pair3(float a, float b, h2_t& hi, h2_t& mid, h2_t& lo) {
    unsigned h, m, l;
    split_pair3(a, b, h, m, l);
    hi = __builtin_bit_cast(h2_t, h);
    mid = __builtin_bit_cast(h2_t, m);
    lo = __builtin_bit_cast(h2_t, l);
}

__device__ __forceinline__ void split16(float v, half_t& hi, half_t& lo) {
    const h2_t p = cvt_pk16(v, 0.f);
    hi = p.x;
    const h2_t q = cvt_pk16(v - (float)hi, 0.f);
    lo = q.x;
}
__device__ __forceinline__ void split16_3(float v, half_t& hi, half_t& mid, half_t& lo) {
    split16(v, hi, mid);
    const h2_t q = cvt_pk16((v - (float)hi) - (float)mid, 0.f);
    lo = q.x;
}

template <int ROWS, int K, bool TRANSPOSED, int NT = 2>
__device__ __forceinline__ void stage_image16(float* dst_f, const float* __restrict__ src, int ld, float* lo_f = nullptr) {
    half_t* dst = reinterpret_cast<half_t*>(dst_f);
    half_t* dlo = reinterpret_cast<half_t*>(lo_f);
    constexpr int RS = 2 * K + 8, RSL = K + 8;
    unsigned* slot = reinterpret_cast<unsigned*>(dst_f + K);
    if (threadIdx.x == 0) *slot = 0u;
    __syncthreads();
    unsigned mb = 0u;
    for (int e = threadIdx.x; e < ROWS * K; e += blockDim.x) {
        const unsigned b = __builtin_bit_cast(unsigned, src[e]) & 0x7fffffffu;
        mb = b > mb ? b : mb;
    }
    atomicMax(slot, mb);
    __syncthreads();
    int E = (int)(*slot >> 23);
    E = E < 16 ? 16 : (E > 240 ? 240 : E);
    const float sc = __builtin_bit_cast(float, (unsigned)(268 - E) << 23);
    const float un = __builtin_bit_cast(float, (unsigned)(E - 14) << 23);
    __syncthreads();
    for (int e = threadIdx.x; e < ROWS * K; e += blockDim.x) {
        const int R = e / K, c = e - R * K;
        const float v = (TRANSPOSED ? src[(size_t)c * ld + R] : src[(size_t)R * ld + c]) * sc;
        half_t hi, lo, l3 = (half_t)0.f;
        if (NT == 3)
            split16_3(v, hi, lo, l3);
        else
            split16(v, hi, lo);
        const int s = c >> 4, w = c & 15;
        const int h = (w >> 2) & 1, j = (w & 3) + 4 * (w >> 3);
        half_t* p = dst + (size_t)R * RS + (size_t)(4 * s + h) * 8 + j;
        p[0] = hi;
        p[16] = lo;
        if (NT == 3) {
            const int hf = c >= K / 2 ? 1 : 0, s2 = (c - hf * (K / 2)) >> 4;
            dlo[(size_t)R * RSL + (size_t)(4 * s2 + h) * 8 + j + 16 * hf] = l3;
        }
    }
    for (int R = threadIdx.x; R < ROWS; R += blockDim.x) dst_f[(size_t)R * (K + 4) + K] = un;
}

#ifndef TT_MV16_FENCE
#define TT_MV16_FENCE 0
#endif

template <int MT, int NT>
__device__ __forceinline__ void mfma_terms(f32x16 (&acc)[MT], const h8_t (&a0)[MT], const h8_t (&a1)[MT],
                                           const h8_t (&a2)[MT], const h8_t& b0, const h8_t& b1, const h8_t& b2) {
    if constexpr (NT == 3) {
#pragma unroll
        for (int m = 0; m < MT; ++m) acc[m] = __builtin_amdgcn_mfma_f32_32x32x16_f16(a0[m], b2, acc[m], 0, 0, 0);
#pragma unroll
        for (int m = 0; m < MT; ++m) acc[m] = __builtin_amdgcn_mfma_f32_32x32x16_f16(a2[m], b0, acc[m], 0, 0, 0);
#pragma unroll
        for (int m = 0; m < MT; ++m) acc[m] = __builtin_amdgcn_mfma_f32_32x32x16_f16(a1[m], b1, acc[m], 0, 0, 0);
#pragma unroll
        for (int m = 0; m < MT; ++m) acc[m] = __builtin_amdgcn_mfma_f32_32x32x16_f16(a0[m], b1, acc[m], 0, 0, 0);
#pragma unroll
        for (int m = 0; m < MT; ++m) acc[m] = __builtin_amdgcn_mfma_f32_32x32x16_f16(a1[m], b0, acc[m], 0, 0, 0);
#pragma unroll
        for (int m = 0; m < MT; ++m) acc[m] = __builtin_amdgcn_mfma_f32_32x32x16_f16(a0[m], b0, acc[m], 0, 0, 0);
    } else {
#pragma unroll
        for (int m = 0; m < MT; ++m) acc[m] = __builtin_amdgcn_mfma_f32_32x32x16_f16(a0[m], b0, acc[m], 0, 0, 0);
#pragma unroll
        for (int m = 0; m < MT; ++m) acc[m] = __builtin_amdgcn_mfma_f32_32x32x16_f16(a0[m], b1, acc[m], 0, 0, 0);
#pragma unroll
        for (int m = 0; m < MT; ++m) acc[m] = __builtin_amdgcn_mfma_f32_32x32x16_f16(a1[m], b0, acc[m], 0, 0, 0);
    }
}
template <int NT, bool SCALED>
__device__ __forceinline__ void split_bfrag(float x0, float x1, float sc, int d, h8_t& b0, h8_t& b1, h8_t& b2) {
    const f2_t ab = {x0, x1};
    const f2_t as = SCALED ? ab * sc : ab;
    h2_t p, q, r;
    if constexpr (NT == 3)
        split_pair3(as.x, as.y, p, q, r);
    else
        split_pair(as.x, as.y, p, q);
    b0[2 * d] = p.x;
    b0[2 * d + 1] = p.y;
    b1[2 * d] = q.x;
    b1[2 * d + 1] = q.y;
    if constexpr (NT == 3) {
        b2[2 * d] = r.x;
        b2[2 * d + 1] = r.y;
    }
}
template <int K>
__device__ __forceinline__ h8_t lo_frag(const half_t* lrow, int m, int s) {
    constexpr int RSL = K + 8, KH = K / 32;
    return *reinterpret_cast<const h8_t*>(lrow + (size_t)(32 * m) * RSL + 32 * (s % KH) + 16 * (s / KH));
}

template <int NOUT, int NIN, bool SCALED = true, bool RAW = false, int NT = 2>
__device__ __forceinline__ void mv16(const float* img_f, const float (&x)[NIN / 2], float (&y)[NOUT / 2], int i,
                                     int hi, float xf = 1.f, float* yf = nullptr, const float* lo_f = nullptr) {
    constexpr int MT = NOUT / 32, KS = NIN / 16, RS = 2 * NIN + 8;
    const half_t* row = reinterpret_cast<const half_t*>(img_f) + (size_t)i * RS + 8 * hi;
    const half_t* lrow = reinterpret_cast<const half_t*>(lo_f) + (size_t)i * (NIN + 8) + 8 * hi;
    const float wun = img_f[(size_t)i * (NIN + 4) + NIN];
    float sc = 1.f, un = wun;
    if (SCALED) {
        float m = 0.f;
#pragma unroll
        for (int r = 0; r < NIN / 2; ++r) m = fmaxf(m, __builtin_fabsf(x[r]));
        m = fmaxf(m, __shfl_xor(m, 32));
        int E = (int)(__builtin_bit_cast(unsigned, m) >> 23);
        E = E < 16 ? 16 : (E > 240 ? 240 : E);
        sc = __builtin_bit_cast(float, (unsigned)(268 - E) << 23);
        un = wun * __builtin_bit_cast(float, (unsigned)(E - 14) << 23);
    }
    un *= xf;
    f32x16 acc[MT];
#pragma unroll
    for (int m = 0; m < MT; ++m)
        acc[m] = f32x16{0.f, 0.f, 0.f, 0.f, 0.f, 0.f, 0.f, 0.f, 0.f, 0.f, 0.f, 0.f, 0.f, 0.f, 0.f, 0.f};
    if (TT_MV16_FENCE) __builtin_amdgcn_sched_barrier(0);
#pragma unroll
    for (int s = 0; s < KS; ++s) {
        h8_t bh, bl, bt;
#pragma unroll
        for (int j = 0; j < 4; ++j) split_bfrag<NT, SCALED>(x[8 * s + 2 * j], x[8 * s + 2 * j + 1], sc, j, bh, bl, bt);
        h8_t ah[MT], al[MT], at[MT];
#pragma unroll
        for (int m = 0; m < MT; ++m) {
            const half_t* a = row + (size_t)(32 * m) * RS + 32 * s;
            ah[m] = *reinterpret_cast<const h8_t*>(a);
            al[m] = *reinterpret_cast<const h8_t*>(a + 16);
            if constexpr (NT == 3) at[m] = lo_frag<NIN>(lrow, m, s);
        }
        mfma_terms<MT, NT>(acc, ah, al, at, bh, bl, bt);
    }
    if (RAW) *yf = un;
#pragma unroll
    for (int m = 0; m < MT; ++m)
#pragma unroll
        for (int k = 0; k < 16; ++k) y[16 * m + k] = RAW ? acc[m][k] : acc[m][k] * un;
}

#define PAIR_SEQ 0
#define PAIR_TR 1
template <int PAIR>
__device__ __forceinline__ constexpr int pair_reg(int t, int which) {
    return PAIR == PAIR_SEQ ? 2 * t + which : 8 * (t >> 2) + ((t & 3) >> 1) + 4 * (t & 1) + 2 * which;
}
template <int N, int PAIR = PAIR_SEQ, int NT = 2>
struct Split16 {
    unsigned h[N / 4], l[N / 4];
    unsigned t[NT == 3 ? N / 4 : 1];
};
template <int N, int PAIR, int NT>
__device__ __forceinline__ void split16_vec(const float (&x)[N / 2], float sc, Split16<N, PAIR, NT>& o) {
#pragma unroll
    for (int t = 0; t < N / 4; ++t) {
        const f2_t ab = {x[pair_reg<PAIR>(t, 0)], x[pair_reg<PAIR>(t, 1)]};
        const f2_t as = ab * sc;
        if constexpr (NT == 3)
            split_pair3(as.x, as.y, o.h[t], o.l[t], o.t[t]);
        else
            split_pair(as.x, as.y, o.h[t], o.l[t]);
    }
}
template <int NOUT, int NIN, bool RAW = false, int NT = 2>
__device__ __forceinline__ void mv16_pre(const float* img_f, const Split16<NIN, PAIR_SEQ, NT>& x, float un_x,
                                         float (&y)[NOUT / 2], int i, int hi, float* yf = nullptr,
                                         const float* lo_f = nullptr) {
    constexpr int MT = NOUT / 32, KS = NIN / 16, RS = 2 * NIN + 8;
    const half_t* row = reinterpret_cast<const half_t*>(img_f) + (size_t)i * RS + 8 * hi;
    const half_t* lrow = reinterpret_cast<const half_t*>(lo_f) + (size_t)i * (NIN + 8) + 8 * hi;
    const float un = img_f[(size_t)i * (NIN + 4) + NIN] * un_x;
    f32x16 acc[MT];
#pragma unroll
    for (int m = 0; m < MT; ++m)
        acc[m] = f32x16{0.f, 0.f, 0.f, 0.f, 0.f, 0.f, 0.f, 0.f, 0.f, 0.f, 0.f, 0.f, 0.f, 0.f, 0.f, 0.f};
    typedef unsigned u4_t __attribute__((ext_vector_type(4)));
#pragma unroll
    for (int s = 0; s < KS; ++s) {
        const h8_t bh = __builtin_bit_cast(h8_t, u4_t{x.h[4 * s], x.h[4 * s + 1], x.h[4 * s + 2], x.h[4 * s + 3]});
        const h8_t bl = __builtin_bit_cast(h8_t, u4_t{x.l[4 * s], x.l[4 * s + 1], x.l[4 * s + 2], x.l[4 * s + 3]});
        h8_t bt;
        if constexpr (NT == 3)
            bt = __builtin_bit_cast(h8_t, u4_t{x.t[4 * s], x.t[4 * s + 1], x.t[4 * s + 2], x.t[4 * s + 3]});
        h8_t ah[MT], al[MT], at[MT];
#pragma unroll
        for (int m = 0; m < MT; ++m) {
            const half_t* a = row + (size_t)(32 * m) * RS + 32 * s;
            ah[m] = *reinterpret_cast<const h8_t*>(a);
            al[m] = *reinterpret_cast<const h8_t*>(a + 16);
            if constexpr (NT == 3) at[m] = lo_frag<NIN>(lrow, m, s);
        }
        mfma_terms<MT, NT>(acc, ah, al, at, bh, bl, bt);
    }
    if (RAW) *yf = un;
#pragma unroll
    for (int m = 0; m < MT; ++m)
#pragma unroll
        for (int k = 0; k < 16; ++k) y[16 * m + k] = RAW ? acc[m][k] : acc[m][k] * un;
}

typedef short sv4_t __attribute__((__vector_size__(4 * sizeof(short))));
typedef __attribute__((address_space(3))) sv4_t lds_sv4_t;

template <int KM>
__device__ __forceinline__ const lds_sv4_t* tr_lane_base(const float* img_f, int col0, int lane) {
    constexpr int RS = 2 * KM + 8;
    const int L = lane & 15, g1 = (lane >> 4) & 1, hh = lane >> 5, j = L >> 2, q = L & 3;
    const int r1 = 2 * (j & 1) + 8 * (j >> 1) + 4 * hh;
    const int off = r1 * RS + 32 * ((col0 >> 4) + g1) + 8 * (q & 1) + 4 * (q >> 1);
    return (const lds_sv4_t*)(reinterpret_cast<const half_t*>(img_f) + off);
}
template <int KM>
__device__ __forceinline__ h8_t tr_frag(const lds_sv4_t* base, int ks, int m, int term) {
    constexpr int RS = 2 * KM + 8;
    const int off4 = (16 * ks * RS + 64 * m + 16 * term) / 4;
    const sv4_t a = __builtin_amdgcn_ds_read_tr16_b64_v4i16(const_cast<lds_sv4_t*>(base) + off4);
    const sv4_t b = __builtin_amdgcn_ds_read_tr16_b64_v4i16(const_cast<lds_sv4_t*>(base) + off4 + RS / 4);
    typedef short sv8_t __attribute__((__vector_size__(8 * sizeof(short))));
    const sv8_t ab = __builtin_shufflevector(a, b, 0, 1, 2, 3, 4, 5, 6, 7);
    return __builtin_bit_cast(h8_t, ab);
}

template <int KM>
__device__ __forceinline__ const lds_sv4_t* tr_lane_base_lo(const float* lo_f, int col0, int m, int lane) {
    constexpr int RSL = KM + 8, KH = KM / 32;
    const int L = lane & 15, g1 = (lane >> 4) & 1, hh = lane >> 5, j = L >> 2, q = L & 3;
    const int r1 = 2 * (j & 1) + 8 * (j >> 1) + 4 * hh;
    const int cb0 = (col0 >> 4) + 2 * m, cb1 = cb0 + 1;
    const int b0 = 32 * (cb0 % KH) + 16 * (cb0 / KH), b1 = 32 * (cb1 % KH) + 16 * (cb1 / KH);
    const int off = r1 * RSL + (g1 ? b1 : b0) + 8 * (q & 1) + 4 * (q >> 1);
    return (const lds_sv4_t*)(reinterpret_cast<const half_t*>(lo_f) + off);
}
template <int KM>
__device__ __forceinline__ h8_t tr_frag_lo(const lds_sv4_t* base_m, int ks) {
    constexpr int RSL = KM + 8;
    const int off4 = (16 * ks * RSL) / 4;
    const sv4_t a = __builtin_amdgcn_ds_read_tr16_b64_v4i16(const_cast<lds_sv4_t*>(base_m) + off4);
    const sv4_t b = __builtin_amdgcn_ds_read_tr16_b64_v4i16(const_cast<lds_sv4_t*>(base_m) + off4 + RSL / 4);
    typedef short sv8_t __attribute__((__vector_size__(8 * sizeof(short))));
    const sv8_t ab = __builtin_shufflevector(a, b, 0, 1, 2, 3, 4, 5, 6, 7);
    return __builtin_bit_cast(h8_t, ab);
}

template <int NOUT, int NIN, int KM, bool SCALED = true, bool RAW = false, int NT = 2>
__device__ __forceinline__ void mv16t(const float* img_f, int col0, const float (&x)[NIN / 2], float (&y)[NOUT / 2],
                                      int lane, float xf = 1.f, float* yf = nullptr, const float* lo_f = nullptr) {
    constexpr int MT = NOUT / 32, KS = NIN / 16;
    const lds_sv4_t* base = tr_lane_base<KM>(img_f, col0, lane);
    const lds_sv4_t* base_lo[MT];
    if constexpr (NT == 3) {
#pragma unroll
        for (int m = 0; m < MT; ++m) base_lo[m] = tr_lane_base_lo<KM>(lo_f, col0, m, lane);
    }
    const float wun = img_f[KM];
    float sc = 1.f, un = wun;
    if (SCALED) {
        float m = 0.f;
#pragma unroll
        for (int r = 0; r < NIN / 2; ++r) m = fmaxf(m, __builtin_fabsf(x[r]));
        m = fmaxf(m, __shfl_xor(m, 32));
        int E = (int)(__builtin_bit_cast(unsigned, m) >> 23);
        E = E < 16 ? 16 : (E > 240 ? 240 : E);
        sc = __builtin_bit_cast(float, (unsigned)(268 - E) << 23);
        un = wun * __builtin_bit_cast(float, (unsigned)(E - 14) << 23);
    }
    un *= xf;
    f32x16 acc[MT];
#pragma unroll
    for (int m = 0; m < MT; ++m)
        acc[m] = f32x16{0.f, 0.f, 0.f, 0.f, 0.f, 0.f, 0.f, 0.f, 0.f, 0.f, 0.f, 0.f, 0.f, 0.f, 0.f, 0.f};
    if (TT_MV16_FENCE) __builtin_amdgcn_sched_barrier(0);
#pragma unroll
    for (int s = 0; s < KS; ++s) {
        h8_t bh, bl, bt;
#pragma unroll
        for (int d = 0; d < 4; ++d)
            split_bfrag<NT, SCALED>(x[8 * s + pair_reg<PAIR_TR>(d, 0)], x[8 * s + pair_reg<PAIR_TR>(d, 1)], sc, d, bh, bl, bt);
        h8_t ah[MT], al[MT], at[MT];
#pragma unroll
        for (int m = 0; m < MT; ++m) {
            ah[m] = tr_frag<KM>(base, s, m, 0);
            al[m] = tr_frag<KM>(base, s, m, 1);
            if constexpr (NT == 3) at[m] = tr_frag_lo<KM>(base_lo[m], s);
        }
        mfma_terms<MT, NT>(acc, ah, al, at, bh, bl, bt);
    }
    if (RAW) *yf = un;
#pragma unroll
    for (int m = 0; m < MT; ++m)
#pragma unroll
        for (int k = 0; k < 16; ++k) y[16 * m + k] = RAW ? acc[m][k] : acc[m][k] * un;
}

template <int PREC>
struct PrecNT {
    static constexpr int value = PREC == PREC_S3 ? 3 : 2;
};
template <int PREC, int ROWS, int K>
__device__ __forceinline__ void stage_weights(float* dst_f, float* lo_f, const float* __restrict__ src) {
    if constexpr (PREC == PREC_F32) {
        lds_load_matrix(dst_f, src, ROWS, K, K + 4);
    } else {
        stage_image16<ROWS, K, false, PrecNT<PREC>::value>(dst_f, src, K, lo_f);
    }
}

template <int PREC, int ROWS_SRC, int K_SRC>
__device__ __forceinline__ void stage_weights_t(float* dst_f, float* lo_f, const float* __restrict__ src) {
    if constexpr (PREC != PREC_F32) stage_image16<K_SRC, ROWS_SRC, true, PrecNT<PREC>::value>(dst_f, src, K_SRC, lo_f);
}

template <int PREC, int NOUT, int NIN, bool RAW = false>
__device__ __forceinline__ void mvx(const float* img, const float* lo, const float (&x)[NIN / 2], float (&y)[NOUT / 2],
                                    int i, int hi, float xf = 1.f, float* yf = nullptr) {
    if constexpr (PREC == PREC_F32) {
        mv_fwd<NOUT, NIN>(img, x, y, i, hi);
        if (RAW) *yf = 1.f;
    } else {
        mv16<NOUT, NIN, true, RAW, PrecNT<PREC>::value>(img, x, y, i, hi, xf, yf, lo);
    }
}
template <int PREC, int NOUT, int NIN, int KM, bool RAW = false>
__device__ __forceinline__ void mvtx_copy(const float* img_t, const float* lo_t, const float* img,
                                          const float (&x)[NIN / 2], float (&y)[NOUT / 2], int i, int hi, float xf = 1.f,
                                          float* yf = nullptr) {
    if constexpr (PREC == PREC_F32) {
        mv_bwd<NOUT, NIN, KM + 4>(img, x, y, i, hi);
        if (RAW) *yf = 1.f;
    } else {
        mv16<NOUT, NIN, true, RAW, PrecNT<PREC>::value>(img_t, x, y, i, hi, xf, yf, lo_t);
    }
}
template <int PREC, int NOUT, int NIN, int KM, bool RAW = false>
__device__ __forceinline__ void mvtx(const float* img, const float* lo, int col0, const float (&x)[NIN / 2],
                                     float (&y)[NOUT / 2], int i, int hi, float xf = 1.f, float* yf = nullptr) {
    if constexpr (PREC == PREC_F32) {
        mv_bwd<NOUT, NIN, KM + 4>(img + col0, x, y, i, hi);
        if (RAW) *yf = 1.f;
    } else {
        mv16t<NOUT, NIN, KM, true, RAW, PrecNT<PREC>::value>(img, col0, x, y, 32 * hi + i, xf, yf, lo);
    }
}

#define LO_W1 LDS_W_FLOATS
#define LO_W2 (LO_W1 + LO16_FLOATS(64, 32))
#define LO_V1 (LO_W2 + LO16_FLOATS(64, 64))
#define LO_V2 (LO_V1 + LO16_FLOATS(64, 96))
#define LDS_W3P_FLOATS (LO_V2 + LO16_FLOATS(64, 64))
template <int PREC>
struct FwdWFloats {
    static constexpr int value = PREC == PREC_S3 ? LDS_W3P_FLOATS : LDS_W_FLOATS;
};
#define TT_PREC_OF(exact, split2) ((exact) ? PREC_F32 : ((split2) ? PREC_S2 : PREC_S3))
```

Before: 7.280 million.

## Specialize MLP and scatter paths for waves touching a single triplane

Gather routines now report a per-wave bitmask of which planes had in-bounds samples. When only one plane is live, the first texture layer's matvec runs only over that plane's 32 input columns, and the gradient scatter handles a single plane instead of looping over all three, in forward, geo backward and tex backward. Some scale factors and the wave index are also forced wave-uniform with readfirstlane so they stay in scalar registers. This adds code paths and register pressure, and any gain depends on how often waves are single-plane.

New measurement: 7.439 million, median of 6. 2.2% higher.

```diff
diff --git a/triplaneturbo_amd/csrc/tt_backward.hip b/triplaneturbo_amd/csrc/tt_backward.hip
--- a/triplaneturbo_amd/csrc/tt_backward.hip
+++ b/triplaneturbo_amd/csrc/tt_backward.hip
@@ -143,13 +143,14 @@
             const float X = scale_coord(px, cfg.radius), Y = scale_coord(py, cfg.radius),
                         Z = scale_coord(pz, cfg.radius);
             float f[16], u[16];
-            bool anyp[3];
+            unsigned pmask;
             const bool any = __any(gather_geo_bwd_c(p.packed, (unsigned)(pofs / TT_C), H, W, X, Y, Z, rvalid, sbar, gbx,
-                                                    gby, gbz, ju, jv, lane, Xs, f, u, anyp,
+                                                    gby, gbz, ju, jv, lane, Xs, f, u, pmask,
                                                     tile_stat_ptr(st, TT_STAT_INBOUNDS)));
             TT_PHASE(1);
             if (!any) continue;
-            tile_stat(st, TT_STAT_EXECUTED);
+            const bool one = single_plane(pmask);
+            tile_stat_executed(st, one);
             float h1[32], h2[32], a2[32], a1[32], q[16], u1, u2;
             mvx<PREC, 64, 32, true>(L + OFF_W1, L + GLO_W1, f, h1, i, hi, 1.f, &u1);
 #pragma unroll
@@ -230,8 +231,7 @@
                     float* Qs = Xs + SCATTER_M_FLOATS;
                     TT_PHASE(9);
                     const int tex0 = (int)(pofs / TT_C);
-                    scatter_planes<EXACT>(grad_out, grad_bytes, Qs, Xs, tags, Qs + 32 * 33, i, hi,
-                                          [&](int pl, PlaneRefs& refs) {
+                    auto prep = [&](int pl, PlaneRefs& refs) {
                         Corners c;
                         float coef[4];
                         geo_corner_coefs(pl, H, W, X, Y, Z, rvalid, sbar, gbx, gby, gbz, ju, jv, c, coef);
@@ -241,11 +241,17 @@
                         refs = plane_refs<!EXACT>(coef, aoff, c.hs, hi);
 #pragma unroll
                         for (int r = 0; r < 16; ++r) Qs[i * 33 + LIDX(r, hi)] = q[r] * refs.qs;
-                    }
-#ifdef TT_TUNING
-                    , ph_acc + 14
-#endif
-                    );
+                    };
+#ifdef TT_TUNING
+                    unsigned long long* const sc_st = ph_acc + 14;
+#else
+                    unsigned long long* const sc_st = nullptr;
+#endif
+                    if (one)
+                        scatter_one_plane<EXACT>(grad_out, grad_bytes, Qs, Xs, tags, Qs + 32 * 33, i, hi,
+                                                 single_plane_index(pmask), prep, sc_st);
+                    else
+                        scatter_planes<EXACT>(grad_out, grad_bytes, Qs, Xs, tags, Qs + 32 * 33, i, hi, prep, sc_st);
                     TT_PHASE(10);
                 }
             }
diff --git a/triplaneturbo_amd/csrc/tt_backward_common.h b/triplaneturbo_amd/csrc/tt_backward_common.h
--- a/triplaneturbo_amd/csrc/tt_backward_common.h
+++ b/triplaneturbo_amd/csrc/tt_backward_common.h
@@ -608,6 +608,53 @@
     }
 }
 
+template <bool EXACT, class Prep>
+__device__ __forceinline__ void scatter_one_plane(float* __restrict__ grad, unsigned grad_bytes, const float* Qs, float* M,
+                                                  int* tags, float* Ls, int i, int hi, int pl, Prep&& prep,
+                                                  unsigned long long* st = nullptr) {
+    const __amdgpu_buffer_rsrc_t grsrc = __builtin_amdgcn_make_buffer_rsrc(grad, 0, (int)grad_bytes, 0x00020000);
+    const unsigned lane_b = 4u * (unsigned)i;
+    const int lane = i + 32 * hi;
+    int* const dummy = tags + i;
+    int* const htab = reinterpret_cast<int*>(Ls + 256);
+    int* const ct = htab + SC2_HT;
+    int* const cdump = ct + 2 * SC2_CT;
+    typename std::conditional<EXACT, ScA32, ScA16>::type A;
+    typename std::conditional<EXACT, ScB32, ScB16>::type B;
+    {
+        const i32x4 e4 = {-1, -1, -1, -1};
+        *reinterpret_cast<i32x4*>(htab + 4 * lane) = e4;
+    }
+    PlaneRefs rc;
+    prep(pl, rc);
+    const Sc2State sc = sc2_claim_rank(rc, htab, ct, cdump, dummy, lane, st);
+    scatter_lost(rc, sc.l0, sc.l1, Qs, Ls, grsrc, i, hi);
+    m_store<EXACT>(M, sc2_row_a(sc.rx0), i, rc.c0);
+    m_store<EXACT>(M, sc2_row_a(sc.rx1), i, rc.c1);
+    const bool pass_b = sc.n > 64;
+    f32x16 acc0, acc1;
+    sc2_load_a(M, i, hi, sc.n, A);
+    m_zero<EXACT>(M, sc2_row_a(sc.rx0), i);
+    m_zero<EXACT>(M, sc2_row_a(sc.rx1), i);
+    if (pass_b) {
+        m_store<EXACT>(M, sc2_row_b(sc.rx0), i, rc.c0);
+        m_store<EXACT>(M, sc2_row_b(sc.rx1), i, rc.c1);
+    }
+    sc2_load_b(Qs, i, hi, B);
+    sc2_split_b(B);
+    sc2_gemm(A, B, sc.n, acc0, acc1);
+    if (pass_b) {
+        sc2_flush(acc0, acc1, ct, 64, grsrc, lane_b, hi);
+        sc2_load_a(M, i, hi, sc.n - 64, A);
+        m_zero<EXACT>(M, sc2_row_b(sc.rx0), i);
+        m_zero<EXACT>(M, sc2_row_b(sc.rx1), i);
+        sc2_gemm(A, B, sc.n - 64, acc0, acc1);
+        sc2_flush(acc0, acc1, ct + 64, sc.n - 64, grsrc, lane_b, hi);
+    } else {
+        sc2_flush(acc0, acc1, ct, sc.n, grsrc, lane_b, hi);
+    }
+}
+
 struct BwdTexParams {
     const float* packed;
     MlpPtrs w;
diff --git a/triplaneturbo_amd/csrc/tt_backward_tex.hip b/triplaneturbo_amd/csrc/tt_backward_tex.hip
--- a/triplaneturbo_amd/csrc/tt_backward_tex.hip
+++ b/triplaneturbo_amd/csrc/tt_backward_tex.hip
@@ -1,6 +1,9 @@
 #include "tt_backward_common.h"
 
 #define TEX_SCRATCH_FLOATS (128 * XS)
+__device__ __forceinline__ float uniform_f(float v) {
+    return __builtin_bit_cast(float, __builtin_amdgcn_readfirstlane(__builtin_bit_cast(int, v)));
+}
 
 template <int PREC, bool WG16, bool STATS = false>
 __global__ __launch_bounds__(256, 1) void k_decode_bwd_tex(BwdTexParams p) {
@@ -43,8 +46,11 @@
         sK2B = wg16_scale(K2Bw * CBmax);
         sKB1 = wg16_scale(KB1w * CBmax);
     }
+    sE = uniform_f(sE), sK1 = uniform_f(sK1), sK2B = uniform_f(sK2B), sKB1 = uniform_f(sKB1);
+    const float uE = uniform_f(1.f / sE), uK1 = uniform_f(1.f / sK1);
     const TileGeom& tg = p.geom;
-    const int lane = threadIdx.x & 63, i = lane & 31, hi = lane >> 5, wave_in_blk = threadIdx.x >> 6;
+    const int lane = threadIdx.x & 63, i = lane & 31, hi = lane >> 5,
+              wave_in_blk = __builtin_amdgcn_readfirstlane((int)(threadIdx.x >> 6));
     float* Xs = Lt + WF + wave_in_blk * (TEX_SCRATCH_FLOATS + SCATTER_TAG_INTS);
     float* Ys = Xs + 32 * XS;
     int* tags = reinterpret_cast<int*>(Xs + 128 * XS);
@@ -146,12 +152,15 @@
         sample_position(ox, oy, oz, dx, dy, dz, in.ts, in.te, tm, px, py, pz);
         const float X = scale_coord(px, cfg.radius), Y = scale_coord(py, cfg.radius), Z = scale_coord(pz, cfg.radius);
         float e[48];
+        unsigned pmask;
         const bool any =
-            __any(gather_tex_c(p.packed, (unsigned)(pofs / TT_C), H, W, X, Y, Z, valid, lane, Xs, e,
+            __any(gather_tex_c(p.packed, (unsigned)(pofs / TT_C), H, W, X, Y, Z, valid, lane, Xs, e, pmask,
                                tile_stat_ptr(st, TT_STAT_INBOUNDS)));
         TT_PHASE(1);
         if (!any) continue;
-        tile_stat(st, TT_STAT_EXECUTED);
+        const bool one = single_plane(pmask);
+        const int pl1 = single_plane_index(pmask);
+        tile_stat_executed(st, one);
         const bool region = cfg.flags >= 0;
         const bool region_w = WG16 ? true : region;
         const bool do_wgrad = region_w && !TT_DBG(cfg.flags, TT_DBG_NO_WGRAD);
@@ -161,11 +170,23 @@
             split16_vec<96, PAIR_SEQ, NT>(e, sE, es);
             if (do_wgrad) stage_rows16_pre<96>(Ys, es, i, hi);
             TT_PHASE(2);
-            mv16_pre<64, 96, false, NT>(Lt + TV1, es, 1.f / sE, k1, i, hi, nullptr, Lt + TLO_V1);
+            if (one) {
+                Split16<32, PAIR_SEQ, NT> e1s;
+                live_split32(es, e1s);
+                mv16_pre_ks<64, 96, 2, NT>(Lt + TV1, e1s, 2 * pl1, uE, k1, i, hi, Lt + TLO_V1);
+            } else {
+                mv16_pre<64, 96, false, NT>(Lt + TV1, es, uE, k1, i, hi, nullptr, Lt + TLO_V1);
+            }
         } else {
             if (do_wgrad) stage_rows<96>(Ys, e, i, hi);
             TT_PHASE(2);
-            mvx<PREC, 64, 96>(Lt + TV1, Lt + TLO_V1, e, k1, i, hi);
+            if (one) {
+                float e1[16];
+                live_block16(e, e1);
+                mvx_plane<PREC, 64, 96>(Lt + TV1, Lt + TLO_V1, e1, pl1, k1, i, hi);
+            } else {
+                mvx<PREC, 64, 96>(Lt + TV1, Lt + TLO_V1, e, k1, i, hi);
+            }
         }
 #pragma unroll
         for (int r = 0; r < 32; ++r) k1[r] = fmaxf(k1[r], 0.f);
@@ -173,7 +194,7 @@
         Split16<64, PAIR_SEQ, NT> k1s;
         if (WG16) {
             split16_vec<64, PAIR_SEQ, NT>(k1, sK1, k1s);
-            mv16_pre<64, 64, false, NT>(Lt + TV2, k1s, 1.f / sK1, k2, i, hi, nullptr, Lt + TLO_V2);
+            mv16_pre<64, 64, false, NT>(Lt + TV2, k1s, uK1, k2, i, hi, nullptr, Lt + TLO_V2);
         } else {
             mvx<PREC, 64, 64>(Lt + TV2, Lt + TLO_V2, k1, k2, i, hi);
         }
@@ -257,13 +278,35 @@
             float* M = Xs;
             float* Es = Xs + (EXACT ? 65 * XS : SCATTER_M_FLOATS);
             scatter_clear<EXACT>(M, lane);
+            const int tex0 = (int)(pofs / TT_C);
             float eb[48];
             if constexpr (COPIES)
                 mvtx_copy<PREC, 96, 64, 96>(Lt + TV1T, nullptr, Lt + TV1, kb1, eb, i, hi);
             else
                 mvtx<PREC, 96, 64, 96>(Lt + TV1, Lt + TLO_V1, 0, kb1, eb, i, hi);
             TT_PHASE(9);
-            const int tex0 = (int)(pofs / TT_C);
+            if (one) {
+                float eb1[16];
+#pragma unroll
+                for (int r = 0; r < 16; ++r) eb1[r] = pl1 == 0 ? eb[r] : (pl1 == 1 ? eb[16 + r] : eb[32 + r]);
+                scatter_one_plane<EXACT>(grad_out, grad_bytes, Es, M, tags, Es + 32 * 33, i, hi, pl1,
+                                         [&](int pl, PlaneRefs& refs) {
+                    Corners c;
+                    corners_setup(PLANE_U(pl, X, Y, Z), PLANE_V(pl, X, Y, Z), H, W, valid, c);
+                    int aoff[4];
+#pragma unroll
+                    for (int q4 = 0; q4 < 4; ++q4) aoff[q4] = tex0 + (int)((3 + pl) * HW) + c.off[q4];
+                    refs = plane_refs<!EXACT>(c.w, aoff, c.hs, hi);
+#pragma unroll
+                    for (int r = 0; r < 16; ++r) Es[i * 33 + LIDX(r, hi)] = eb1[r] * refs.qs;
+                }
+#ifdef TT_TUNING
+                , scat_st
+#endif
+                );
+                TT_PHASE(10);
+                continue;
+            }
             scatter_planes<EXACT>(grad_out, grad_bytes, Es, M, tags, Es + 32 * 33, i, hi, [&](int pl, PlaneRefs& refs) {
                 Corners c;
                 corners_setup(PLANE_U(pl, X, Y, Z), PLANE_V(pl, X, Y, Z), H, W, valid, c);
diff --git a/triplaneturbo_amd/csrc/tt_device.h b/triplaneturbo_amd/csrc/tt_device.h
--- a/triplaneturbo_amd/csrc/tt_device.h
+++ b/triplaneturbo_amd/csrc/tt_device.h
@@ -92,6 +92,32 @@
                 acc[m] = __builtin_amdgcn_mfma_f32_32x32x2f32(a_cur[m][k], x[4 * g + k], acc[m], 0, 0, 0);
 #pragma unroll
         for (int m = 0; m < MT; ++m) a_cur[m] = a_nxt[m];
+    }
+#pragma unroll
+    for (int m = 0; m < MT; ++m)
+#pragma unroll
+        for (int k = 0; k < 16; ++k) y[16 * m + k] = acc[m][k];
+}
+
+template <int NOUT, int NIN, int NG>
+__device__ __forceinline__ void mv_fwd_cols(const float* Wl, const float (&x)[4 * NG], int g0, float (&y)[NOUT / 2], int i,
+                                            int hi) {
+    constexpr int MT = NOUT / 32;
+    f32x16 acc[MT];
+    const float* row = Wl + i * (NIN + 4) + 4 * hi + 8 * g0;
+#pragma unroll
+    for (int m = 0; m < MT; ++m)
+        acc[m] = f32x16{0.f, 0.f, 0.f, 0.f, 0.f, 0.f, 0.f, 0.f, 0.f, 0.f, 0.f, 0.f, 0.f, 0.f, 0.f, 0.f};
+#pragma unroll
+    for (int g = 0; g < NG; ++g) {
+        f32x4 a[MT];
+#pragma unroll
+        for (int m = 0; m < MT; ++m) a[m] = *reinterpret_cast<const f32x4*>(row + 32 * m * (NIN + 4) + 8 * g);
+#pragma unroll
+        for (int k = 0; k < 4; ++k)
+#pragma unroll
+            for (int m = 0; m < MT; ++m)
+                acc[m] = __builtin_amdgcn_mfma_f32_32x32x2f32(a[m][k], x[4 * g + k], acc[m], 0, 0, 0);
     }
 #pragma unroll
     for (int m = 0; m < MT; ++m)
@@ -319,7 +345,7 @@
     unsigned long long* p;
     unsigned* w;
 };
-enum { TT_STAT_VISITED = 0, TT_STAT_EXECUTED = 1, TT_STAT_INBOUNDS = 2 };
+enum { TT_STAT_VISITED = 0, TT_STAT_EXECUTED = 1, TT_STAT_INBOUNDS = 2, TT_STAT_SINGLE = 3 };
 __device__ __forceinline__ TileStats tile_stats(uint64_t* stats64) {
     TileStats st = {nullptr, nullptr};
     __shared__ unsigned tt_stat_slots[16 * 4];
@@ -335,12 +361,29 @@
         if ((threadIdx.x & 63) == 0) st.w[which] += v;
     }
 }
+__device__ __forceinline__ void tile_stat_executed(const TileStats& st, bool single) {
+    if (st.p) {
+        if ((threadIdx.x & 63) == 0) {
+            st.w[TT_STAT_EXECUTED] += 1u;
+            st.w[TT_STAT_SINGLE] += single ? 1u : 0u;
+        }
+    }
+}
 __device__ __forceinline__ unsigned* tile_stat_ptr(const TileStats& st, int which) { return st.p ? st.w + which : nullptr; }
 __device__ __forceinline__ void tile_stats_flush(const TileStats& st) {
     if (st.p) {
         const int l = threadIdx.x & 63;
-        if (l < 3) atomicAdd(st.p + l, (unsigned long long)st.w[l]);
-    }
+        if (l < 4) atomicAdd(st.p + l, (unsigned long long)st.w[l]);
+    }
+}
+
+__device__ __forceinline__ bool single_plane(unsigned pmask) { return pmask != 0u && (pmask & (pmask - 1u)) == 0u; }
+__device__ __forceinline__ int single_plane_index(unsigned pmask) { return __builtin_ctz(pmask | 8u); }
+__device__ __forceinline__ void live_block16(const float (&e)[48], float (&e1)[16]) {
+#pragma unroll
+    for (int r = 0; r < 16; ++r)
+        e1[r] = __builtin_bit_cast(float, __builtin_bit_cast(unsigned, e[r]) | __builtin_bit_cast(unsigned, e[16 + r]) |
+                                              __builtin_bit_cast(unsigned, e[32 + r]));
 }
 
 typedef int ti32x4 __attribute__((ext_vector_type(4)));
@@ -379,7 +422,7 @@
 __device__ __forceinline__ bool gather_geo_c(const float* __restrict__ planes, unsigned tex0, int H, int W, float X,
                                              float Y, float Z, bool valid, float jscale_u, float jscale_v, int lane,
                                              float* T, float (&f)[16], float (&jx)[16], float (&jy)[16],
-                                             float (&jz)[16], unsigned* inb = nullptr) {
+                                             float (&jz)[16], unsigned& pmask, unsigned* inb = nullptr) {
     const int i = lane & 31, hi = lane >> 5, js = lane >> 3, c = lane & 7;
     int* Toff = reinterpret_cast<int*>(T);
     float* Tw = T + 32 * 4;
@@ -390,6 +433,7 @@
     const f32x4 z4 = {0.f, 0.f, 0.f, 0.f};
     f32x4 af[4] = {z4, z4, z4, z4}, ax[4] = {z4, z4, z4, z4}, ay[4] = {z4, z4, z4, z4}, az[4] = {z4, z4, z4, z4};
     bool any = false;
+    pmask = 0u;
 #pragma unroll
     for (int p = 0; p < 3; ++p) {
         Corners cn;
@@ -400,6 +444,7 @@
             if ((threadIdx.x & 63) == 0) *inb += (unsigned)__popcll(inmask & 0xffffffffull);
         }
         if (inmask == 0) continue;
+        pmask |= 1u << p;
         if (hi == 0) {
             const unsigned b = tex0 + (unsigned)(p * HW);
             const ti32x4 o = {(int)(b + cn.off[0]), (int)(b + cn.off[1]), (int)(b + cn.off[2]), (int)(b + cn.off[3])};
@@ -453,13 +498,15 @@
 }
 
 __device__ __forceinline__ bool gather_tex_cp(const float* __restrict__ planes, unsigned tex0, int H, int W, float X,
-                                              float Y, float Z, bool valid, int lane, float* T, float (&e)[48]) {
+                                              float Y, float Z, bool valid, int lane, float* T, float (&e)[48],
+                                              unsigned& pmask) {
     const int i = lane & 31, hi = lane >> 5, js = lane >> 3, c = lane & 7;
     int* Toff = reinterpret_cast<int*>(T);
     float* Tw = T + 32 * 4;
     float* R = T + GC_PLANE_TABLE_FLOATS;
     const size_t HW = (size_t)H * W;
     bool any = false;
+    pmask = 0u;
 #pragma unroll
     for (int p = 0; p < 3; ++p) {
         Corners cn;
@@ -470,6 +517,7 @@
             for (int r = 0; r < 16; ++r) e[16 * p + r] = 0.f;
             continue;
         }
+        pmask |= 1u << p;
         if (hi == 0) {
             const unsigned b = tex0 + (unsigned)((3 + p) * HW);
             const ti32x4 o = {(int)(b + cn.off[0]), (int)(b + cn.off[1]), (int)(b + cn.off[2]), (int)(b + cn.off[3])};
@@ -497,13 +545,14 @@
 
 __device__ __forceinline__ bool gather_tex_c(const float* __restrict__ planes, unsigned tex0, int H, int W, float X,
                                              float Y, float Z, bool valid, int lane, float* T, float (&e)[48],
-                                             unsigned* inb = nullptr) {
+                                             unsigned& pmask, unsigned* inb = nullptr) {
     const int i = lane & 31, hi = lane >> 5, js = lane >> 3, c = lane & 7;
     int* Toff = reinterpret_cast<int*>(T);
     float* Tw = T + 3 * 32 * 4;
     float* R = T + GC_TABLE_FLOATS(1);
     const size_t HW = (size_t)H * W;
     bool any = false, anyp[3];
+    pmask = 0u;
 #pragma unroll
     for (int p = 0; p < 3; ++p) {
         Corners cn;
@@ -513,6 +562,7 @@
             if ((threadIdx.x & 63) == 0) *inb += (unsigned)__popcll(inmask & 0xffffffffull);
         }
         anyp[p] = inmask != 0;
+        pmask |= anyp[p] ? 1u << p : 0u;
         any = any || cn.any;
         if (hi == 0) {
             const unsigned b = tex0 + (unsigned)((3 + p) * HW);
@@ -569,7 +619,7 @@
 __device__ __forceinline__ bool gather_geo_bwd_c(const float* __restrict__ planes, unsigned tex0, int H, int W, float X,
                                                  float Y, float Z, bool valid, float sbar, float gux, float guy,
                                                  float guz, float jscale_u, float jscale_v, int lane, float* T,
-                                                 float (&f)[16], float (&u)[16], bool (&anyp)[3],
+                                                 float (&f)[16], float (&u)[16], unsigned& pmask,
                                                  unsigned* inb = nullptr) {
     const int i = lane & 31, hi = lane >> 5, js = lane >> 3, c = lane & 7;
     int* Toff = reinterpret_cast<int*>(T);
@@ -577,7 +627,8 @@
     float* Tc = T + 2 * 3 * 32 * 4;
     float* R = T + GC_TABLE_FLOATS(2);
     const size_t HW = (size_t)H * W;
-    bool any = false;
+    bool any = false, anyp[3];
+    pmask = 0u;
 #pragma unroll
     for (int p = 0; p < 3; ++p) {
         Corners cn;
@@ -588,6 +639,7 @@
             if ((threadIdx.x & 63) == 0) *inb += (unsigned)__popcll(inmask & 0xffffffffull);
         }
         anyp[p] = inmask != 0;
+        pmask |= anyp[p] ? 1u << p : 0u;
         any = any || cn.any;
         if (hi == 0) {
             const unsigned b = tex0 + (unsigned)(p * HW);
diff --git a/triplaneturbo_amd/csrc/tt_forward.hip b/triplaneturbo_amd/csrc/tt_forward.hip
--- a/triplaneturbo_amd/csrc/tt_forward.hip
+++ b/triplaneturbo_amd/csrc/tt_forward.hip
@@ -129,7 +129,8 @@
                                                bool valid, int i, int hi, float (&c)[3]) {
     c[0] = c[1] = c[2] = 0.f;
     float e[48];
-    bool any = gather_tex_cp(dc.planes, dc.tex0, dc.H, dc.W, X, Y, Z, valid, 32 * hi + i, dc.T, e);
+    unsigned pmask;
+    bool any = gather_tex_cp(dc.planes, dc.tex0, dc.H, dc.W, X, Y, Z, valid, 32 * hi + i, dc.T, e, pmask);
     if (TT_DBG(dc.dbg, TT_DBG_NO_MLP)) {
         float t = 0.f;
 #pragma unroll
@@ -137,7 +138,14 @@
         c[0] = c[1] = c[2] = t;
     } else if (__any(any)) {
         float k1[32], k2[32], u1, u2;
-        mvx<PREC, 64, 96, true>(L + OFF_V1, L + LO_V1, e, k1, i, hi, 1.f, &u1);
+        if (single_plane(pmask)) {
+            tile_stat(dc.st, TT_STAT_SINGLE);
+            float e1[16];
+            live_block16(e, e1);
+            mvx_plane<PREC, 64, 96, true>(L + OFF_V1, L + LO_V1, e1, single_plane_index(pmask), k1, i, hi, &u1);
+        } else {
+            mvx<PREC, 64, 96, true>(L + OFF_V1, L + LO_V1, e, k1, i, hi, 1.f, &u1);
+        }
 #pragma unroll
         for (int r = 0; r < 32; ++r) k1[r] = fmaxf(k1[r], 0.f);
         mvx<PREC, 64, 64, true>(L + OFF_V2, L + LO_V2, k1, k2, i, hi, u1, &u2);
@@ -154,8 +162,9 @@
     s0 = 0.f;
     gq[0] = gq[1] = gq[2] = 0.f;
     float f[16], jx[16], jy[16], jz[16];
+    unsigned pmask;
     bool any = gather_geo_c<NEED_N>(dc.planes, dc.tex0, dc.H, dc.W, X, Y, Z, valid, dc.ju, dc.jv, 32 * hi + i, dc.T, f, jx,
-                                 jy, jz, tile_stat_ptr(dc.st, TT_STAT_INBOUNDS));
+                                 jy, jz, pmask, tile_stat_ptr(dc.st, TT_STAT_INBOUNDS));
     if (TT_DBG(dc.dbg, TT_DBG_NO_MLP)) {
         float t = 0.f, tx = 0.f, ty = 0.f, tz = 0.f;
 #pragma unroll
@@ -355,8 +364,9 @@
         const float px = p.points[idx * 3 + 0], py = p.points[idx * 3 + 1], pz = p.points[idx * 3 + 2];
         const float X = scale_coord(px, p.radius), Y = scale_coord(py, p.radius), Z = scale_coord(pz, p.radius);
         float f[16], jx[16], jy[16], jz[16];
+        unsigned pmask;
         const bool any =
-            __any(gather_geo_c<false>(p.packed, tex0, p.H, p.W, X, Y, Z, valid, 0.f, 0.f, lane, T, f, jx, jy, jz));
+            __any(gather_geo_c<false>(p.packed, tex0, p.H, p.W, X, Y, Z, valid, 0.f, 0.f, lane, T, f, jx, jy, jz, pmask));
         float s0 = 0.f, d[3] = {0.f, 0.f, 0.f};
         if (any) {
             float h1[32], h2[32];
diff --git a/triplaneturbo_amd/csrc/tt_mfma16.h b/triplaneturbo_amd/csrc/tt_mfma16.h
--- a/triplaneturbo_amd/csrc/tt_mfma16.h
+++ b/triplaneturbo_amd/csrc/tt_mfma16.h
@@ -224,6 +224,15 @@
             split_pair(as.x, as.y, o.h[t], o.l[t]);
     }
 }
+template <int NT>
+__device__ __forceinline__ void live_split32(const Split16<96, PAIR_SEQ, NT>& x, Split16<32, PAIR_SEQ, NT>& o) {
+#pragma unroll
+    for (int t = 0; t < 8; ++t) {
+        o.h[t] = x.h[t] | x.h[8 + t] | x.h[16 + t];
+        o.l[t] = x.l[t] | x.l[8 + t] | x.l[16 + t];
+        if constexpr (NT == 3) o.t[t] = x.t[t] | x.t[8 + t] | x.t[16 + t];
+    }
+}
 template <int NOUT, int NIN, bool RAW = false, int NT = 2>
 __device__ __forceinline__ void mv16_pre(const float* img_f, const Split16<NIN, PAIR_SEQ, NT>& x, float un_x,
                                          float (&y)[NOUT / 2], int i, int hi, float* yf = nullptr,
@@ -259,6 +268,88 @@
     for (int m = 0; m < MT; ++m)
 #pragma unroll
         for (int k = 0; k < 16; ++k) y[16 * m + k] = RAW ? acc[m][k] : acc[m][k] * un;
+}
+
+template <int K>
+__device__ __forceinline__ h8_t lo_frag_rt(const half_t* lrow, int m, int s) {
+    constexpr int RSL = K + 8, KH = K / 32;
+    const int t = s >= KH ? 1 : 0;
+    return *reinterpret_cast<const h8_t*>(lrow + (size_t)(32 * m) * RSL + 32 * (s - KH * t) + 16 * t);
+}
+template <int NOUT, int NIN, int NK, bool RAW = false, int NT = 2>
+__device__ __forceinline__ void mv16_ks(const float* img_f, const float (&x)[8 * NK], int s0, float (&y)[NOUT / 2], int i,
+                                        int hi, float xf = 1.f, float* yf = nullptr, const float* lo_f = nullptr) {
+    constexpr int MT = NOUT / 32, RS = 2 * NIN + 8;
+    const half_t* row = reinterpret_cast<const half_t*>(img_f) + (size_t)i * RS + 8 * hi + 32 * s0;
+    const half_t* lrow = reinterpret_cast<const half_t*>(lo_f) + (size_t)i * (NIN + 8) + 8 * hi;
+    const float wun = img_f[(size_t)i * (NIN + 4) + NIN];
+    float m = 0.f;
+#pragma unroll
+    for (int r = 0; r < 8 * NK; ++r) m = fmaxf(m, __builtin_fabsf(x[r]));
+    m = fmaxf(m, __shfl_xor(m, 32));
+    int E = (int)(__builtin_bit_cast(unsigned, m) >> 23);
+    E = E < 16 ? 16 : (E > 240 ? 240 : E);
+    const float sc = __builtin_bit_cast(float, (unsigned)(268 - E) << 23);
+    const float un = wun * __builtin_bit_cast(float, (unsigned)(E - 14) << 23) * xf;
+    f32x16 acc[MT];
+#pragma unroll
+    for (int mm = 0; mm < MT; ++mm)
+        acc[mm] = f32x16{0.f, 0.f, 0.f, 0.f, 0.f, 0.f, 0.f, 0.f, 0.f, 0.f, 0.f, 0.f, 0.f, 0.f, 0.f, 0.f};
+    if (TT_MV16_FENCE) __builtin_amdgcn_sched_barrier(0);
+#pragma unroll
+    for (int s = 0; s < NK; ++s) {
+        h8_t bh, bl, bt;
+#pragma unroll
+        for (int j = 0; j < 4; ++j) split_bfrag<NT, true>(x[8 * s + 2 * j], x[8 * s + 2 * j + 1], sc, j, bh, bl, bt);
+        h8_t ah[MT], al[MT], at[MT];
+#pragma unroll
+        for (int mm = 0; mm < MT; ++mm) {
+            const half_t* a = row + (size_t)(32 * mm) * RS + 32 * s;
+            ah[mm] = *reinterpret_cast<const h8_t*>(a);
+            al[mm] = *reinterpret_cast<const h8_t*>(a + 16);
+            if constexpr (NT == 3) at[mm] = lo_frag_rt<NIN>(lrow, mm, s0 + s);
+        }
+        mfma_terms<MT, NT>(acc, ah, al, at, bh, bl, bt);
+    }
+    if (RAW) *yf = un;
+#pragma unroll
+    for (int mm = 0; mm < MT; ++mm)
+#pragma unroll
+        for (int k = 0; k < 16; ++k) y[16 * mm + k] = RAW ? acc[mm][k] : acc[mm][k] * un;
+}
+template <int NOUT, int NIN, int NK, int NT = 2>
+__device__ __forceinline__ void mv16_pre_ks(const float* img_f, const Split16<16 * NK, PAIR_SEQ, NT>& x, int s0, float un_x,
+                                            float (&y)[NOUT / 2], int i, int hi, const float* lo_f = nullptr) {
+    constexpr int MT = NOUT / 32, RS = 2 * NIN + 8;
+    const half_t* row = reinterpret_cast<const half_t*>(img_f) + (size_t)i * RS + 8 * hi + 32 * s0;
+    const half_t* lrow = reinterpret_cast<const half_t*>(lo_f) + (size_t)i * (NIN + 8) + 8 * hi;
+    const float un = img_f[(size_t)i * (NIN + 4) + NIN] * un_x;
+    f32x16 acc[MT];
+#pragma unroll
+    for (int m = 0; m < MT; ++m)
+        acc[m] = f32x16{0.f, 0.f, 0.f, 0.f, 0.f, 0.f, 0.f, 0.f, 0.f, 0.f, 0.f, 0.f, 0.f, 0.f, 0.f, 0.f};
+    typedef unsigned u4_t __attribute__((ext_vector_type(4)));
+#pragma unroll
+    for (int s = 0; s < NK; ++s) {
+        const h8_t bh = __builtin_bit_cast(h8_t, u4_t{x.h[4 * s], x.h[4 * s + 1], x.h[4 * s + 2], x.h[4 * s + 3]});
+        const h8_t bl = __builtin_bit_cast(h8_t, u4_t{x.l[4 * s], x.l[4 * s + 1], x.l[4 * s + 2], x.l[4 * s + 3]});
+        h8_t bt;
+        if constexpr (NT == 3)
+            bt = __builtin_bit_cast(h8_t, u4_t{x.t[4 * s], x.t[4 * s + 1], x.t[4 * s + 2], x.t[4 * s + 3]});
+        h8_t ah[MT], al[MT], at[MT];
+#pragma unroll
+        for (int m = 0; m < MT; ++m) {
+            const half_t* a = row + (size_t)(32 * m) * RS + 32 * s;
+            ah[m] = *reinterpret_cast<const h8_t*>(a);
+            al[m] = *reinterpret_cast<const h8_t*>(a + 16);
+            if constexpr (NT == 3) at[m] = lo_frag_rt<NIN>(lrow, m, s0 + s);
+        }
+        mfma_terms<MT, NT>(acc, ah, al, at, bh, bl, bt);
+    }
+#pragma unroll
+    for (int m = 0; m < MT; ++m)
+#pragma unroll
+        for (int k = 0; k < 16; ++k) y[16 * m + k] = acc[m][k] * un;
 }
 
 typedef short sv4_t __attribute__((__vector_size__(4 * sizeof(short))));
@@ -404,6 +495,16 @@
     }
 }
 
+template <int PREC, int NOUT, int NIN, bool RAW = false>
+__device__ __forceinline__ void mvx_plane(const float* img, const float* lo, const float (&x1)[16], int pl,
+                                          float (&y)[NOUT / 2], int i, int hi, float* yf = nullptr) {
+    if constexpr (PREC == PREC_F32) {
+        mv_fwd_cols<NOUT, NIN, 4>(img, x1, 4 * pl, y, i, hi);
+        if (RAW) *yf = 1.f;
+    } else {
+        mv16_ks<NOUT, NIN, 2, RAW, PrecNT<PREC>::value>(img, x1, 2 * pl, y, i, hi, 1.f, yf, lo);
+    }
+}
 #define LO_W1 LDS_W_FLOATS
 #define LO_W2 (LO_W1 + LO16_FLOATS(64, 32))
 #define LO_V1 (LO_W2 + LO16_FLOATS(64, 64))
```
